# ChunLI-666/PointCloudProcessor

Hardware: AMD Instinct MI355X
Metric: Mpoints×frames/sec colorized (higher is better)
Workload: dtype f32/f64

## Files before the change

### include/pcp_hip.h

```cpp
#ifndef PCP_HIP_H
#define PCP_HIP_H

#include <stdint.h>

#ifdef __cplusplus
extern "C" {
#endif

#define PCP_ABI_VERSION 6

#define PCP_OK 0
#define PCP_ERR_INVALID (-1)
#define PCP_ERR_STATE (-2)
#define PCP_ERR_DEVICE (-3)
#define PCP_ERR_NOMEM (-4)
#define PCP_ERR_RANGE (-5)

typedef struct pcp_context pcp_context;

typedef struct pcp_pose {
  double x, y, z, qw, qx, qy, qz;
} pcp_pose;

typedef struct pcp_camera {
// ... 87 lines not shown
  int32_t h, v;
  int32_t blocks_w, blocks_h;
  int32_t down_w, down_h;
} pcp_jpeg_component;
typedef struct pcp_jpeg_header {
  uint32_t magic, version;
  int32_t width, height, ncomp, reserved;
  pcp_jpeg_component comp[3];
  int64_t n_blocks, n_values;
  int64_t quant_off, mask_off, offset_off, value_off;
} pcp_jpeg_header;
int pcp_upload_image_jpeg(pcp_context *ctx, int32_t frame, const uint8_t *blob, int64_t bytes);
int pcp_upload_image_jpeg_async(pcp_context *ctx, int32_t frame, const uint8_t *blob, int64_t bytes);
int pcp_upload_mask(pcp_context *ctx, int32_t frame, const uint8_t *gray, int64_t row_stride_bytes);

int pcp_project_frame(pcp_context *ctx, int32_t frame, int32_t *out_cell, int32_t *out_pixel, float *out_range,
                      float *out_xyz_cam);
int pcp_cull_frame(pcp_context *ctx, int32_t frame, uint8_t *out_keep, int64_t *out_kept, float *out_depth_map);
int pcp_frame_visible(pcp_context *ctx, int32_t frame, int64_t capacity, int32_t *out_index, uint8_t *out_rgb,
                      uint16_t *out_mask, float *out_xyz_cam, float *out_xyz_world, int64_t *out_count);

int pcp_hpr_stats(pcp_context *ctx, int64_t out[10]);

int pcp_depth_pass(pcp_context *ctx, int32_t frame_begin, int32_t frame_end);
int pcp_depth_maps_device(pcp_context *ctx, void **device_ptr, int64_t *n_floats);
int pcp_download_depth_map(pcp_context *ctx, int32_t frame, float *out_depth_map);
int pcp_depth_accum_reset(pcp_context *ctx);
int pcp_depth_accum_merge(pcp_context *ctx);
int pcp_depth_accum_apply(pcp_context *ctx);
int pcp_depth_accum_device(pcp_context *ctx, void **device_ptr, int64_t *n_floats);
#define PCP_DEPTH_OWN 0
#define PCP_DEPTH_BATCHED 1
int pcp_set_depth_source(pcp_context *ctx, int32_t source);
int pcp_hull_flags_import(pcp_context *ctx, int32_t frame, const uint8_t *keep);
int pcp_colour_reset(pcp_context *ctx);
int pcp_colour_pass(pcp_context *ctx, int32_t frame_begin, int32_t frame_end);
int pcp_colour_finalise(pcp_context *ctx, uint8_t *out_rgb, uint8_t *out_has, int32_t *out_count,
                        float *out_top_score, uint32_t *out_top_rgb, int32_t *out_top_frame);
int pcp_colorize(pcp_context *ctx, uint8_t *out_rgb, uint8_t *out_has);
int pcp_colorize_from_depth(pcp_context *ctx, uint8_t *out_rgb, uint8_t *out_has);
int pcp_download_result_packed(pcp_context *ctx, uint32_t *out_rgba);
int pcp_download_result_packed_async(pcp_context *ctx, uint32_t *out_rgba);
int pcp_download_wait_previous(pcp_context *ctx);
int pcp_colour_result_device(pcp_context *ctx, void **device_ptr, int64_t *n_words);
int pcp_colour_compact(pcp_context *ctx, int64_t capacity, int32_t *out_index, float *out_xyz, uint8_t *out_rgb, uint8_t *out_label,
                       int64_t *out_count);

int pcp_set_label_fusion(pcp_context *ctx, int32_t enable);
int pcp_colour_labels(pcp_context *ctx, uint8_t *out_label, uint8_t *out_hits, uint8_t *out_views);
int pcp_colour_labels_device(pcp_context *ctx, void **device_ptr, int64_t *n_words);

int pcp_view_pair_stats(pcp_context *ctx, uint64_t *out_n, uint64_t *out_sum);
int pcp_view_pair_stats_counters(pcp_context *ctx, int64_t out[5]);
int pcp_exposure_gains(int32_t n_frames, const uint64_t *n, const uint64_t *sum, double sigma_n, double sigma_g, double *out_gains);
int pcp_set_frame_gains(pcp_context *ctx, const double *gains, int32_t n);

int pcp_colour_smooth_local(pcp_context *ctx, float radius, int64_t *out_has_count);
int pcp_colour_smooth_local_packed(pcp_context *ctx, float radius, const uint32_t *in_rgba, uint32_t *out_rgba,
                                   int64_t *out_has_count);

int pcp_mls_process(pcp_context *ctx, const pcp_mls_params *p, int64_t *out_count);
int pcp_set_mls_local_plane(pcp_context *ctx, double upsampling_radius, double upsampling_step);
int pcp_mls_local_plane_samples(double radius, double step, int64_t capacity, float *out_u, float *out_v, int64_t *out_count);
int pcp_mls_process_shard(pcp_context *ctx, const pcp_mls_params *p, int64_t index_begin, int64_t index_end,
                          int64_t *out_count);
int pcp_mls_process_slab(pcp_context *ctx, const pcp_mls_params *p, int32_t slab, int32_t n_slabs, int64_t *out_count);
int pcp_mls_stream_begin(pcp_context *ctx, const pcp_mls_params *p, int64_t chunk_capacity, int64_t *out_total,
                         int32_t *out_chunks);
int pcp_mls_stream_next(pcp_context *ctx, int64_t *out_count);
int pcp_mls_stream_seek(pcp_context *ctx, int32_t chunk);
int pcp_mls_fetch(pcp_context *ctx, int64_t capacity, float *out_xyz, float *out_normal, float *out_curvature,
                  int32_t *out_index);
int pcp_cloud_smooth(pcp_context *ctx, const pcp_mls_params *p, int64_t *out_count);

int pcp_cloud_smooth_stream_begin(pcp_context *ctx, const pcp_mls_params *p, int64_t chunk_capacity, int64_t *out_total_rows,
                                  int64_t *out_kept_rows, int32_t *out_chunks);
int pcp_cloud_smooth_stream_next(pcp_context *ctx, int64_t *out_count);
int pcp_cloud_smooth_stream_end(pcp_context *ctx);
int pcp_cloud_smooth_stream_seek(pcp_context *ctx, int32_t chunk);
int pcp_cloud_smooth_stream_stats(pcp_context *ctx, double out[13]);
int pcp_sor(pcp_context *ctx, int32_t mean_k, double std_mul, uint8_t *out_keep, int64_t *out_kept);
int64_t pcp_sor_chunk_points(void);
int pcp_sor_partial(pcp_context *ctx, int32_t mean_k, int32_t slab, int32_t n_slabs, int64_t capacity, double *out_chunk_sums,
                    int64_t *out_first_chunk, int64_t *out_chunks);
int pcp_sor_finish(pcp_context *ctx, double std_mul, const double *all_chunk_sums, int64_t n_chunks, int32_t slab, int32_t n_slabs,
                   uint8_t *out_keep, int64_t *out_kept);

int pcp_upload_intensity(pcp_context *ctx, const float *intensity, int64_t n);
int pcp_nid_prepare(pcp_context *ctx, int64_t *out_points);
int pcp_nid_evaluate(pcp_context *ctx, const double T[16], const double *T_init, int32_t bins, double *cost,
                     double grad6[6], int32_t *valid);
int pcp_nid_optimize(pcp_context *ctx, const double T_init[16], int32_t bins, int32_t max_outer_iterations,
                     double T_out[16], double *final_cost, int32_t *evaluations);

int pcp_nid_accumulate(pcp_context *ctx, const double T[16], int32_t bins);
int pcp_nid_histograms_device(pcp_context *ctx, void **device_ptr, int64_t *count);
int pcp_nid_finish(pcp_context *ctx, int32_t bins, double *cost, double grad6[6], int32_t *valid);
typedef int (*pcp_nid_eval_fn)(void *user, const double T[16], int32_t bins, double *cost, double grad6[6], int32_t *valid);
int pcp_nid_optimize_with(pcp_context *ctx, pcp_nid_eval_fn eval, void *user, const double T_init[16], int32_t bins,
                          int32_t max_outer_iterations, double T_out[16], double *final_cost, int32_t *evaluations);

#define PCP_ROWS_XYZI 0
#define PCP_ROWS_XYZRGB 1
#define PCP_ROWS_XYZRGBMASK 2
#define PCP_ROWS_POINTNORMAL 3
int64_t pcp_ascii_row_bound(int32_t kind);
int pcp_ascii_rows_host(int32_t kind, int64_t n, const float *f, const uint8_t *rgb, const uint16_t *mask, int64_t capacity,
                        char *out_text, int64_t *out_bytes);
int pcp_ascii_rows(pcp_context *ctx, int32_t kind, int64_t n, const float *f, const uint8_t *rgb, const uint16_t *mask,
                   int64_t capacity, char *out_text, int64_t *out_bytes);
int pcp_colour_compact_ascii(pcp_context *ctx, int32_t with_label, int64_t first_row, int64_t max_rows, int64_t capacity,
                             char *out_text, int64_t *out_rows, int64_t *out_bytes);
int pcp_mls_fetch_ascii(pcp_context *ctx, int64_t first_row, int64_t max_rows, int64_t capacity, char *out_text,
                        int64_t *out_rows, int64_t *out_bytes);

#define PCP_ASCII_PARSE_MAX_ROW 65536
#define PCP_PARSE_LIMIT_ROW 0
#define PCP_PARSE_LIMIT_TILE 1
#define PCP_PARSE_LIMIT_PIECE 2
#define PCP_PARSE_LIMIT_TILE_ROWS 3
#define PCP_PARSE_LIMIT_WINDOW 4
int64_t pcp_ascii_parse_limit(int32_t which);
int pcp_ascii_parse_host(const char *text, int64_t bytes, int32_t columns, const int32_t col[4], int32_t final_window,
                         int64_t max_rows, float *out_x, float *out_y, float *out_z, float *out_intensity,
                         int64_t *out_rows, int64_t *out_consumed, int64_t *out_bad_row);
int pcp_ascii_parse(pcp_context *ctx, const char *text, int64_t bytes, int32_t columns, const int32_t col[4], int32_t final_window,
                    int64_t max_rows, float *out_x, float *out_y, float *out_z, float *out_intensity,
                    int64_t *out_rows, int64_t *out_consumed, int64_t *out_bad_row);

int pcp_voxel_reduce_begin(pcp_context *ctx, float leaf, int64_t initial_slots);
int pcp_voxel_reduce_add(pcp_context *ctx, int64_t *out_rows_added);
int pcp_voxel_reduce_finish(pcp_context *ctx, int64_t *out_voxels);
int pcp_voxel_reduce_fetch(pcp_context *ctx, int64_t first, int64_t max_rows, float *out_xyz, uint8_t *out_rgb, uint8_t *out_label,
                           uint32_t *out_count, int64_t *out_rows);
int pcp_voxel_reduce_stats(pcp_context *ctx, int64_t out[6]);
int pcp_voxel_reduce_end(pcp_context *ctx);
int pcp_voxel_reduce_host(float leaf, int64_t n, const float *xyz, const uint8_t *rgb, const uint8_t *label, int64_t capacity,
                          float *out_xyz, uint8_t *out_rgb, uint8_t *out_label, uint32_t *out_count, int64_t *out_voxels);

int pcp_estimate_normals(pcp_context *ctx, float radius, int64_t *out_valid, int64_t *out_moments);
int pcp_normals_fetch(pcp_context *ctx, float *out_normal, float *out_curvature, int32_t *out_neighbours);
int pcp_normals_moments_host(float radius, int64_t n, const float *xyz, int64_t *out_moments);
int pcp_frame_geometry(pcp_context *ctx, int32_t frame, int32_t *out_index, float *out_range, float *out_xyz_cam,
                       float *out_normal_cam, int64_t *out_pixels);

int pcp_close_pairs(pcp_context *ctx, double radius, int64_t *points_with_close_neighbour);

int pcp_timing_enable(pcp_context *ctx, int32_t on);
int pcp_timing_reset(pcp_context *ctx);
int pcp_timing_get(pcp_context *ctx, int32_t kernel_id, double *total_ms, int64_t *launches);
const char *pcp_kernel_name(int32_t kernel_id);
int pcp_tile_mask_density(pcp_context *ctx, double *kept_fraction);
int pcp_tile_masks(pcp_context *ctx, int64_t *tiles, int32_t *mask_words, uint32_t *out_words);
int pcp_sor_redo_fraction(pcp_context *ctx, double *fraction);
int pcp_sor_distances(pcp_context *ctx, int64_t capacity, float *out_distance);
int pcp_selftest_arithmetic(pcp_context *ctx, int64_t samples, uint64_t seed, int64_t *mismatches_fp64,
                            int64_t *mismatches_fp32);
int pcp_selftest_visit_forms(pcp_context *ctx, int64_t samples, uint64_t seed, int64_t *mismatches_uv, int64_t *mismatches_cell,
                             int64_t *mismatches_sqrt, int32_t *short_distortion);

#ifdef __cplusplus
}
#endif
#endif
```

### pointcloudprocessor_amd/_build.py

```python
from __future__ import annotations

import os
import subprocess

_PKG = os.path.dirname(os.path.abspath(__file__))
_ROOT = os.path.dirname(_PKG)
CSRC = os.path.join(_PKG, "csrc")
LIB_DIR = os.path.join(_PKG, "lib")
LIB_PATH = os.path.join(LIB_DIR, "libpcp_hip.so")
INCLUDE = os.path.join(_ROOT, "include")

SOURCES = ["pcp_context.hip", "pcp_colour.hip", "pcp_mls.hip", "pcp_nid.hip", "pcp_hpr.hip", "pcp_colour_smooth.hip", "pcp_match.hip", "pcp_jpeg.hip",
           "pcp_stream_colour.hip", "pcp_ascii.hip", "pcp_ascii_parse.hip", "pcp_exposure.hip", "pcp_voxel_reduce.hip", "pcp_normals.hip"]
HEADERS = ["pcp_internal.hpp", "pcp_device.hpp", "pcp_scan.hpp", "pcp_hsv.hpp", "pcp_exact.hpp", "pcp_ascii.hpp", "pcp_ascii_parse.hpp", "pcp_visit_forms.hpp", "pcp_voxel_reduce.hpp", "pcp_eigen33.hpp", "pcp_normals.hpp"]

HIPCC_FLAGS = [
    "--offload-arch=gfx950",
    "-O3",
    "-std=c++17",
    "-fPIC",
    "-ffp-contract=off",
    "-fhip-fp32-correctly-rounded-divide-sqrt",
    "-Wall",
    "-Wextra",
]


def _hipcc() -> str:
    for cand in (os.environ.get("HIPCC"), "/opt/rocm/bin/hipcc", "hipcc"):
        if cand and (os.path.isabs(cand) and os.path.exists(cand) or not os.path.isabs(cand)):
            return cand
    return "hipcc"


def source_sha256() -> str:
    import hashlib

    h = hashlib.sha256()
    h.update(" ".join(HIPCC_FLAGS).encode())
    for f in [os.path.join(CSRC, f) for f in SOURCES + HEADERS] + [os.path.join(INCLUDE, "pcp_hip.h")]:
        h.update(os.path.basename(f).encode())
        with open(f, "rb") as fh:
            h.update(fh.read())
    return h.hexdigest()


def is_stale() -> bool:
    if not os.path.exists(LIB_PATH):
        return True
    t = os.path.getmtime(LIB_PATH)
    deps = [os.path.join(CSRC, f) for f in SOURCES + HEADERS] + [os.path.join(INCLUDE, "pcp_hip.h")]
    return any(os.path.getmtime(d) > t for d in deps)


def build(force: bool = False, verbose: bool = False) -> str:
    if not force and not is_stale():
        return LIB_PATH
    os.makedirs(LIB_DIR, exist_ok=True)
    from concurrent.futures import ThreadPoolExecutor

    obj_dir = os.path.join(LIB_DIR, "obj")
    os.makedirs(obj_dir, exist_ok=True)
    inc = ["-I", os.path.relpath(INCLUDE, CSRC), "-I", "."]

    def compile_one(src):
        stem = os.path.splitext(src)[0]
        obj = os.path.join(os.path.relpath(obj_dir, CSRC), stem + ".o")
        cmd = [_hipcc()] + HIPCC_FLAGS + inc + [f"-cuid={stem}", "-c", src, "-o", obj]
        return cmd, subprocess.run(cmd, capture_output=True, text=True, cwd=CSRC)

    with ThreadPoolExecutor(max_workers=len(SOURCES)) as pool:
        results = list(pool.map(compile_one, SOURCES))
    log = ""
    for cmd, proc in results:
        if verbose or proc.returncode != 0:
            log += " ".join(cmd) + "\n" + proc.stdout + proc.stderr
    if any(proc.returncode != 0 for _, proc in results):
        print(log)
        raise RuntimeError("hipcc failed building libpcp_hip.so:\n" + log[-4000:])
    objs = [os.path.join(os.path.relpath(obj_dir, CSRC), os.path.splitext(src)[0] + ".o") for src in SOURCES]
    link = [_hipcc(), "--offload-arch=gfx950", "--hip-link", "-shared", "-fPIC", "-o", LIB_PATH] + objs
    proc = subprocess.run(link, capture_output=True, text=True, cwd=CSRC)
    if verbose or proc.returncode != 0:
        print(log + " ".join(link))
        print(proc.stdout)
        print(proc.stderr)
    if proc.returncode != 0:
        raise RuntimeError("hipcc failed linking libpcp_hip.so:\n" + proc.stderr[-4000:])
    return LIB_PATH


if __name__ == "__main__":
    print(build(force=True, verbose=True))
```

### pointcloudprocessor_amd/capi.py

```python
from __future__ import annotations

import ctypes as C
import os
import re

import numpy as np

from . import _build

PCP_OK = 0
PCP_ERR_INVALID = -1
PCP_ERR_STATE = -2
PCP_ERR_DEVICE = -3
PCP_ERR_NOMEM = -4
PCP_ERR_RANGE = -5

NID_EVAL_FN = C.CFUNCTYPE(C.c_int, C.c_void_p, C.POINTER(C.c_double), C.c_int32, C.POINTER(C.c_double), C.POINTER(C.c_double),
                          C.POINTER(C.c_int32))
K_PROJECT, K_DEPTH, K_COLOUR, K_VISIBILITY, K_MLS_GRID, K_MLS_FIT, K_MISC, K_SOR, K_MLS_VOXEL, K_TILE_MASK, K_NID, K_HPR = range(12)
K_COLOUR_SMOOTH = 12
K_COUNT = 13


class PcpError(RuntimeError):
# ... 780 lines not shown
        xyz = np.empty((count, 3), np.float32)
        nrm = np.empty((count, 3), np.float32)
        curv = np.empty(count, np.float32)
        idx = np.empty(count, np.int32)
        self._check(self.lib.pcp_mls_fetch(self.h, C.c_int64(count), _ptr(xyz), _ptr(nrm), _ptr(curv), _ptr(idx)))
        return dict(xyz=xyz, normal=nrm, curvature=curv, index=idx)

    def mls_fetch_index(self, count: int) -> np.ndarray:
        idx = np.empty(count, np.int32)
        self._check(self.lib.pcp_mls_fetch(self.h, C.c_int64(count), None, None, None, _ptr(idx)))
        return idx

    def sor(self, mean_k: int = 60, std_mul: float = 0.7):
        keep = np.empty(self.n, np.uint8)
        kept = C.c_int64()
        self._check(self.lib.pcp_sor(self.h, C.c_int32(mean_k), C.c_double(std_mul), _ptr(keep), C.byref(kept)))
        return keep, kept.value

    def sor_chunk_points(self) -> int:
        return int(self.lib.pcp_sor_chunk_points())

    def sor_partial(self, mean_k: int, slab: int, n_slabs: int):
        c = self.sor_chunk_points()
        chunks = (self.n + c - 1) // c
        out = np.zeros((max(chunks, 1), 2), np.float64)
        first, cnt = C.c_int64(), C.c_int64()
        self._check(self.lib.pcp_sor_partial(self.h, C.c_int32(mean_k), C.c_int32(slab), C.c_int32(n_slabs), C.c_int64(len(out)),
                                             _ptr(out), C.byref(first), C.byref(cnt)))
        return first.value, out[:cnt.value].copy()

    def sor_finish(self, std_mul: float, all_chunk_sums: np.ndarray, slab: int, n_slabs: int):
        sums = np.ascontiguousarray(all_chunk_sums, np.float64)
        keep = np.empty(self.n, np.uint8)
        kept = C.c_int64()
        self._check(self.lib.pcp_sor_finish(self.h, C.c_double(std_mul), _ptr(sums), C.c_int64(len(sums)), C.c_int32(slab),
                                            C.c_int32(n_slabs), _ptr(keep), C.byref(kept)))
        return keep, kept.value

    def close_pairs(self, radius: float = 2.5e-5) -> int:
        cnt = C.c_int64()
        self._check(self.lib.pcp_close_pairs(self.h, C.c_double(radius), C.byref(cnt)))
        return cnt.value

    def sor_distances(self) -> np.ndarray:
        out = np.empty(self.n, np.float32)
        self._check(self.lib.pcp_sor_distances(self.h, C.c_int64(len(out)), _ptr(out)))
        return out

    def sor_redo_fraction(self) -> float:
        v = C.c_double()
        self._check(self.lib.pcp_sor_redo_fraction(self.h, C.byref(v)))
        return v.value

    def upload_intensity(self, intensity):
        a = np.ascontiguousarray(intensity, np.float32)
        self._check(self.lib.pcp_upload_intensity(self.h, _ptr(a), C.c_int64(len(a))))

    def nid_prepare(self) -> int:
        cnt = C.c_int64()
        self._check(self.lib.pcp_nid_prepare(self.h, C.byref(cnt)))
        return cnt.value

    def nid_evaluate(self, T, T_init=None, bins: int = 16):
        T = np.ascontiguousarray(T, np.float64).reshape(16)
        Ti = None if T_init is None else np.ascontiguousarray(T_init, np.float64).reshape(16)
        cost = C.c_double()
        grad = np.zeros(6, np.float64)
        valid = C.c_int32()
        self._check(self.lib.pcp_nid_evaluate(self.h, _ptr(T), _ptr(Ti), C.c_int32(bins), C.byref(cost), _ptr(grad),
                                              C.byref(valid)))
        return cost.value, grad, bool(valid.value)

    def nid_optimize(self, T_init, bins: int = 16, max_outer_iterations: int = 10):
        Ti = np.ascontiguousarray(T_init, np.float64).reshape(16)
        out = np.zeros(16, np.float64)
        cost = C.c_double()
        evals = C.c_int32()
        self._check(self.lib.pcp_nid_optimize(self.h, _ptr(Ti), C.c_int32(bins), C.c_int32(max_outer_iterations), _ptr(out),
                                              C.byref(cost), C.byref(evals)))
        return out.reshape(4, 4), cost.value, evals.value

    def nid_accumulate(self, T, bins: int = 16):
        T = np.ascontiguousarray(T, np.float64).reshape(16)
        self._check(self.lib.pcp_nid_accumulate(self.h, _ptr(T), C.c_int32(bins)))

    def nid_histograms_device(self):
        p = C.c_void_p()
        n = C.c_int64()
        self._check(self.lib.pcp_nid_histograms_device(self.h, C.byref(p), C.byref(n)))
        return p.value, n.value

    def nid_finish(self, bins: int = 16):
        cost = C.c_double()
        grad = np.zeros(6, np.float64)
        valid = C.c_int32()
        self._check(self.lib.pcp_nid_finish(self.h, C.c_int32(bins), C.byref(cost), _ptr(grad), C.byref(valid)))
        return cost.value, grad, bool(valid.value)

    def nid_optimize_with(self, evaluate, T_init, bins: int = 16, max_outer_iterations: int = 10):
        errors = []

        @NID_EVAL_FN
        def trampoline(_user, T, b, cost, grad, valid):
            try:
                c, g, ok = evaluate(np.ctypeslib.as_array(T, (16,)).copy().reshape(4, 4), int(b))
                cost[0] = float(c)
                for k in range(6):
                    grad[k] = float(g[k])
                valid[0] = 1 if ok else 0
                return 0
            except Exception as e:
                errors.append(e)
                return -3

        Ti = np.ascontiguousarray(T_init, np.float64).reshape(16)
        out = np.zeros(16, np.float64)
        cost = C.c_double()
        evals = C.c_int32()
        rc = self.lib.pcp_nid_optimize_with(self.h, trampoline, None, _ptr(Ti), C.c_int32(bins), C.c_int32(max_outer_iterations),
                                            _ptr(out), C.byref(cost), C.byref(evals))
        if errors:
            raise errors[0]
        self._check(rc)
        return out.reshape(4, 4), cost.value, evals.value

    def timing_enable(self, on: bool = True):
        self._check(self.lib.pcp_timing_enable(self.h, C.c_int32(1 if on else 0)))

    def timing_reset(self):
        self._check(self.lib.pcp_timing_reset(self.h))

    def timing_get(self, kernel_id: int):
        ms = C.c_double()
        cnt = C.c_int64()
        self._check(self.lib.pcp_timing_get(self.h, C.c_int32(kernel_id), C.byref(ms), C.byref(cnt)))
        return ms.value, cnt.value

    def tile_mask_density(self) -> float:
        v = C.c_double()
        self._check(self.lib.pcp_tile_mask_density(self.h, C.byref(v)))
        return v.value

    def selftest_arithmetic(self, samples: int = 1 << 26, seed: int = 1):
        a, b = C.c_int64(), C.c_int64()
        self._check(self.lib.pcp_selftest_arithmetic(self.h, C.c_int64(samples), C.c_uint64(seed), C.byref(a), C.byref(b)))
        return a.value, b.value

    def selftest_visit_forms(self, samples: int = 1 << 24, seed: int = 1):
        a, b, c, f = C.c_int64(), C.c_int64(), C.c_int64(), C.c_int32()
        self._check(self.lib.pcp_selftest_visit_forms(self.h, C.c_int64(samples), C.c_uint64(seed), C.byref(a), C.byref(b), C.byref(c),
                                                      C.byref(f)))
        return a.value, b.value, c.value, bool(f.value)

    def tile_masks(self) -> np.ndarray:
        t, w = C.c_int64(), C.c_int32()
        self._check(self.lib.pcp_tile_masks(self.h, C.byref(t), C.byref(w), None))
        out = np.empty((t.value, w.value), np.uint32)
        self._check(self.lib.pcp_tile_masks(self.h, None, None, _ptr(out)))
        return out

    def kernel_name(self, kernel_id: int) -> str:
        return self.lib.pcp_kernel_name(C.c_int32(kernel_id)).decode()
```

### pointcloudprocessor_amd/csrc/pcp_colour.hip

```cpp
#include <algorithm>
#include <cfloat>
#include <cstdlib>

#include "pcp_device.hpp"
#include "pcp_hsv.hpp"
#include "pcp_scan.hpp"

namespace pcp {

constexpr int kBlock = 256;
constexpr uint32_t kFltMaxBits = 0x7f7fffffu;

template <bool kCommon>
__device__ __forceinline__ DevCamera common_camera(const DevCamera &in) {
  DevCamera c = in;
  if constexpr (kCommon) {
    c.cull_mode = PCP_CULL_ZBUFFER;
    c.enable_zbuf = 1;
    c.pretest = 1;
    c.ds_fast = 1;
  }
  return c;
}
inline bool is_common_camera(const pcp_context *ctx) {
  const DevCamera &c = ctx->dcam;
  return c.cull_mode == PCP_CULL_ZBUFFER && c.enable_zbuf == 1 && c.pretest == 1 && c.ds_fast == 1 && ctx->uv_tame;
}

struct ProjectOut {
  int32_t *cell;
  int32_t *pixel;
  float *range;
  float *xc, *yc, *zc;
};

__device__ __forceinline__ void project_store_one(const DevCamera &cam, const DevFrame &fr, float x, float y, float z,
                                                  int32_t &cell, int32_t &pixel, float &range, float &xc, float &yc,
                                                  float &zc) {
  const Projected p = project_point<true, false>(cam, fr.w2c, x, y, z);
  cell = p.cell;
  pixel = p.pixel;
  range = p.cell != -1 ? static_cast<float>(range64(p.xc, p.yc, p.zc)) : FLT_MAX;
  xc = p.xc;
  yc = p.yc;
  zc = p.zc;
}

template <bool kCommon>
__global__ __launch_bounds__(kBlock) void k_project_frame(const float *__restrict__ x, const float *__restrict__ y,
                                                          const float *__restrict__ z, int64_t n, DevCamera cam_in,
                                                          DevFrame fr, ProjectOut out) {
  const DevCamera cam = common_camera<kCommon>(cam_in);
  const int64_t q = static_cast<int64_t>(blockIdx.x) * kBlock + threadIdx.x;
  const int64_t i0 = q * 4;
  if (i0 >= n) return;
  if (i0 + 3 < n) {
    typedef float nt_f4 __attribute__((ext_vector_type(4)));
    typedef int nt_i4 __attribute__((ext_vector_type(4)));
    const nt_f4 ax = __builtin_nontemporal_load(reinterpret_cast<const nt_f4 *>(x + i0));
    const nt_f4 ay = __builtin_nontemporal_load(reinterpret_cast<const nt_f4 *>(y + i0));
    const nt_f4 az = __builtin_nontemporal_load(reinterpret_cast<const nt_f4 *>(z + i0));
    const float4 vx = make_float4(ax.x, ax.y, ax.z, ax.w), vy = make_float4(ay.x, ay.y, ay.z, ay.w),
                 vz = make_float4(az.x, az.y, az.z, az.w);
    int4 cell, pixel;
    float4 range, xc, yc, zc;
    project_store_one(cam, fr, vx.x, vy.x, vz.x, cell.x, pixel.x, range.x, xc.x, yc.x, zc.x);
    project_store_one(cam, fr, vx.y, vy.y, vz.y, cell.y, pixel.y, range.y, xc.y, yc.y, zc.y);
    project_store_one(cam, fr, vx.z, vy.z, vz.z, cell.z, pixel.z, range.z, xc.z, yc.z, zc.z);
    project_store_one(cam, fr, vx.w, vy.w, vz.w, cell.w, pixel.w, range.w, xc.w, yc.w, zc.w);
    if (out.cell) {
      const nt_i4 c4 = {cell.x, cell.y, cell.z, cell.w};
      __builtin_nontemporal_store(c4, reinterpret_cast<nt_i4 *>(out.cell + i0));
    }
    if (out.range) {
      const nt_f4 r4 = {range.x, range.y, range.z, range.w};
      __builtin_nontemporal_store(r4, reinterpret_cast<nt_f4 *>(out.range + i0));
    }
    if (out.pixel) *reinterpret_cast<int4 *>(out.pixel + i0) = pixel;
    if (out.xc) {
      *reinterpret_cast<float4 *>(out.xc + i0) = xc;
      *reinterpret_cast<float4 *>(out.yc + i0) = yc;
      *reinterpret_cast<float4 *>(out.zc + i0) = zc;
    }
  } else {
    for (int64_t i = i0; i < n; ++i) {
      int32_t cell, pixel;
      float range, xc, yc, zc;
      project_store_one(cam, fr, x[i], y[i], z[i], cell, pixel, range, xc, yc, zc);
      if (out.cell) out.cell[i] = cell;
      if (out.range) out.range[i] = range;
      if (out.pixel) out.pixel[i] = pixel;
      if (out.xc) {
        out.xc[i] = xc;
        out.yc[i] = yc;
        out.zc[i] = zc;
      }
    }
  }
}

struct Interval {
  double lo, hi;
};
__device__ __forceinline__ Interval iv_add(Interval a, Interval b) { return {a.lo + b.lo, a.hi + b.hi}; }
__device__ __forceinline__ Interval iv_scale(double k, Interval a) {
  return k >= 0.0 ? Interval{k * a.lo, k * a.hi} : Interval{k * a.hi, k * a.lo};
}
__device__ __forceinline__ Interval iv_mul(Interval a, Interval b) {
  const double p0 = a.lo * b.lo, p1 = a.lo * b.hi, p2 = a.hi * b.lo, p3 = a.hi * b.hi;
  return {fmin(fmin(p0, p1), fmin(p2, p3)), fmax(fmax(p0, p1), fmax(p2, p3))};
}
__device__ __forceinline__ Interval iv_sqr(Interval a) {
  const double l = fabs(a.lo), h = fabs(a.hi);
  const double mx = fmax(l, h), mn = (a.lo <= 0.0 && a.hi >= 0.0) ? 0.0 : fmin(l, h);
  return {mn * mn, mx * mx};
}
__device__ __forceinline__ Interval iv_mul_pos(Interval a, Interval b) { return {a.lo * b.lo, a.hi * b.hi}; }
__device__ __forceinline__ Interval iv_mul_by_pos(Interval a, Interval b) {
  return {a.lo * (a.lo >= 0.0 ? b.lo : b.hi), a.hi * (a.hi >= 0.0 ? b.hi : b.lo)};
}
__device__ __forceinline__ double iv_rcp_pos(double b) {
  double r = __builtin_amdgcn_rcp(b);
  r = fma(fma(-b, r, 1.0), r, r);
  r = fma(fma(-b, r, 1.0), r, r);
  return r;
}
__device__ __forceinline__ Interval iv_pad(Interval a) {
  const double e = 1e-12 * (fabs(a.lo) + fabs(a.hi)) + 1e-300;
  return {a.lo - e, a.hi + e};
}

__device__ __forceinline__ int tile_classify(const DevCamera &c, const DevFrame &fr, float4 sph) {
  const double cx = sph.x, cy = sph.y, cz = sph.z;
  const float *m = fr.w2c;
  const double X = (m[0] * cx + m[1] * cy) + (m[2] * cz + m[3]);
  const double Y = (m[4] * cx + m[5] * cy) + (m[6] * cz + m[7]);
  const double Z = (m[8] * cx + m[9] * cy) + (m[10] * cz + m[11]);
  const double mag = fr.norm_bound * (fabs(cx) + fabs(cy) + fabs(cz) + 3.0 * sph.w) + fabs(static_cast<double>(m[3])) +
                     fabs(static_cast<double>(m[7])) + fabs(static_cast<double>(m[11])) + 1e-3;
  const double rho = fr.norm_bound * static_cast<double>(sph.w) * (1.0 + 1e-6) + 1e-6 * mag;
  if (!(rho >= 0.0) || !isfinite(X + Y + Z + rho)) return 0;
  if (Z + rho <= 0.0) return 1;
  if (Z - rho <= 0.0) return 0;
  const Interval zi{Z - rho, Z + rho};
  if (!(zi.lo >= 1e-290)) return 0;
  const Interval iz{iv_rcp_pos(zi.hi) * (1.0 - 1e-13), iv_rcp_pos(zi.lo) * (1.0 + 1e-13)};
  const Interval xn = iv_pad(iv_mul_by_pos(Interval{X - rho, X + rho}, iz));
  const Interval yn = iv_pad(iv_mul_by_pos(Interval{Y - rho, Y + rho}, iz));
  const Interval x2 = iv_sqr(xn), y2 = iv_sqr(yn);
  const Interval r2 = iv_add(x2, y2);
  const Interval r4 = iv_mul_pos(r2, r2);
  const Interval r6 = iv_mul_pos(r2, r4);
  Interval rc = iv_add(iv_add(iv_scale(c.k1, r2), iv_scale(c.k2, r4)), iv_scale(c.k3, r6));
  rc.lo += 1.0;
  rc.hi += 1.0;
  const Interval t1 = iv_scale(2.0, iv_mul(xn, yn));
  const Interval t2 = iv_add(r2, iv_scale(2.0, x2));
  const Interval t3 = iv_add(r2, iv_scale(2.0, y2));
  const Interval xd = iv_pad(iv_add(iv_add(iv_mul(rc, xn), iv_scale(c.p1, t1)), iv_scale(c.p2, t2)));
  const Interval yd = iv_pad(iv_add(iv_add(iv_mul(rc, yn), iv_scale(c.p1, t3)), iv_scale(c.p2, t1)));
  Interval u = iv_pad(iv_scale(c.fx, xd)), v = iv_pad(iv_scale(c.fy, yd));
  u.lo += c.cx; u.hi += c.cx;
  v.lo += c.cy; v.hi += c.cy;
  if (!isfinite(u.lo + u.hi + v.lo + v.hi)) return 0;
  if (u.hi < static_cast<double>(c.u_lo) || u.lo > static_cast<double>(c.u_hi) ||
      v.hi < static_cast<double>(c.v_lo) || v.lo > static_cast<double>(c.v_hi))
    return 1;
  return (u.lo > static_cast<double>(c.u_lo) + 1.0 && u.hi < static_cast<double>(c.u_hi) - 1.0 &&
          v.lo > static_cast<double>(c.v_lo) + 1.0 && v.hi < static_cast<double>(c.v_hi) - 1.0)
             ? 2
             : 0;
}

constexpr int kTileGroup = 16;

__global__ __launch_bounds__(kBlock) void k_group_mask_flat(const float4 *__restrict__ spheres, int64_t groups, DevCamera cam,
                                                            const DevFrame *__restrict__ frames, int32_t n_frames,
                                                            int32_t w0, int32_t w1, int32_t words,
                                                            uint32_t *__restrict__ group_mask,
                                                            uint32_t *__restrict__ group_inside, int32_t cull_enabled,
                                                            int32_t *__restrict__ zeroed, int32_t n_zeroed,
                                                            unsigned long long *__restrict__ far_maps, int64_t far_cells) {
  const int64_t idx = static_cast<int64_t>(blockIdx.x) * kBlock + threadIdx.x;
  if (idx < n_zeroed) zeroed[idx] = 0;
  for (int64_t c = idx; c < far_cells; c += static_cast<int64_t>(gridDim.x) * kBlock) far_maps[c] = 0x7f7f7f7f7f7f7f7full;
  const int32_t nw = w1 - w0;
  const int64_t gw = idx >> 5;
  const int64_t group = gw / nw;
  const bool live = group < groups;
  const int32_t w = w0 + static_cast<int32_t>(gw - group * nw);
  const int32_t f = (w << 5) + static_cast<int32_t>(idx & 31);
  int cls = 1;
  if (live && f < n_frames) cls = cull_enabled ? tile_classify(cam, frames[f], spheres[group]) : 0;
  const unsigned long long m = __ballot(cls != 1), in = __ballot(cls == 2);
  if (live && (idx & 31) == 0) {
    group_mask[group * words + w] = static_cast<uint32_t>((threadIdx.x & 32) ? (m >> 32) : m);
    group_inside[group * words + w] = static_cast<uint32_t>((threadIdx.x & 32) ? (in >> 32) : in);
  }
}

__global__ __launch_bounds__(kBlock) void k_tile_mask_dense(const float4 *__restrict__ spheres, int64_t tiles,
                                                            DevCamera cam, const DevFrame *__restrict__ frames,
                                                            int32_t n_frames, int32_t w0, int32_t w1, int32_t words,
                                                            const uint32_t *__restrict__ group_mask,
                                                            const uint32_t *__restrict__ group_inside,
                                                            uint32_t *__restrict__ tile_mask,
                                                            uint32_t *__restrict__ inside_mask, int32_t cull_enabled) {
  const int lane = threadIdx.x & 63;
  const int32_t nw = w1 - w0;
  const int64_t gw = static_cast<int64_t>(blockIdx.x) * (kBlock / 64) + (threadIdx.x >> 6);
  const int64_t group = gw / nw;
  if (group >= (tiles + kTileGroup - 1) / kTileGroup) return;
  const int32_t w = w0 + static_cast<int32_t>(gw - group * nw);
  const int t = lane & 15, slot = lane >> 4;
  const int64_t tile = group * kTileGroup + t;
  const bool have = tile < tiles;
  uint32_t todo = __builtin_amdgcn_readfirstlane(group_mask[group * words + w]);
  const int32_t nb = n_frames - (w << 5);
  if (nb < 32) todo &= nb <= 0 ? 0u : ((1u << nb) - 1u);
  const uint32_t whole = __builtin_amdgcn_readfirstlane(group_inside[group * words + w]) & todo;
  todo &= ~whole;
  uint32_t word = whole, inside = whole;
  if (todo) {
    const float4 sph = spheres[have ? tile : tiles - 1];
    while (todo) {
      int32_t bit[4];
#pragma unroll
      for (int k = 0; k < 4; ++k) {
        bit[k] = todo ? __builtin_ctz(todo) : -1;
        todo &= todo - (todo ? 1u : 0u);
      }
      const int32_t b = slot == 0 ? bit[0] : slot == 1 ? bit[1] : slot == 2 ? bit[2] : bit[3];
      int cls = 1;
      if (b >= 0 && have) cls = cull_enabled ? tile_classify(cam, frames[(w << 5) + b], sph) : 0;
      const unsigned long long keep = __ballot(cls != 1), ins = __ballot(cls == 2);
#pragma unroll
      for (int k = 0; k < 4; ++k) {
        if (bit[k] >= 0) {
          word |= static_cast<uint32_t>((keep >> (k * 16 + t)) & 1ull) << bit[k];
          inside |= static_cast<uint32_t>((ins >> (k * 16 + t)) & 1ull) << bit[k];
        }
      }
    }
  }
  if (slot == 0 && have) {
    tile_mask[tile * words + w] = word;
    if (inside_mask) inside_mask[tile * words + w] = inside;
  }
}

constexpr int kWorkBins = 1024;
constexpr int kWorkPerBlock = 1024;
__global__ __launch_bounds__(kBlock) void k_tile_work_hist(const uint32_t *__restrict__ tile_mask, int64_t tiles, int32_t w0,
                                                          int32_t w1, int32_t words, int32_t *__restrict__ tile_work,
                                                          int32_t *__restrict__ hist) {
  __shared__ int32_t cnt[kWorkBins];
  for (int b = threadIdx.x; b < kWorkBins; b += kBlock) cnt[b] = 0;
  __syncthreads();
  const int64_t base = static_cast<int64_t>(blockIdx.x) * kWorkPerBlock;
  for (int q = 0; q < kWorkPerBlock / kBlock; ++q) {
    const int64_t t = base + q * kBlock + threadIdx.x;
    if (t < tiles) {
      int32_t visits = 0;
      for (int32_t w = w0; w < w1; ++w) visits += __builtin_popcount(tile_mask[t * words + w]);
      tile_work[t] = visits;
      atomicAdd(&cnt[min(visits, kWorkBins - 1)], 1);
    }
  }
  __syncthreads();
  for (int b = threadIdx.x; b < kWorkBins; b += kBlock)
    if (cnt[b]) atomicAdd(&hist[b], cnt[b]);
}
__device__ __forceinline__ int32_t block_exclusive_scan(int32_t v, int32_t *total);
__global__ __launch_bounds__(kBlock) void k_work_scatter(const int32_t *__restrict__ work, int64_t tiles,
                                                        const int32_t *__restrict__ hist, int32_t *__restrict__ cursor,
                                                        int32_t *__restrict__ order) {
  __shared__ int32_t cnt[kWorkBins];
  __shared__ int32_t first[kWorkBins];
  for (int b = threadIdx.x; b < kWorkBins; b += kBlock) cnt[b] = 0;
  {
    constexpr int kPer = kWorkBins / kBlock;
    int32_t h[kPer], mine = 0;
#pragma unroll
    for (int k = 0; k < kPer; ++k) {
      h[k] = hist[kWorkBins - 1 - (static_cast<int>(threadIdx.x) * kPer + k)];
      mine += h[k];
    }
    int32_t total = 0;
    int32_t run = block_exclusive_scan(mine, &total);
#pragma unroll
    for (int k = 0; k < kPer; ++k) {
      first[kWorkBins - 1 - (static_cast<int>(threadIdx.x) * kPer + k)] = run;
      run += h[k];
    }
  }
  __syncthreads();
  const int64_t base = static_cast<int64_t>(blockIdx.x) * kWorkPerBlock;
  int32_t bin[kWorkPerBlock / kBlock], rank[kWorkPerBlock / kBlock];
#pragma unroll
  for (int q = 0; q < kWorkPerBlock / kBlock; ++q) {
    const int64_t t = base + q * kBlock + threadIdx.x;
    bin[q] = t < tiles ? min(work[t], kWorkBins - 1) : -1;
    rank[q] = bin[q] >= 0 ? atomicAdd(&cnt[bin[q]], 1) : 0;
  }
  __syncthreads();
  for (int b = threadIdx.x; b < kWorkBins; b += kBlock)
    if (cnt[b]) cnt[b] = first[b] + atomicAdd(&cursor[b], cnt[b]);
  __syncthreads();
#pragma unroll
  for (int q = 0; q < kWorkPerBlock / kBlock; ++q)
    if (bin[q] >= 0) order[cnt[bin[q]] + rank[q]] = static_cast<int32_t>(base + q * kBlock + threadIdx.x);
}

constexpr uint32_t kXcdChunk = 16;
__device__ __forceinline__ uint32_t xcd_chunked_block() {
  constexpr uint32_t kXcd = 8, kSuper = kXcd * kXcdChunk;
  const uint32_t b = blockIdx.x;
  if (b >= (gridDim.x / kSuper) * kSuper) return b;
  const uint32_t x = b % kXcd, slot = b / kXcd;
  return ((slot / kXcdChunk) * kXcd + x) * kXcdChunk + slot % kXcdChunk;
}

constexpr unsigned long long kDepthEmpty = 0x7f7f7f7f7f7f7f7full;
__device__ __forceinline__ void depth_min(unsigned long long *__restrict__ map, int32_t cell, unsigned long long bits) {
  if (bits < map[cell]) atomicMin(map + cell, bits);
}
__device__ __forceinline__ double sumsq64(float xc, float yc, float zc) {
  const double X = xc, Y = yc, Z = zc;
  return (X * X + Y * Y) + Z * Z;
}
__global__ __launch_bounds__(kBlock) void k_depth_finish(const unsigned long long *__restrict__ sq, int64_t count,
                                                         uint32_t *__restrict__ range) {
  int64_t i = static_cast<int64_t>(blockIdx.x) * kBlock + threadIdx.x;
  const int64_t stride = static_cast<int64_t>(gridDim.x) * kBlock;
  for (; i < count; i += stride) {
    const unsigned long long b = sq[i];
    float r = FLT_MAX;
    if (b != kDepthEmpty) r = fminf(static_cast<float>(sqrt(__longlong_as_double(static_cast<long long>(b)))), FLT_MAX);
    range[i] = __float_as_uint(r);
  }
}

__device__ __forceinline__ uint32_t range_bits(int32_t w, int32_t f0, int32_t f1) {
  const int32_t fb = max(f0, w << 5), fe = min(f1, (w << 5) + 32);
  const int32_t nb = fe - fb;
  return nb <= 0 ? 0u : (((nb >= 32) ? 0xffffffffu : ((1u << nb) - 1u)) << (fb & 31));
}

template <bool kCommon>
__global__ __launch_bounds__(kBlock) void k_depth_pass(const float *__restrict__ x, const float *__restrict__ y,
                                                       const float *__restrict__ z, int64_t n, DevCamera cam_in,
                                                       const DevFrame *__restrict__ frames, int32_t f0, int32_t f1,
                                                       unsigned long long *__restrict__ depth, int64_t cells,
                                                       int32_t depth_first_frame, uint32_t *__restrict__ tile_mask,
                                                       const uint32_t *__restrict__ tile_inside, int32_t words,
                                                       const int32_t *__restrict__ tile_order) {
  DevCamera cam = common_camera<kCommon>(cam_in);
  if constexpr (kCommon) cam.pretest = 0;
  __shared__ unsigned long long combine[kBlock];
  const int lane = threadIdx.x & 63;
  unsigned long long *tbl = combine + (threadIdx.x & ~63);
  const int64_t j = tile_order ? static_cast<int64_t>(tile_order[blockIdx.x]) * 64 + threadIdx.x
                               : static_cast<int64_t>(xcd_chunked_block()) * kBlock + threadIdx.x;
  const bool live = j < n;
  if (!__ballot(live)) return;
  const float px = live ? x[j] : 0.0f, py = live ? y[j] : 0.0f, pz = live ? z[j] : 0.0f;
  const int64_t tile = __builtin_amdgcn_readfirstlane(static_cast<int32_t>(j >> 6));
  const bool finite_sure = cam.frames_bounded != 0 && __all(fabsf(px) <= 0x1p40f && fabsf(py) <= 0x1p40f && fabsf(pz) <= 0x1p40f);
  unsigned long long *held_at = nullptr;
  unsigned long long held_bits = 0ull, held_seen = 0ull;
  auto settle_held = [&]() {
    if (held_at && held_bits < held_seen) atomicMin(held_at, held_bits);
    held_at = nullptr;
  };
  for (int32_t w = f0 >> 5; w <= (f1 - 1) >> 5; ++w) {
    const uint32_t in_range = range_bits(w, f0, f1);
    uint32_t todo = in_range;
    if (tile_mask) todo &= tile_mask[tile * words + w];
    todo = __builtin_amdgcn_readfirstlane(todo);
    const uint32_t inside = tile_inside ? __builtin_amdgcn_readfirstlane(tile_inside[tile * words + w]) : 0u;
    uint32_t seen = 0u;
    while (todo) {
      const int32_t b = __builtin_ctz(todo);
      const int32_t f = (w << 5) + b;
      todo &= todo - 1u;
      const DevFrame &fr = frames[f];
      const auto p = project_visit<true, kCommon>(cam, fr.w2c, px, py, pz, ((inside >> b) & 1u) == 0u, finite_sure);
      bool in_map, cand;
      if constexpr (kCommon) {
        in_map = live && p.map_ok;
        cand = in_map && p.image_ok;
      } else {
        in_map = live && p.cell >= 0;
        cand = live && p.pixel >= 0 && (cam.enable_zbuf ? p.cell >= 0 : p.cell != -1);
      }
      if (__builtin_amdgcn_ballot_w64(cand)) seen |= 1u << b;
      settle_held();
      if (cam.enable_zbuf && __builtin_amdgcn_ballot_w64(in_map)) {
        unsigned long long *map = depth + static_cast<uint64_t>(static_cast<uint32_t>(f - depth_first_frame)) * static_cast<uint32_t>(cells);
        unsigned long long key = ~0ull, sbits = 0ull;
        if (in_map) {
          sbits = static_cast<unsigned long long>(__double_as_longlong(sumsq64(p.xc, p.yc, p.zc)));
          key = (static_cast<unsigned long long>(static_cast<uint32_t>(p.cell)) << 32) | (sbits >> 32);
        }
        tbl[lane] = ~0ull;
        __builtin_amdgcn_wave_barrier();
        if (in_map) atomicMin(&tbl[p.cell & 63], key);
        __builtin_amdgcn_wave_barrier();
        if (in_map) {
          const unsigned long long got = tbl[p.cell & 63];
          if (got == key || static_cast<uint32_t>(got >> 32) != static_cast<uint32_t>(p.cell)) {
            held_at = map + p.cell;
            held_bits = sbits;
            held_seen = *held_at;
          }
        }
        __builtin_amdgcn_wave_barrier();
      }
    }
    if (tile_mask && lane == 0 && live) {
      uint32_t *dst = tile_mask + tile * words + w;
      *dst = (*dst & ~in_range) | seen;
    }
  }
  settle_held();
}

__global__ __launch_bounds__(kBlock) void k_visibility(const float *__restrict__ x, const float *__restrict__ y,
                                                       const float *__restrict__ z, int64_t n, DevCamera cam,
                                                       DevFrame fr, const uint32_t *__restrict__ depth,
                                                       const int32_t *__restrict__ perm,
                                                       uint8_t *__restrict__ keep, int32_t require_pixel) {
  const int64_t i = static_cast<int64_t>(blockIdx.x) * kBlock + threadIdx.x;
  if (i >= n) return;
  const Projected p = project_point(cam, fr.w2c, x[i], y[i], z[i]);
  bool k = keep_rule(cam, p, depth);
  if (require_pixel) k = k && p.pixel >= 0;
  if (k) keep[perm ? perm[i] : i] = 1;
}

__device__ __forceinline__ bool keep_by_depth(float xc, float yc, float zc, double lim) {
  const double s = sumsq64(xc, yc, zc);
  const double L = lim * lim;
  bool keep = s < L * (1.0 - 0x1p-40);
  const bool sure = lim > 0.0 && (keep || s > L * (1.0 + 0x1p-40));
  if (!sure) keep = !(sqrt(s) > lim);
  return keep;
}

struct TopState {
  float *score;
  uint32_t *rgb;
  int32_t *frame;
  int32_t *count;
};

struct MatchArgs {
  const uint8_t *in_a;
  unsigned long long *moved;
  float e2;
};

struct LabelOut {
  uint32_t *word;
};

template <bool kCommon, int kMatch, bool kOneShot, bool kLabel = false>
__global__ __launch_bounds__(kBlock) void k_colour_pass(const float *__restrict__ x, const float *__restrict__ y,
                                                        const float *__restrict__ z, int64_t n, DevCamera cam_in,
                                                        const DevFrame *__restrict__ frames, int32_t f0, int32_t f1,
                                                        const uint32_t *__restrict__ depth, int64_t cells,
                                                        const uint32_t *__restrict__ tile_mask, int32_t words,
                                                        const uint32_t *__restrict__ images, int64_t image_px,
                                                        TopState st, const int32_t *__restrict__ perm,
                                                        uint32_t *__restrict__ rgba, int32_t flags_in,
                                                        const uint32_t *__restrict__ hull_bits_in, MatchArgs mb,
                                                        [[maybe_unused]] LabelOut lab) {
  constexpr bool kShort = kCommon && kOneShot && kMatch == 2;
  DevCamera cam = common_camera<kCommon>(cam_in);
  if constexpr (kMatch == 1) cam.match_mode = PCP_MATCH_IDENTITY;
  if constexpr (kMatch == 2 || kMatch == 3) cam.match_mode = PCP_MATCH_ROUNDTRIP;
  const uint32_t *__restrict__ hull_bits = kCommon ? nullptr : hull_bits_in;
  const int32_t flags = kOneShot ? 4 : flags_in;
  const int64_t j = static_cast<int64_t>(xcd_chunked_block()) * kBlock + threadIdx.x;
  const bool live = j < n;
  if (!__ballot(live)) return;
  const float px = live ? x[j] : 0.0f, py = live ? y[j] : 0.0f, pz = live ? z[j] : 0.0f;
  const int64_t tile = __builtin_amdgcn_readfirstlane(static_cast<int32_t>(j >> 6));
  const bool finite_sure = cam.frames_bounded != 0 && __all(fabsf(px) <= 0x1p40f && fabsf(py) <= 0x1p40f && fabsf(pz) <= 0x1p40f);
  Top5 t;
  t.init();
  if ((flags & 1) && live) {
    t.s0 = st.score[0 * n + j]; t.s1 = st.score[1 * n + j]; t.s2 = st.score[2 * n + j];
    t.s3 = st.score[3 * n + j]; t.s4 = st.score[4 * n + j];
    t.c0 = st.rgb[0 * n + j]; t.c1 = st.rgb[1 * n + j]; t.c2 = st.rgb[2 * n + j];
    t.c3 = st.rgb[3 * n + j]; t.c4 = st.rgb[4 * n + j];
    t.f0 = st.frame[0 * n + j]; t.f1 = st.frame[1 * n + j]; t.f2 = st.frame[2 * n + j];
    t.f3 = st.frame[3 * n + j]; t.f4 = st.frame[4 * n + j];
    t.count = st.count[j];
  }
  [[maybe_unused]] bool in_a = false;
  [[maybe_unused]] uint32_t moved = 0u;
  if constexpr (kMatch == 3) in_a = live && mb.in_a[j] != 0;
  for (int32_t w = f0 >> 5; w <= (f1 - 1) >> 5; ++w) {
    uint32_t todo = range_bits(w, f0, f1);
    if (tile_mask) todo &= tile_mask[tile * words + w];
    todo = __builtin_amdgcn_readfirstlane(todo);
    const uint32_t hull_word = (hull_bits && live) ? hull_bits[static_cast<int64_t>(w) * n + j] : 0xffffffffu;
    while (todo) {
      const int32_t f = (w << 5) + __builtin_ctz(todo);
      todo &= todo - 1u;
      const DevFrame &fr = frames[f];
      const auto p = project_visit<false, kShort>(cam, fr.w2c, px, py, pz, true, finite_sure);
      bool cand;
      if constexpr (kShort)
        cand = live && p.image_ok && p.map_ok && ((hull_word >> (f & 31)) & 1u);
      else
        cand = live && p.pixel >= 0 && (cam.enable_zbuf ? p.cell >= 0 : p.cell != -1) && ((hull_word >> (f & 31)) & 1u);
      if (cand) {
        const uint32_t dbits = cam.enable_zbuf ? depth[static_cast<uint64_t>(static_cast<uint32_t>(f)) * static_cast<uint32_t>(cells) + static_cast<uint32_t>(p.cell)] : 0u;
        bool keep = true;
        if (cam.enable_zbuf) keep = keep_by_depth(p.xc, p.yc, p.zc, static_cast<double>(__uint_as_float(dbits)) + cam.slack);
        float sx = p.xc, sy = p.yc, sz = p.zc;
        if constexpr (kMatch == 3) {
          if (keep) keep = roundtrip_sample_moved(cam, fr, px, py, pz, sx, sy, sz, mb.e2, moved) && !in_a;
        } else {
          if (cam.match_mode == PCP_MATCH_ROUNDTRIP && keep) keep = roundtrip_sample(cam, fr, px, py, pz, sx, sy, sz);
        }
        if (keep) {
          const uint32_t texel = images[static_cast<uint64_t>(static_cast<uint32_t>(f)) * static_cast<uint32_t>(image_px) + static_cast<uint32_t>(p.pixel)];
          t.insert(final_score<kShort>(sx, sy, sz, fr.px, fr.py, fr.pz), kLabel ? texel : texel & 0xffffffu, f);
        }
      }
    }
  }
  if constexpr (kMatch == 3) {
    if (moved) atomicAdd(mb.moved, static_cast<unsigned long long>(moved));
  }
  if (!live) return;
  if (flags & 2) {
    st.score[0 * n + j] = t.s0; st.score[1 * n + j] = t.s1; st.score[2 * n + j] = t.s2;
    st.score[3 * n + j] = t.s3; st.score[4 * n + j] = t.s4;
    st.rgb[0 * n + j] = t.c0; st.rgb[1 * n + j] = t.c1; st.rgb[2 * n + j] = t.c2;
    st.rgb[3 * n + j] = t.c3; st.rgb[4 * n + j] = t.c4;
    st.frame[0 * n + j] = t.f0; st.frame[1 * n + j] = t.f1; st.frame[2 * n + j] = t.f2;
    st.frame[3 * n + j] = t.f3; st.frame[4 * n + j] = t.f4;
    st.count[j] = t.count;
  }
  if (flags & 4) {
    const int64_t o = perm[j];
    rgba[o] = t.finalise();
    if constexpr (kLabel) {
      uint32_t bad = 0u;
      lab.word[o] = t.labels(bad);
      if (bad) lab.word[n] = 1u;
    }
  }
}

__device__ __forceinline__ Top5 load_top5(const TopState &st, int64_t n, int64_t j) {
  Top5 t;
  t.s0 = st.score[0 * n + j]; t.s1 = st.score[1 * n + j]; t.s2 = st.score[2 * n + j];
  t.s3 = st.score[3 * n + j]; t.s4 = st.score[4 * n + j];
  t.c0 = st.rgb[0 * n + j]; t.c1 = st.rgb[1 * n + j]; t.c2 = st.rgb[2 * n + j];
  t.c3 = st.rgb[3 * n + j]; t.c4 = st.rgb[4 * n + j];
  t.f0 = st.frame[0 * n + j]; t.f1 = st.frame[1 * n + j]; t.f2 = st.frame[2 * n + j];
  t.f3 = st.frame[3 * n + j]; t.f4 = st.frame[4 * n + j];
  t.count = st.count[j];
  return t;
}
__global__ __launch_bounds__(kBlock) void k_finalise(int64_t n, TopState st, const int32_t *__restrict__ perm,
// ... 47 lines not shown
    const DevFrame &fr = frames[f];
    const int32_t w = f >> 5;
    const uint32_t bit = 1u << (f & 31);
    for (int64_t r = r0; r < r1; ++r) {
      const int64_t i = cols[r];
      if (tile_mask && !(tile_mask[(i >> 6) * words + w] & bit)) continue;
      if (hull_bits && !(hull_bits[static_cast<int64_t>(w) * n + i] & bit)) continue;
      const float px = x[i], py = y[i], pz = z[i];
      const Projected p = project_point<false>(cam, fr.w2c, px, py, pz);
      const bool cand = p.pixel >= 0 && (cam.enable_zbuf ? p.cell >= 0 : p.cell != -1);
      if (!cand) continue;
      if (cam.enable_zbuf) {
        const uint32_t dbits = depth[static_cast<uint64_t>(static_cast<uint32_t>(f)) * static_cast<uint32_t>(cells) + static_cast<uint32_t>(p.cell)];
        if (!keep_by_depth(p.xc, p.yc, p.zc, static_cast<double>(__uint_as_float(dbits)) + cam.slack)) continue;
      }
      float sx = p.xc, sy = p.yc, sz = p.zc;
      if (!roundtrip_sample(cam, fr, qx, qy, qz, sx, sy, sz)) continue;
      const uint32_t texel = images[static_cast<uint64_t>(static_cast<uint32_t>(f)) * static_cast<uint32_t>(image_px) + static_cast<uint32_t>(p.pixel)];
      t.insert(final_score(sx, sy, sz, fr.px, fr.py, fr.pz), kLabel ? texel : texel & 0xffffffu, f);
    }
  }
  if (flags & 2) {
    st.score[0 * n + j] = t.s0; st.score[1 * n + j] = t.s1; st.score[2 * n + j] = t.s2;
    st.score[3 * n + j] = t.s3; st.score[4 * n + j] = t.s4;
    st.rgb[0 * n + j] = t.c0; st.rgb[1 * n + j] = t.c1; st.rgb[2 * n + j] = t.c2;
    st.rgb[3 * n + j] = t.c3; st.rgb[4 * n + j] = t.c4;
    st.frame[0 * n + j] = t.f0; st.frame[1 * n + j] = t.f1; st.frame[2 * n + j] = t.f2;
    st.frame[3 * n + j] = t.f3; st.frame[4 * n + j] = t.f4;
    st.count[j] = t.count;
  }
  if (flags & 4) {
    const int64_t o = perm[j];
    rgba[o] = t.finalise();
    if constexpr (kLabel) {
      uint32_t bad = 0u;
      lab.word[o] = t.labels(bad);
      if (bad) lab.word[n] = 1u;
    }
  }
}

template <bool kLabel>
inline auto colour_pass_kernel(bool common, int32_t match_mode, int32_t flags) {
  auto kernel = k_colour_pass<false, 0, false, kLabel>;
  if (common && match_mode == PCP_MATCH_IDENTITY)
    kernel = flags == 4 ? k_colour_pass<true, 1, true, kLabel> : k_colour_pass<true, 1, false, kLabel>;
  if (common && match_mode == PCP_MATCH_ROUNDTRIP)
    kernel = flags == 4 ? k_colour_pass<true, 2, true, kLabel> : k_colour_pass<true, 2, false, kLabel>;
  if (match_mode == PCP_MATCH_RADIUS)
    kernel = !common ? k_colour_pass<false, 3, false, kLabel>
                     : flags == 4 ? k_colour_pass<true, 3, true, kLabel> : k_colour_pass<true, 3, false, kLabel>;
  return kernel;
}

__device__ __forceinline__ uint64_t mix64(uint64_t v) {
  v += 0x9e3779b97f4a7c15ull;
  v = (v ^ (v >> 30)) * 0xbf58476d1ce4e5b9ull;
  v = (v ^ (v >> 27)) * 0x94d049bb133111ebull;
  return v ^ (v >> 31);
}
__device__ __forceinline__ bool same_f64(double a, double b) {
  if (a != a && b != b) return true;
  if (a == 0.0 && b == 0.0) return true;
  return __double_as_longlong(a) == __double_as_longlong(b);
}

__global__ __launch_bounds__(kBlock) void k_selftest_div64(int64_t samples, uint64_t seed,
                                                           unsigned long long *__restrict__ bad) {
  const int64_t i = static_cast<int64_t>(blockIdx.x) * kBlock + threadIdx.x;
  if (i >= samples) return;
  const uint64_t a = mix64(seed ^ static_cast<uint64_t>(i) * 3u), b = mix64(a);
  uint32_t bx = static_cast<uint32_t>(a), by = static_cast<uint32_t>(a >> 32), bz = static_cast<uint32_t>(b);
  const uint32_t mode = static_cast<uint32_t>(b >> 32) & 3u;
  if (mode != 0u) {
    const uint32_t span = mode == 1u ? 12u : 40u;
    bx = (bx & 0x807fffffu) | ((127u - span / 2u + (bx >> 23) % span) << 23);
    by = (by & 0x807fffffu) | ((127u - span / 2u + (by >> 23) % span) << 23);
    bz = (bz & 0x807fffffu) | ((127u - span / 2u + (bz >> 23) % span) << 23);
  }
  const float xc = __uint_as_float(bx), yc = __uint_as_float(by), zc = fabsf(__uint_as_float(bz));
  if (!(zc > 0.0f)) return;
  double xn, yn;
  divide_xy_by_z(xc, yc, zc, xn, yn);
  const double xr = static_cast<double>(xc) / static_cast<double>(zc);
  const double yr = static_cast<double>(yc) / static_cast<double>(zc);
  if (!same_f64(xn, xr) || !same_f64(yn, yr)) atomicAdd(bad, 1ull);
}

__global__ __launch_bounds__(kBlock) void k_selftest_div32(DevCamera cam, unsigned long long *__restrict__ bad) {
  const uint32_t lane = blockIdx.x * kBlock + threadIdx.x;
  uint32_t wrong = 0u;
  for (uint32_t k = 0; k < 256u; ++k) {
    const float x = __uint_as_float((k << 24) | lane);
    const float a = div_by_ds(cam, x), b = x / cam.ds_f;
    const float ax = fabsf(x);
    if (ax >= 0x1p-40f && ax <= 0x1p60f) {
      if (!((a != a && b != b) || __float_as_uint(a) == __float_as_uint(b))) ++wrong;
    } else {
      if (cell_of_quotient(a, cam.cull_wf) != cell_of_quotient(b, cam.cull_wf)) ++wrong;
      if (cell_of_quotient(a, cam.cull_hf) != cell_of_quotient(b, cam.cull_hf)) ++wrong;
    }
  }
  if (wrong) atomicAdd(bad, static_cast<unsigned long long>(wrong));
}

__device__ __forceinline__ bool same_bits_f64(double a, double b) {
  return (a != a && b != b) || __double_as_longlong(a) == __double_as_longlong(b);
}
__global__ __launch_bounds__(kBlock) void k_selftest_uv(DevCamera cam, int32_t tame, int64_t samples, uint64_t seed,
                                                        unsigned long long *__restrict__ bad) {
  const int64_t i = static_cast<int64_t>(blockIdx.x) * kBlock + threadIdx.x;
  if (i >= samples) return;
  const uint64_t a = mix64(seed ^ static_cast<uint64_t>(i) * 3u), b = mix64(a);
  uint32_t bx = static_cast<uint32_t>(a), by = static_cast<uint32_t>(a >> 32), bz = static_cast<uint32_t>(b);
  const uint32_t mode = static_cast<uint32_t>(b >> 32) & 3u;
  if (mode != 0u) {
    const uint32_t span = mode == 1u ? 12u : 40u;
    bx = (bx & 0x807fffffu) | ((127u - span / 2u + (bx >> 23) % span) << 23);
    by = (by & 0x807fffffu) | ((127u - span / 2u + (by >> 23) % span) << 23);
    bz = (bz & 0x807fffffu) | ((127u - span / 2u + (bz >> 23) % span) << 23);
  }
  const float xc = __uint_as_float(bx), yc = __uint_as_float(by), zc = fabsf(__uint_as_float(bz));
  if (!(zc > 0.0f)) return;
  double u0, v0, u1, v1;
  if (tame)
    project_uv<true, true>(cam, xc, yc, zc, u0, v0);
  else
    project_uv<true, false>(cam, xc, yc, zc, u0, v0);
  project_uv<true, false>(cam, xc, yc, zc, u1, v1);
  if (!same_bits_f64(u0, u1) || !same_bits_f64(v0, v1)) atomicAdd(bad, 1ull);
}

__global__ __launch_bounds__(kBlock) void k_selftest_cell_sqrt(DevCamera cam, unsigned long long *__restrict__ bad_cell,
                                                               unsigned long long *__restrict__ bad_sqrt) {
  const uint32_t lane = blockIdx.x * kBlock + threadIdx.x;
  uint32_t wrong_cell = 0u, wrong_sqrt = 0u;
  for (uint32_t k = 0; k < 256u; ++k) {
    const float q = __uint_as_float((k << 24) | lane);
    const float qx[3] = {q, 0.5f, q}, qy[3] = {0.5f, q, q};
#pragma unroll
    for (int t = 0; t < 3; ++t) {
      const int32_t old_cell = vf::map_cell_written(qx[t], qy[t], cam.cull_wf, cam.cull_hf, cam.mw, cam.mh);
      int32_t cell;
      const bool ok = vf::map_cell_short(qx[t], qy[t], vf::map_bound(cam.mw), vf::map_bound(cam.mh), cam.mw, cell);
      if ((ok ? cell : -1) != old_cell) ++wrong_cell;
    }
    const float r0 = sqrt_rn(q), r1 = sqrtf(q);
    if (!((r0 != r0 && r1 != r1) || __float_as_uint(r0) == __float_as_uint(r1))) ++wrong_sqrt;
  }
  if (wrong_cell) atomicAdd(bad_cell, static_cast<unsigned long long>(wrong_cell));
  if (wrong_sqrt) atomicAdd(bad_sqrt, static_cast<unsigned long long>(wrong_sqrt));
}

__global__ __launch_bounds__(kBlock) void k_unpack_result(const uint32_t *__restrict__ packed, int64_t n,
                                                         uint8_t *__restrict__ rgb, uint8_t *__restrict__ has) {
  const int64_t i = static_cast<int64_t>(blockIdx.x) * kBlock + threadIdx.x;
  if (i >= n) return;
  const uint32_t v = packed[i];
  rgb[3 * i + 0] = static_cast<uint8_t>(v & 0xffu);
  rgb[3 * i + 1] = static_cast<uint8_t>((v >> 8) & 0xffu);
  rgb[3 * i + 2] = static_cast<uint8_t>((v >> 16) & 0xffu);
  has[i] = static_cast<uint8_t>(v >> 24);
}

__global__ __launch_bounds__(kBlock) void k_unpack_labels(const uint32_t *__restrict__ packed, int64_t n,
                                                         uint8_t *__restrict__ label, uint8_t *__restrict__ hits,
                                                         uint8_t *__restrict__ views) {
  const int64_t i = static_cast<int64_t>(blockIdx.x) * kBlock + threadIdx.x;
  if (i >= n) return;
  const uint32_t v = packed[i];
  if (label) label[i] = static_cast<uint8_t>(v & 0xffu);
  if (hits) hits[i] = static_cast<uint8_t>((v >> 8) & 0xffu);
  if (views) views[i] = static_cast<uint8_t>((v >> 16) & 0xffu);
}

__global__ __launch_bounds__(kBlock) void k_fill_u32(uint32_t *__restrict__ p, int64_t n, uint32_t v) {
  int64_t i = static_cast<int64_t>(blockIdx.x) * kBlock + threadIdx.x;
  const int64_t stride = static_cast<int64_t>(gridDim.x) * kBlock;
  for (; i < n; i += stride) p[i] = v;
}

__global__ __launch_bounds__(kBlock) void k_scatter_u32(const uint32_t *__restrict__ in,
                                                        const int32_t *__restrict__ perm, int64_t n,
                                                        uint32_t *__restrict__ out) {
  const int64_t j = static_cast<int64_t>(blockIdx.x) * kBlock + threadIdx.x;
  if (j < n) out[perm[j]] = in[j];
}

__global__ __launch_bounds__(kBlock) void k_pack_bgr(const uint8_t *__restrict__ bgr, int64_t row_stride, int32_t w,
                                                     int32_t h, uint32_t *__restrict__ texels, int32_t clear_mask,
                                                     const int32_t *__restrict__ hsv_tables, float sat_scale,
                                                     float val_scale) {
  const int64_t i = static_cast<int64_t>(blockIdx.x) * kBlock + threadIdx.x;
  if (i >= static_cast<int64_t>(w) * h) return;
  const int32_t v = static_cast<int32_t>(i / w), u = static_cast<int32_t>(i - static_cast<int64_t>(v) * w);
  const uint8_t *p = bgr + static_cast<int64_t>(v) * row_stride + 3 * u;
  const uint32_t keep = clear_mask ? 0u : (texels[i] & 0xff000000u);
  uint32_t b = p[0], g = p[1], r = p[2];
  if (hsv_tables) hsv_round_trip(hsv_tables, hsv_tables + 256, sat_scale, val_scale, b, g, r);
  texels[i] = keep | b | (g << 8) | (r << 16);
}

__global__ __launch_bounds__(kBlock) void k_pack_bgr16(const uint8_t *__restrict__ bgr, int64_t row_stride, int32_t w,
                                                       int32_t h, uint32_t *__restrict__ texels, int32_t clear_mask,
                                                       const int32_t *__restrict__ hsv_tables, float sat_scale,
                                                       float val_scale) {
  const int32_t groups = w >> 4;
  const int64_t n_groups = static_cast<int64_t>(groups) * h;
  const int64_t g = static_cast<int64_t>(blockIdx.x) * kBlock + threadIdx.x;
  uint4 a, b, c;
  if (row_stride == 3 * static_cast<int64_t>(w)) {
    __shared__ uint4 piece[3 * kBlock];
    const int64_t base = static_cast<int64_t>(blockIdx.x) * (3 * kBlock);
    const int64_t pieces = 3 * n_groups;
    const uint4 *src = reinterpret_cast<const uint4 *>(bgr);
#pragma unroll
    for (int q = 0; q < 3; ++q) {
      const int64_t i = base + q * kBlock + threadIdx.x;
      if (i < pieces) piece[q * kBlock + threadIdx.x] = src[i];
    }
    __syncthreads();
    if (g >= n_groups) return;
    a = piece[3 * threadIdx.x];
    b = piece[3 * threadIdx.x + 1];
    c = piece[3 * threadIdx.x + 2];
  } else {
    if (g >= n_groups) return;
    const int32_t vr = static_cast<int32_t>(g / groups), gr = static_cast<int32_t>(g - static_cast<int64_t>(vr) * groups);
    const uint4 *src = reinterpret_cast<const uint4 *>(bgr + static_cast<int64_t>(vr) * row_stride + static_cast<int64_t>(gr) * 48);
    a = src[0];
    b = src[1];
    c = src[2];
  }
  const int32_t v = static_cast<int32_t>(g / groups), gu = static_cast<int32_t>(g - static_cast<int64_t>(v) * groups);
  const uint32_t in[12] = {a.x, a.y, a.z, a.w, b.x, b.y, b.z, b.w, c.x, c.y, c.z, c.w};
  uint4 *dst = reinterpret_cast<uint4 *>(texels + static_cast<int64_t>(v) * w + static_cast<int64_t>(gu) * 16);
  uint32_t out[16];
#pragma unroll
  for (int q = 0; q < 4; ++q) {
    const uint32_t d0 = in[3 * q], d1 = in[3 * q + 1], d2 = in[3 * q + 2];
    out[4 * q + 0] = d0 & 0xffffffu;
    out[4 * q + 1] = (d0 >> 24) | ((d1 & 0xffffu) << 8);
    out[4 * q + 2] = (d1 >> 16) | ((d2 & 0xffu) << 16);
    out[4 * q + 3] = d2 >> 8;
  }
  if (hsv_tables) {
#pragma unroll
    for (int k = 0; k < 16; ++k) {
      uint32_t bb = out[k] & 0xffu, gg = (out[k] >> 8) & 0xffu, rr = out[k] >> 16;
      hsv_round_trip(hsv_tables, hsv_tables + 256, sat_scale, val_scale, bb, gg, rr);
      out[k] = bb | (gg << 8) | (rr << 16);
    }
  }
  if (!clear_mask) {
#pragma unroll
    for (int q = 0; q < 4; ++q) {
      const uint4 old = dst[q];
      out[4 * q + 0] |= old.x & 0xff000000u;
      out[4 * q + 1] |= old.y & 0xff000000u;
      out[4 * q + 2] |= old.z & 0xff000000u;
      out[4 * q + 3] |= old.w & 0xff000000u;
    }
  }
#pragma unroll
  for (int q = 0; q < 4; ++q) dst[q] = make_uint4(out[4 * q], out[4 * q + 1], out[4 * q + 2], out[4 * q + 3]);
}

__global__ __launch_bounds__(kBlock) void k_pack_mask(const uint8_t *__restrict__ gray, int64_t row_stride, int32_t w,
                                                      int32_t h, uint32_t *__restrict__ texels) {
  const int64_t i = static_cast<int64_t>(blockIdx.x) * kBlock + threadIdx.x;
  if (i >= static_cast<int64_t>(w) * h) return;
  const int32_t v = static_cast<int32_t>(i / w), u = static_cast<int32_t>(i - static_cast<int64_t>(v) * w);
  texels[i] = (texels[i] & 0x00ffffffu) | (static_cast<uint32_t>(gray[static_cast<int64_t>(v) * row_stride + u]) << 24);
}

constexpr int kTile = 1024;

__device__ __forceinline__ int32_t block_exclusive_scan(int32_t v, int32_t *total) {
  __shared__ int32_t wave_sum[kBlock / 64];
  const int lane = threadIdx.x & 63, wid = threadIdx.x >> 6;
  int32_t incl = v;
#pragma unroll
  for (int o = 1; o < 64; o <<= 1) {
    const int32_t t = __shfl_up(incl, o, 64);
    if (lane >= o) incl += t;
  }
  if (lane == 63) wave_sum[wid] = incl;
  __syncthreads();
  int32_t base = 0, tot = 0;
#pragma unroll
  for (int k = 0; k < kBlock / 64; ++k) {
    if (k < wid) base += wave_sum[k];
    tot += wave_sum[k];
  }
  __syncthreads();
  *total = tot;
  return base + incl - v;
}

__global__ __launch_bounds__(kBlock) void k_tile_count(const uint8_t *__restrict__ flags, int64_t n,
                                                       int32_t *__restrict__ tile_count) {
  const int64_t base = static_cast<int64_t>(blockIdx.x) * kTile + threadIdx.x * 4;
  int32_t c = 0;
#pragma unroll
  for (int k = 0; k < 4; ++k)
    if (base + k < n) c += flags[base + k] ? 1 : 0;
// ... 597 lines not shown
                       row_stride_bytes, w, h, ctx->images.p + static_cast<int64_t>(frame) * px);
    PCP_HIP_TRY(ctx, hipGetLastError());
  }
  PCP_HIP_TRY(ctx, hipStreamSynchronize(ctx->stream));
  ctx->mask_set[static_cast<size_t>(frame)] = 1;
  return PCP_OK;
}

int pcp_project_frame(pcp_context *ctx, int32_t frame, int32_t *out_cell, int32_t *out_pixel, float *out_range,
                      float *out_xyz_cam) {
  int rc = check_ready(ctx, "pcp_project_frame", true);
  if (rc != PCP_OK) return rc;
  if ((rc = check_frame(ctx, "pcp_project_frame", frame)) != PCP_OK) return rc;
  const int64_t n = ctx->n;
  const size_t plane = plane_of(ctx);
  PCP_HIP_TRY(ctx, ctx->s_cell.ensure(plane + 4));
  PCP_HIP_TRY(ctx, ctx->s_range.ensure(plane + 4));
  if (out_pixel) PCP_HIP_TRY(ctx, ctx->s_pixel.ensure(plane + 4));
  if (out_xyz_cam) PCP_HIP_TRY(ctx, ctx->s_cam.ensure(3 * plane + 4));
  if (n == 0) return PCP_OK;
  ProjectOut o{};
  o.cell = ctx->s_cell.p;
  o.range = ctx->s_range.p;
  o.pixel = out_pixel ? ctx->s_pixel.p : nullptr;
  o.xc = out_xyz_cam ? ctx->s_cam.p : nullptr;
  o.yc = out_xyz_cam ? ctx->s_cam.p + plane : nullptr;
  o.zc = out_xyz_cam ? ctx->s_cam.p + 2 * plane : nullptr;
  {
    LaunchTimer t(ctx, PCP_K_PROJECT);
    hipLaunchKernelGGL(is_common_camera(ctx) ? k_project_frame<true> : k_project_frame<false>, dim3(blocks_for(div_up(n, 4))), dim3(kBlock), 0, ctx->stream, ctx->sxyz.p,
                       ctx->sxyz.p + plane, ctx->sxyz.p + 2 * plane, n, ctx->dcam,
                       ctx->hframes[static_cast<size_t>(frame)], o);
    PCP_HIP_TRY(ctx, hipGetLastError());
  }
  if (!(out_cell || out_range || out_pixel || out_xyz_cam)) return PCP_OK;
  const size_t sn = static_cast<size_t>(n);
  PCP_HIP_TRY(ctx, ctx->s_u32.ensure(plane + 4));
  auto fetch = [&](const void *sorted, void *host) -> int {
    {
      LaunchTimer t(ctx, PCP_K_MISC);
      hipLaunchKernelGGL(k_scatter_u32, dim3(blocks_for(n)), dim3(kBlock), 0, ctx->stream,
                         static_cast<const uint32_t *>(sorted), ctx->perm.p, n, ctx->s_u32.p);
      PCP_HIP_TRY(ctx, hipGetLastError());
    }
    PCP_HIP_TRY(ctx, hipMemcpyAsync(host, ctx->s_u32.p, sn * 4, hipMemcpyDeviceToHost, ctx->stream));
    PCP_HIP_TRY(ctx, hipStreamSynchronize(ctx->stream));
    return PCP_OK;
  };
  if (out_cell && (rc = fetch(o.cell, out_cell)) != PCP_OK) return rc;
  if (out_range && (rc = fetch(o.range, out_range)) != PCP_OK) return rc;
  if (out_pixel && (rc = fetch(o.pixel, out_pixel)) != PCP_OK) return rc;
  if (out_xyz_cam) {
    if ((rc = fetch(o.xc, out_xyz_cam)) != PCP_OK) return rc;
    if ((rc = fetch(o.yc, out_xyz_cam + sn)) != PCP_OK) return rc;
    if ((rc = fetch(o.zc, out_xyz_cam + 2 * sn)) != PCP_OK) return rc;
  }
  return PCP_OK;
}

int pcp_cull_frame(pcp_context *ctx, int32_t frame, uint8_t *out_keep, int64_t *out_kept, float *out_depth_map) {
  int rc = check_ready(ctx, "pcp_cull_frame", true);
  if (rc != PCP_OK) return rc;
  if ((rc = check_frame(ctx, "pcp_cull_frame", frame)) != PCP_OK) return rc;
  const int64_t n = ctx->n;
  if ((rc = single_frame_depth(ctx, frame)) != PCP_OK) return rc;
  if ((rc = frame_keep_flags(ctx, frame, false)) != PCP_OK) return rc;
  if (out_kept) {
    int64_t cnt = 0;
    if (n > 0 && (rc = compact_flags(ctx, ctx->s_keep.p, n, nullptr, 0, &cnt)) != PCP_OK) return rc;
    *out_kept = cnt;
  }
  if (out_keep && n > 0)
    PCP_HIP_TRY(ctx, hipMemcpyAsync(out_keep, ctx->s_keep.p, static_cast<size_t>(n), hipMemcpyDefault, ctx->stream));
  if (out_depth_map)
    PCP_HIP_TRY(ctx, hipMemcpyAsync(out_depth_map, ctx->s_u32.p, static_cast<size_t>(cells_of(ctx)) * 4,
                                    hipMemcpyDeviceToHost, ctx->stream));
  PCP_HIP_TRY(ctx, hipStreamSynchronize(ctx->stream));
  return PCP_OK;
}

int pcp_frame_visible(pcp_context *ctx, int32_t frame, int64_t capacity, int32_t *out_index, uint8_t *out_rgb,
                      uint16_t *out_mask, float *out_xyz_cam, float *out_xyz_world, int64_t *out_count) {
  int rc = check_ready(ctx, "pcp_frame_visible", true);
  if (rc != PCP_OK) return rc;
  if ((rc = check_frame(ctx, "pcp_frame_visible", frame)) != PCP_OK) return rc;
  if (capacity < 0) return set_error(ctx, PCP_ERR_INVALID, "pcp_frame_visible: negative capacity");
  const int64_t n = ctx->n;
  if (out_count) *out_count = 0;
  if (n == 0) return PCP_OK;
  if ((rc = ensure_images(ctx)) != PCP_OK) return rc;
  if ((rc = wait_images(ctx, frame, frame + 1)) != PCP_OK) return rc;
  int64_t m = 0;
  if ((rc = visible_indices(ctx, frame, &m)) != PCP_OK) return rc;
  const size_t plane = plane_of(ctx);
  if (out_count) *out_count = m;
  const int64_t take = std::min(m, capacity);
  if (take == 0) return PCP_OK;
  const size_t st = static_cast<size_t>(take);
  PCP_HIP_TRY(ctx, ctx->s_range.ensure(st + 4));
  const bool want_cam = out_xyz_cam != nullptr, want_world = out_xyz_world != nullptr;
  PCP_HIP_TRY(ctx, ctx->s_cam.ensure((want_cam ? 3 * st : 0) + (want_world ? 3 * st : 0) + 4));
  float *d_cam = want_cam ? ctx->s_cam.p : nullptr;
  float *d_world = want_world ? ctx->s_cam.p + (want_cam ? 3 * st : 0) : nullptr;
  const int64_t px = static_cast<int64_t>(ctx->dcam.img_w) * ctx->dcam.img_h;
  {
    LaunchTimer t(ctx, PCP_K_MISC);
    hipLaunchKernelGGL(k_gather_visible, dim3(blocks_for(take)), dim3(kBlock), 0, ctx->stream, ctx->xyz.p,
                       ctx->xyz.p + plane, ctx->xyz.p + 2 * plane, ctx->dcam, ctx->hframes[static_cast<size_t>(frame)],
                       ctx->s_cell.p, take, ctx->images.p + static_cast<int64_t>(frame) * px,
                       static_cast<int32_t>(ctx->image_set[static_cast<size_t>(frame)]),
                       static_cast<int32_t>(ctx->mask_set[static_cast<size_t>(frame)]),
                       reinterpret_cast<uint32_t *>(ctx->s_range.p), d_cam, d_world);
    PCP_HIP_TRY(ctx, hipGetLastError());
  }
  std::vector<uint32_t> rgbm;
  if (out_rgb || out_mask) {
    rgbm.resize(st);
    PCP_HIP_TRY(ctx, hipMemcpyAsync(rgbm.data(), ctx->s_range.p, st * 4, hipMemcpyDeviceToHost, ctx->stream));
  }
  if (out_index) PCP_HIP_TRY(ctx, hipMemcpyAsync(out_index, ctx->s_cell.p, st * 4, hipMemcpyDeviceToHost, ctx->stream));
  if (want_cam) PCP_HIP_TRY(ctx, hipMemcpyAsync(out_xyz_cam, d_cam, 3 * st * 4, hipMemcpyDeviceToHost, ctx->stream));
  if (want_world) PCP_HIP_TRY(ctx, hipMemcpyAsync(out_xyz_world, d_world, 3 * st * 4, hipMemcpyDeviceToHost, ctx->stream));
  PCP_HIP_TRY(ctx, hipStreamSynchronize(ctx->stream));
  for (size_t k = 0; k < rgbm.size(); ++k) {
    if (out_rgb) {
      out_rgb[3 * k + 0] = static_cast<uint8_t>(rgbm[k] & 0xffu);
      out_rgb[3 * k + 1] = static_cast<uint8_t>((rgbm[k] >> 8) & 0xffu);
      out_rgb[3 * k + 2] = static_cast<uint8_t>((rgbm[k] >> 16) & 0xffu);
    }
    if (out_mask) out_mask[k] = static_cast<uint16_t>(rgbm[k] >> 24);
  }
  return PCP_OK;
}

int pcp_depth_pass(pcp_context *ctx, int32_t frame_begin, int32_t frame_end) {
  int rc = check_ready(ctx, "pcp_depth_pass", true);
  if (rc != PCP_OK) return rc;
  if (frame_begin < 0 || frame_end > ctx->n_frames || frame_begin > frame_end)
    return set_error(ctx, PCP_ERR_RANGE, "pcp_depth_pass: keyframe range [%d,%d) outside 0..%d", frame_begin, frame_end,
                     ctx->n_frames);
  if (frame_begin == frame_end) return PCP_OK;
  if ((rc = ensure_depth(ctx)) != PCP_OK) return rc;
  const int64_t cells = cells_of(ctx);
  const int64_t map_cells = static_cast<int64_t>(frame_end - frame_begin) * cells;
  const bool z_maps = ctx->n > 0 && ctx->dcam.enable_zbuf;
  if (z_maps) {
    PCP_HIP_TRY(ctx, ctx->depth_sq.ensure(static_cast<size_t>(map_cells) + 4));
  } else if ((rc = fill_u32(ctx, ctx->depth.p + static_cast<int64_t>(frame_begin) * cells, map_cells, kFltMaxBits)) != PCP_OK) {
    return rc;
  }
  if (ctx->n > 0) {
    const size_t plane = plane_of(ctx);
    const int32_t w0 = frame_begin >> 5, w1 = ((frame_end - 1) >> 5) + 1;
    static const bool cull_tiles = [] {
      const char *e = std::getenv("PCP_DISABLE_TILE_CULL");
      return !(e && e[0] == '1');
    }();
    {
      LaunchTimer t(ctx, PCP_K_TILE_MASK);
      const int64_t groups = div_up(ctx->n_tiles, kTileGroup);
      const float4 *tile_sph = reinterpret_cast<const float4 *>(ctx->tile_sphere.p);
      const size_t gwords = static_cast<size_t>(groups) * ctx->mask_words;
      PCP_HIP_TRY(ctx, ctx->group_mask.ensure(2 * gwords + 8));
      uint32_t *group_inside = ctx->group_mask.p + gwords + 4;
      hipLaunchKernelGGL(k_group_mask_flat, dim3(std::max(blocks_for(groups * (w1 - w0) * 32), blocks_for(2 * kWorkBins))),
                         dim3(kBlock), 0, ctx->stream, tile_sph + ctx->n_tiles, groups, ctx->dcam, ctx->frames.p, ctx->n_frames,
                         w0, w1, ctx->mask_words, ctx->group_mask.p, group_inside, cull_tiles ? 1 : 0, ctx->work_hist.p,
                         2 * kWorkBins, z_maps ? reinterpret_cast<unsigned long long *>(ctx->depth_sq.p) : nullptr,
                         z_maps ? map_cells : int64_t(0));
      hipLaunchKernelGGL(k_tile_mask_dense, dim3(static_cast<uint32_t>(div_up(groups * (w1 - w0), kBlock / 64))), dim3(kBlock),
                         0, ctx->stream, tile_sph, ctx->n_tiles, ctx->dcam, ctx->frames.p, ctx->n_frames, w0, w1,
                         ctx->mask_words, ctx->group_mask.p, group_inside, ctx->tile_mask.p, ctx->tile_inside.p, cull_tiles ? 1 : 0);
      if ((rc = sort_tiles_by_work(ctx, w0, w1, ctx->tile_order.p)) != PCP_OK) return rc;
      ctx->tile_order_live = true;
    }
    if (ctx->cull.cull_mode == PCP_CULL_HPR) {
      int rch = ensure_hull_bits(ctx);
      if (rch != PCP_OK) return rch;
      if (!ctx->depth_from_batch) {
        int32_t clear_until = frame_begin;
        for (int32_t f = frame_begin; f < frame_end; ++f) {
          uint32_t *hull_plane = ctx->hull_bits.p + static_cast<size_t>(f >> 5) * static_cast<size_t>(ctx->n);
          if ((f & 31) == 0 && std::min(f + 32, ctx->n_frames) <= frame_end) {
            PCP_HIP_TRY(ctx, hipMemsetAsync(hull_plane, 0, static_cast<size_t>(ctx->n) * 4, ctx->stream));
            clear_until = std::min(f + 32, ctx->n_frames);
          }
          if (f >= clear_until) {
            LaunchTimer t(ctx, PCP_K_HPR);
            hipLaunchKernelGGL(k_hull_clear, dim3(blocks_for(ctx->n)), dim3(kBlock), 0, ctx->stream, hull_plane, ctx->n, 1u << (f & 31));
          }
        }
        PCP_HIP_TRY(ctx, hipGetLastError());
        const char *le = std::getenv("PCP_HPR_LANES");
        const int32_t lanes = le && le[0] >= '1' && le[0] <= '8' ? le[0] - '0' : 4;
        if ((rc = hpr_run_range(ctx, frame_begin, frame_end, lanes, ctx->tile_mask.p)) != PCP_OK) return rc;
        for (int32_t f = frame_begin; f < frame_end; ++f) ctx->hull_valid[static_cast<size_t>(f)] = 1;
      }
    }
    {
      LaunchTimer t(ctx, PCP_K_DEPTH);
      hipLaunchKernelGGL(is_common_camera(ctx) ? k_depth_pass<true> : k_depth_pass<false>,
                         dim3(static_cast<uint32_t>(ctx->n_tiles)), dim3(64), 0, ctx->stream, ctx->sxyz.p,
                         ctx->sxyz.p + plane, ctx->sxyz.p + 2 * plane, ctx->n, ctx->dcam, ctx->frames.p, frame_begin,
                         frame_end, ctx->depth_sq.p, cells, frame_begin, ctx->tile_mask.p, ctx->tile_inside.p,
                         ctx->mask_words, ctx->tile_order.p);
      if (z_maps)
        hipLaunchKernelGGL(k_depth_finish, dim3(static_cast<uint32_t>(std::min<int64_t>(div_up(map_cells, kBlock), 4096))),
                           dim3(kBlock), 0, ctx->stream, ctx->depth_sq.p, map_cells,
                           ctx->depth.p + static_cast<int64_t>(frame_begin) * cells);
      PCP_HIP_TRY(ctx, hipGetLastError());
    }
  }
  for (int32_t f = frame_begin; f < frame_end; ++f) ctx->depth_valid[static_cast<size_t>(f)] = 1;
  return PCP_OK;
}

int pcp_depth_maps_device(pcp_context *ctx, void **device_ptr, int64_t *n_floats) {
  int rc = check_ready(ctx, "pcp_depth_maps_device", true);
  if (rc != PCP_OK) return rc;
  if (ctx->cull.cull_mode == PCP_CULL_HPR)
    return set_error(ctx, PCP_ERR_STATE, "pcp_depth_maps_device: PCP_CULL_HPR has no depth maps to merge across point shards "
                     "(the hull needs the whole map on one GPU)");
  if ((rc = ensure_depth(ctx)) != PCP_OK) return rc;
  if (device_ptr) *device_ptr = ctx->depth.p;
  if (n_floats) *n_floats = cells_of(ctx) * ctx->n_frames;
  return PCP_OK;
}

int pcp_set_depth_source(pcp_context *ctx, int32_t source) {
  if (!ctx) return PCP_ERR_INVALID;
  if (source != PCP_DEPTH_OWN && source != PCP_DEPTH_BATCHED)
    return set_error(ctx, PCP_ERR_INVALID, "pcp_set_depth_source: unknown source %d", source);
  ctx->depth_from_batch = source == PCP_DEPTH_BATCHED;
  return PCP_OK;
}

int pcp_hull_flags_import(pcp_context *ctx, int32_t frame, const uint8_t *keep) {
  int rc = check_ready(ctx, "pcp_hull_flags_import", true);
  if (rc != PCP_OK) return rc;
  if ((rc = check_frame(ctx, "pcp_hull_flags_import", frame)) != PCP_OK) return rc;
  if (ctx->cull.cull_mode != PCP_CULL_HPR || !ctx->depth_from_batch)
    return set_error(ctx, PCP_ERR_STATE, "pcp_hull_flags_import: needs cull_mode PCP_CULL_HPR and pcp_set_depth_source(PCP_DEPTH_BATCHED)");
  if (!keep && ctx->n > 0) return set_error(ctx, PCP_ERR_INVALID, "pcp_hull_flags_import: NULL flags");
  if ((rc = ensure_hull_bits(ctx)) != PCP_OK) return rc;
  if (ctx->n > 0) {
    PCP_HIP_TRY(ctx, ctx->s_keep.ensure(static_cast<size_t>(ctx->n) + 16));
    PCP_HIP_TRY(ctx, hipMemcpyAsync(ctx->s_keep.p, keep, static_cast<size_t>(ctx->n), hipMemcpyDefault, ctx->stream));
    if ((rc = store_hull_bits(ctx, frame, false)) != PCP_OK) return rc;
    PCP_HIP_TRY(ctx, hipStreamSynchronize(ctx->stream));
  }
  ctx->hull_valid[static_cast<size_t>(frame)] = 1;
  return PCP_OK;
}

int pcp_download_depth_map(pcp_context *ctx, int32_t frame, float *out_depth_map) {
  int rc = check_ready(ctx, "pcp_download_depth_map", true);
  if (rc != PCP_OK) return rc;
  if ((rc = check_frame(ctx, "pcp_download_depth_map", frame)) != PCP_OK) return rc;
  if (!out_depth_map) return set_error(ctx, PCP_ERR_INVALID, "pcp_download_depth_map: NULL output");
  if (!ctx->depth.p || !ctx->depth_valid[static_cast<size_t>(frame)])
    return set_error(ctx, PCP_ERR_STATE, "pcp_download_depth_map: pcp_depth_pass has not covered keyframe %d", frame);
  const int64_t cells = cells_of(ctx);
  PCP_HIP_TRY(ctx, hipMemcpyAsync(out_depth_map, ctx->depth.p + static_cast<int64_t>(frame) * cells,
                                  static_cast<size_t>(cells) * 4, hipMemcpyDeviceToHost, ctx->stream));
  PCP_HIP_TRY(ctx, hipStreamSynchronize(ctx->stream));
  return PCP_OK;
}

int pcp_colour_reset(pcp_context *ctx) {
  if (!ctx) return PCP_ERR_INVALID;
  ctx->colour_state_live = false;
  ctx->colour_result_live = false;
  ctx->labels_live = false;
  return PCP_OK;
}

static int begin_result(pcp_context *ctx, uint32_t **dst) {
  const int32_t cur = ctx->rgba_cur ^ 1;
  PCP_HIP_TRY(ctx, ctx->rgba2[cur].ensure(static_cast<size_t>(ctx->n) + 4));
  if (ctx->copy_pending[cur]) {
    PCP_HIP_TRY(ctx, hipStreamWaitEvent(ctx->stream, ctx->copy_done[cur], 0));
    ctx->copy_pending[cur] = false;
  }
  *dst = ctx->rgba2[cur].p;
  return PCP_OK;
}

static int labels_begin(pcp_context *ctx) {
  ctx->labels_live = false;
  if (!ctx->label_fusion) return PCP_OK;
  PCP_HIP_TRY(ctx, ctx->labels.ensure(static_cast<size_t>(ctx->n) + 4));
  PCP_HIP_TRY(ctx, hipMemsetAsync(ctx->labels.p + ctx->n, 0, 4, ctx->stream));
  return PCP_OK;
}

static int labels_end(pcp_context *ctx) {
  if (!ctx->label_fusion) return PCP_OK;
  uint32_t bad = 0;
  uint32_t *dst = ctx->readback ? static_cast<uint32_t *>(ctx->readback) : &bad;
  PCP_HIP_TRY(ctx, hipMemcpyAsync(dst, ctx->labels.p + ctx->n, 4, hipMemcpyDeviceToHost, ctx->stream));
  PCP_HIP_TRY(ctx, hipStreamSynchronize(ctx->stream));
  if (*dst != 0)
    return set_error(ctx, PCP_ERR_RANGE, "label fusion: a view score outside [2^-3, 2) reached the label arithmetic "
                     "(final_score cannot produce one): no labels for this result");
  ctx->labels_live = true;
  return PCP_OK;
}

static int check_masks(pcp_context *ctx, int32_t frame_begin, int32_t frame_end) {
  if (!ctx->label_fusion) return PCP_OK;
  for (int32_t f = frame_begin; f < frame_end; ++f)
    if (static_cast<size_t>(f) >= ctx->mask_set.size() || !ctx->mask_set[static_cast<size_t>(f)])
      return set_error(ctx, PCP_ERR_STATE, "pcp_colour_pass: label fusion is on and no mask was uploaded for keyframe %d", f);
  return PCP_OK;
}

static int colour_pass_impl(pcp_context *ctx, int32_t frame_begin, int32_t frame_end, bool one_shot,
                            uint32_t *result = nullptr) {
  int rc = check_ready(ctx, "pcp_colour_pass", true);
  if (rc != PCP_OK) return rc;
  if (frame_begin < 0 || frame_end > ctx->n_frames || frame_begin > frame_end)
    return set_error(ctx, PCP_ERR_RANGE, "pcp_colour_pass: keyframe range [%d,%d) outside 0..%d", frame_begin, frame_end,
                     ctx->n_frames);
  if ((rc = check_masks(ctx, frame_begin, frame_end)) != PCP_OK) return rc;
  for (int32_t f = frame_begin; f < frame_end; ++f) {
    if (!ctx->depth.p || !ctx->depth_valid[static_cast<size_t>(f)])
      return set_error(ctx, PCP_ERR_STATE, "pcp_colour_pass: pcp_depth_pass has not covered keyframe %d", f);
    if (!ctx->images.p || !ctx->image_set[static_cast<size_t>(f)])
      return set_error(ctx, PCP_ERR_STATE, "pcp_colour_pass: no image uploaded for keyframe %d", f);
    if (ctx->cull.cull_mode == PCP_CULL_HPR && ctx->depth_from_batch &&
        (static_cast<size_t>(f) >= ctx->hull_valid.size() || !ctx->hull_valid[static_cast<size_t>(f)]))
      return set_error(ctx, PCP_ERR_STATE, "pcp_colour_pass: PCP_CULL_HPR on an index shard, pcp_hull_flags_import has not covered keyframe %d", f);
  }
  const bool radius = ctx->dcam.match_mode == PCP_MATCH_RADIUS;
  if (radius && ctx->depth_from_batch)
    return set_error(ctx, PCP_ERR_STATE, "pcp_colour_pass: PCP_MATCH_RADIUS needs the whole map on one context: an index shard "
                     "(PCP_DEPTH_BATCHED) cannot see the neighbours that other shards hold");
  if ((rc = ensure_state(ctx)) != PCP_OK) return rc;
  if ((rc = wait_images(ctx, frame_begin, frame_end)) != PCP_OK) return rc;
  if (ctx->n == 0) return PCP_OK;
  if (radius && (rc = match_table_prepare(ctx)) != PCP_OK) return rc;
  if (frame_begin == frame_end) {
    if (one_shot && result) PCP_HIP_TRY(ctx, hipMemsetAsync(result, 0, static_cast<size_t>(ctx->n) * 4, ctx->stream));
    if (one_shot && ctx->label_fusion)
      PCP_HIP_TRY(ctx, hipMemsetAsync(ctx->labels.p, 0, static_cast<size_t>(ctx->n) * 4, ctx->stream));
    return PCP_OK;
  }
  const size_t plane = plane_of(ctx);
  TopState st{ctx->top_score.p, ctx->top_rgb.p, ctx->top_frame.p, ctx->view_count.p};
  int32_t flags = 0;
  if (ctx->colour_state_live) flags |= 1;
  if (one_shot)
    flags |= 4;
  else
    flags |= 2;
  MatchArgs mb{nullptr, nullptr, 0.0f};
  if (radius) {
// ... 80 lines not shown
    if ((rc = finalise_gained(ctx, result)) != PCP_OK) return rc;
  } else if (n > 0) {
    TopState st{ctx->top_score.p, ctx->top_rgb.p, ctx->top_frame.p, ctx->view_count.p};
    LaunchTimer t(ctx, PCP_K_COLOUR);
    const bool label = ctx->label_fusion;
    const LabelOut lab{label ? ctx->labels.p : nullptr};
    if (label)
      hipLaunchKernelGGL(k_finalise_labels, dim3(blocks_for(n)), dim3(kBlock), 0, ctx->stream, n, st, ctx->perm.p, result, lab);
    else
      hipLaunchKernelGGL(k_finalise, dim3(blocks_for(n)), dim3(kBlock), 0, ctx->stream, n, st, ctx->perm.p, result);
    PCP_HIP_TRY(ctx, hipGetLastError());
  }
  if ((rc = labels_end(ctx)) != PCP_OK) return rc;
  if ((rc = end_result(ctx, out_rgb, out_has)) != PCP_OK) return rc;
  if ((out_count || out_top_score || out_top_rgb || out_top_frame) && n > 0) {
    std::vector<int32_t> perm(sn), cnt;
    std::vector<uint32_t> tmp(kTopM * sn);
    PCP_HIP_TRY(ctx, hipMemcpyAsync(perm.data(), ctx->perm.p, sn * 4, hipMemcpyDeviceToHost, ctx->stream));
    auto fetch5 = [&](const void *src, void *dst_v) -> int {
      PCP_HIP_TRY(ctx, hipMemcpyAsync(tmp.data(), src, kTopM * sn * 4, hipMemcpyDeviceToHost, ctx->stream));
      PCP_HIP_TRY(ctx, hipStreamSynchronize(ctx->stream));
      uint32_t *dst = static_cast<uint32_t *>(dst_v);
      for (size_t j = 0; j < sn; ++j)
        for (int k = 0; k < kTopM; ++k) dst[static_cast<size_t>(perm[j]) * kTopM + k] = tmp[static_cast<size_t>(k) * sn + j];
      return PCP_OK;
    };
    if (out_top_score && (rc = fetch5(ctx->top_score.p, out_top_score)) != PCP_OK) return rc;
    if (out_top_rgb && (rc = fetch5(ctx->top_rgb.p, out_top_rgb)) != PCP_OK) return rc;
    if (out_top_rgb && ctx->label_fusion)
      for (size_t k = 0; k < kTopM * sn; ++k) out_top_rgb[k] &= 0xffffffu;
    if (out_top_frame && (rc = fetch5(ctx->top_frame.p, out_top_frame)) != PCP_OK) return rc;
    if (out_count) {
      cnt.resize(sn);
      PCP_HIP_TRY(ctx, hipMemcpyAsync(cnt.data(), ctx->view_count.p, sn * 4, hipMemcpyDeviceToHost, ctx->stream));
      PCP_HIP_TRY(ctx, hipStreamSynchronize(ctx->stream));
      for (size_t j = 0; j < sn; ++j) out_count[perm[j]] = cnt[j];
    }
  }
  return PCP_OK;
}

static int refuse_gains(pcp_context *ctx, const char *who) {
  if (!ctx->gains_set) return PCP_OK;
  return set_error(ctx, PCP_ERR_STATE, "%s: exposure gains are set (pcp_set_frame_gains): they apply to pcp_colour_reset / "
                   "pcp_colour_pass / pcp_colour_finalise; clear them with pcp_set_frame_gains(NULL) for the one-shot call", who);
}

int pcp_colorize(pcp_context *ctx, uint8_t *out_rgb, uint8_t *out_has) {
  int rc = check_ready(ctx, "pcp_colorize", true);
  if (rc != PCP_OK) return rc;
  if ((rc = refuse_gains(ctx, "pcp_colorize")) != PCP_OK) return rc;
  if ((rc = check_masks(ctx, 0, ctx->n_frames)) != PCP_OK) return rc;
  pcp_colour_reset(ctx);
  if ((rc = pcp_depth_pass(ctx, 0, ctx->n_frames)) != PCP_OK) return rc;
  uint32_t *result = nullptr;
  if ((rc = begin_result(ctx, &result)) != PCP_OK) return rc;
  if ((rc = labels_begin(ctx)) != PCP_OK) return rc;
  if ((rc = colour_pass_impl(ctx, 0, ctx->n_frames, true, result)) != PCP_OK) return rc;
  if ((rc = labels_end(ctx)) != PCP_OK) return rc;
  return end_result(ctx, out_rgb, out_has);
}

int pcp_colorize_from_depth(pcp_context *ctx, uint8_t *out_rgb, uint8_t *out_has) {
  int rc = check_ready(ctx, "pcp_colorize_from_depth", true);
  if (rc != PCP_OK) return rc;
  if ((rc = refuse_gains(ctx, "pcp_colorize_from_depth")) != PCP_OK) return rc;
  pcp_colour_reset(ctx);
  uint32_t *result = nullptr;
  if ((rc = begin_result(ctx, &result)) != PCP_OK) return rc;
  if ((rc = labels_begin(ctx)) != PCP_OK) return rc;
  if ((rc = colour_pass_impl(ctx, 0, ctx->n_frames, true, result)) != PCP_OK) return rc;
  if ((rc = labels_end(ctx)) != PCP_OK) return rc;
  return end_result(ctx, out_rgb, out_has);
}

int pcp_colour_smooth_local(pcp_context *ctx, float radius, int64_t *out_has_count) {
  if (!ctx) return PCP_ERR_INVALID;
  if (!smooth_radius_ok(radius))
    return set_error(ctx, PCP_ERR_INVALID, "pcp_colour_smooth_local: radius %g outside (0, 1]", static_cast<double>(radius));
  if (!ctx->colour_result_live)
    return set_error(ctx, PCP_ERR_STATE, "pcp_colour_smooth_local: no result (call pcp_colorize / pcp_colour_finalise)");
  if (out_has_count) *out_has_count = 0;
  if (ctx->n == 0) return PCP_OK;
  PCP_HIP_TRY(ctx, hipSetDevice(ctx->device));
  const uint32_t *src = ctx->rgba2[ctx->rgba_cur].p;
  uint32_t *dst = nullptr;
  int rc = begin_result(ctx, &dst);
  if (rc != PCP_OK) return rc;
  if ((rc = colour_smooth_words(ctx, radius, src, dst, out_has_count)) != PCP_OK) return rc;
  return end_result(ctx, nullptr, nullptr);
}

int pcp_download_result_packed(pcp_context *ctx, uint32_t *out_rgba) {
  if (!ctx) return PCP_ERR_INVALID;
  if (!ctx->colour_result_live)
    return set_error(ctx, PCP_ERR_STATE, "pcp_download_result_packed: no result (call pcp_colorize / pcp_colour_finalise)");
  if (!out_rgba && ctx->n > 0) return set_error(ctx, PCP_ERR_INVALID, "pcp_download_result_packed: NULL output");
  if (ctx->n > 0)
    PCP_HIP_TRY(ctx, hipMemcpyAsync(out_rgba, ctx->rgba2[ctx->rgba_cur].p, static_cast<size_t>(ctx->n) * 4,
                                    hipMemcpyDeviceToHost, ctx->stream));
  PCP_HIP_TRY(ctx, hipStreamSynchronize(ctx->stream));
  return PCP_OK;
}

int pcp_download_result_packed_async(pcp_context *ctx, uint32_t *out_rgba) {
  if (!ctx) return PCP_ERR_INVALID;
  if (!ctx->colour_result_live)
    return set_error(ctx, PCP_ERR_STATE, "pcp_download_result_packed_async: no result (call pcp_colorize / pcp_colour_finalise)");
  if (!out_rgba && ctx->n > 0) return set_error(ctx, PCP_ERR_INVALID, "pcp_download_result_packed_async: NULL output");
  const int32_t cur = ctx->rgba_cur;
  PCP_HIP_TRY(ctx, hipStreamWaitEvent(ctx->copy_stream, ctx->result_ready[cur], 0));
  if (ctx->n > 0)
    PCP_HIP_TRY(ctx, hipMemcpyAsync(out_rgba, ctx->rgba2[cur].p, static_cast<size_t>(ctx->n) * 4, hipMemcpyDeviceToHost,
                                    ctx->copy_stream));
  PCP_HIP_TRY(ctx, hipEventRecord(ctx->copy_done[cur], ctx->copy_stream));
  ctx->copy_pending[cur] = true;
  return PCP_OK;
}

int pcp_download_wait_previous(pcp_context *ctx) {
  if (!ctx) return PCP_ERR_INVALID;
  const int32_t prev = ctx->rgba_cur ^ 1;
  if (ctx->copy_pending[prev]) PCP_HIP_TRY(ctx, hipEventSynchronize(ctx->copy_done[prev]));
  return PCP_OK;
}

int pcp_tile_mask_density(pcp_context *ctx, double *kept_fraction) {
  if (!ctx || !kept_fraction) return PCP_ERR_INVALID;
  if (!ctx->tile_mask.p || ctx->n_tiles == 0 || ctx->n_frames == 0)
    return set_error(ctx, PCP_ERR_STATE, "pcp_tile_mask_density: no masks (call pcp_depth_pass)");
  std::vector<uint32_t> h(static_cast<size_t>(ctx->n_tiles) * ctx->mask_words);
  PCP_HIP_TRY(ctx, hipMemcpyAsync(h.data(), ctx->tile_mask.p, h.size() * 4, hipMemcpyDeviceToHost, ctx->stream));
  PCP_HIP_TRY(ctx, hipStreamSynchronize(ctx->stream));
  uint64_t bits = 0;
  for (uint32_t w : h) bits += static_cast<uint64_t>(__builtin_popcount(w));
  *kept_fraction = static_cast<double>(bits) / (static_cast<double>(ctx->n_tiles) * ctx->n_frames);
  return PCP_OK;
}

int pcp_tile_masks(pcp_context *ctx, int64_t *tiles, int32_t *mask_words, uint32_t *out_words) {
  if (!ctx) return PCP_ERR_INVALID;
  if (!ctx->tile_mask.p || ctx->n_tiles == 0 || ctx->n_frames == 0)
    return set_error(ctx, PCP_ERR_STATE, "pcp_tile_masks: no masks (call pcp_depth_pass)");
  if (tiles) *tiles = ctx->n_tiles;
  if (mask_words) *mask_words = ctx->mask_words;
  if (out_words) {
    PCP_HIP_TRY(ctx, hipMemcpyAsync(out_words, ctx->tile_mask.p, static_cast<size_t>(ctx->n_tiles) * ctx->mask_words * 4,
                                    hipMemcpyDeviceToHost, ctx->stream));
    PCP_HIP_TRY(ctx, hipStreamSynchronize(ctx->stream));
  }
  return PCP_OK;
}

int pcp_colour_result_device(pcp_context *ctx, void **device_ptr, int64_t *n_words) {
  if (!ctx) return PCP_ERR_INVALID;
  if (!ctx->colour_result_live)
    return set_error(ctx, PCP_ERR_STATE, "pcp_colour_result_device: no result (call pcp_colorize / pcp_colour_finalise)");
  if (device_ptr) *device_ptr = ctx->rgba2[ctx->rgba_cur].p;
  if (n_words) *n_words = ctx->n;
  return PCP_OK;
}

int pcp_set_label_fusion(pcp_context *ctx, int32_t enable) {
  if (!ctx) return PCP_ERR_INVALID;
  const bool on = enable != 0;
  if (on != ctx->label_fusion && ctx->colour_state_live)
    return set_error(ctx, PCP_ERR_STATE, "pcp_set_label_fusion: a top-5 accumulation is live (its lists %s the masks): "
                     "call pcp_colour_reset first", ctx->label_fusion ? "hold" : "do not hold");
  ctx->label_fusion = on;
  return PCP_OK;
}

int pcp_colour_labels(pcp_context *ctx, uint8_t *out_label, uint8_t *out_hits, uint8_t *out_views) {
  if (!ctx) return PCP_ERR_INVALID;
  if (!ctx->labels_live)
    return set_error(ctx, PCP_ERR_STATE, "pcp_colour_labels: no labels (pcp_set_label_fusion(1), then pcp_colorize / "
                     "pcp_colorize_from_depth / pcp_colour_finalise)");
  const int64_t n = ctx->n;
  if (n == 0 || !(out_label || out_hits || out_views)) return PCP_OK;
  PCP_HIP_TRY(ctx, hipSetDevice(ctx->device));
  const size_t sn = static_cast<size_t>(n);
  PCP_HIP_TRY(ctx, ctx->s_keep.ensure(4 * sn + 16));
  uint8_t *d_label = ctx->s_keep.p, *d_hits = d_label + sn, *d_views = d_hits + sn;
  hipLaunchKernelGGL(k_unpack_labels, dim3(blocks_for(n)), dim3(kBlock), 0, ctx->stream, ctx->labels.p, n,
                     out_label ? d_label : nullptr, out_hits ? d_hits : nullptr, out_views ? d_views : nullptr);
  PCP_HIP_TRY(ctx, hipGetLastError());
  if (out_label) PCP_HIP_TRY(ctx, hipMemcpyAsync(out_label, d_label, sn, hipMemcpyDeviceToHost, ctx->stream));
  if (out_hits) PCP_HIP_TRY(ctx, hipMemcpyAsync(out_hits, d_hits, sn, hipMemcpyDeviceToHost, ctx->stream));
  if (out_views) PCP_HIP_TRY(ctx, hipMemcpyAsync(out_views, d_views, sn, hipMemcpyDeviceToHost, ctx->stream));
  PCP_HIP_TRY(ctx, hipStreamSynchronize(ctx->stream));
  return PCP_OK;
}

int pcp_colour_labels_device(pcp_context *ctx, void **device_ptr, int64_t *n_words) {
  if (!ctx) return PCP_ERR_INVALID;
  if (!ctx->labels_live)
    return set_error(ctx, PCP_ERR_STATE, "pcp_colour_labels_device: no labels (pcp_set_label_fusion(1), then pcp_colorize / "
                     "pcp_colorize_from_depth / pcp_colour_finalise)");
  if (device_ptr) *device_ptr = ctx->labels.p;
  if (n_words) *n_words = ctx->n;
  return PCP_OK;
}

int pcp_selftest_arithmetic(pcp_context *ctx, int64_t samples, uint64_t seed, int64_t *mismatches_fp64,
                            int64_t *mismatches_fp32) {
  if (!ctx) return PCP_ERR_INVALID;
  if (!ctx->have_camera) return set_error(ctx, PCP_ERR_STATE, "pcp_selftest_arithmetic: pcp_set_camera has not been called");
  PCP_HIP_TRY(ctx, hipSetDevice(ctx->device));
  if (samples < 0) return set_error(ctx, PCP_ERR_INVALID, "pcp_selftest_arithmetic: negative sample count");
  PCP_HIP_TRY(ctx, ctx->s_counter.ensure(4));
  unsigned long long *bad = ctx->s_counter.p;
  PCP_HIP_TRY(ctx, hipMemsetAsync(bad, 0, 16, ctx->stream));
  if (samples > 0)
    hipLaunchKernelGGL(k_selftest_div64, dim3(blocks_for(samples)), dim3(kBlock), 0, ctx->stream, samples, seed, bad);
  hipLaunchKernelGGL(k_selftest_div32, dim3((1u << 24) / kBlock), dim3(kBlock), 0, ctx->stream, ctx->dcam, bad + 1);
  PCP_HIP_TRY(ctx, hipGetLastError());
  unsigned long long h[2] = {0, 0};
  PCP_HIP_TRY(ctx, hipMemcpyAsync(h, bad, 16, hipMemcpyDeviceToHost, ctx->stream));
  PCP_HIP_TRY(ctx, hipStreamSynchronize(ctx->stream));
  if (mismatches_fp64) *mismatches_fp64 = static_cast<int64_t>(h[0]);
  if (mismatches_fp32) *mismatches_fp32 = static_cast<int64_t>(h[1]);
  return PCP_OK;
}

int pcp_selftest_visit_forms(pcp_context *ctx, int64_t samples, uint64_t seed, int64_t *mismatches_uv, int64_t *mismatches_cell,
                             int64_t *mismatches_sqrt, int32_t *short_distortion) {
  if (!ctx) return PCP_ERR_INVALID;
  if (!ctx->have_camera) return set_error(ctx, PCP_ERR_STATE, "pcp_selftest_visit_forms: pcp_set_camera has not been called");
  PCP_HIP_TRY(ctx, hipSetDevice(ctx->device));
  if (samples < 0) return set_error(ctx, PCP_ERR_INVALID, "pcp_selftest_visit_forms: negative sample count");
  PCP_HIP_TRY(ctx, ctx->s_counter.ensure(4));
  unsigned long long *bad = ctx->s_counter.p;
  PCP_HIP_TRY(ctx, hipMemsetAsync(bad, 0, 32, ctx->stream));
  if (samples > 0)
    hipLaunchKernelGGL(k_selftest_uv, dim3(blocks_for(samples)), dim3(kBlock), 0, ctx->stream, ctx->dcam, ctx->uv_tame ? 1 : 0, samples, seed, bad);
  hipLaunchKernelGGL(k_selftest_cell_sqrt, dim3((1u << 24) / kBlock), dim3(kBlock), 0, ctx->stream, ctx->dcam, bad + 1, bad + 2);
  PCP_HIP_TRY(ctx, hipGetLastError());
  unsigned long long h[3] = {0, 0, 0};
  PCP_HIP_TRY(ctx, hipMemcpyAsync(h, bad, 24, hipMemcpyDeviceToHost, ctx->stream));
  PCP_HIP_TRY(ctx, hipStreamSynchronize(ctx->stream));
  if (mismatches_uv) *mismatches_uv = static_cast<int64_t>(h[0]);
  if (mismatches_cell) *mismatches_cell = static_cast<int64_t>(h[1]);
  if (mismatches_sqrt) *mismatches_sqrt = static_cast<int64_t>(h[2]);
  if (short_distortion) *short_distortion = ctx->uv_tame ? 1 : 0;
  return PCP_OK;
}

}
```

### pointcloudprocessor_amd/csrc/pcp_context.hip

```cpp
#include <algorithm>
#include <cfloat>
#include <cmath>
#include <cstdlib>
#include <new>
#include <vector>

#include "pcp_internal.hpp"
#include "pcp_visit_forms.hpp"
#include "pcp_scan.hpp"

namespace pcp {

static thread_local std::string g_error;

int set_error(const pcp_context *ctx, int code, const char *fmt, ...) {
  char buf[1024];
  va_list ap;
  va_start(ap, fmt);
  vsnprintf(buf, sizeof(buf), fmt, ap);
  va_end(ap);
  if (ctx)
    ctx->error = buf;
  else
    g_error = buf;
// ... 686 lines not shown
  ctx->v_plane.release();
  ctx->v_vox.release();
  ctx->v_offsets.release();
  ctx->mls_xyz.release();
  ctx->mls_normal.release();
  ctx->mls_curv.release();
  ctx->mls_index.release();
  ctx->mls_alt_xyz.release();
  ctx->mls_alt_normal.release();
  ctx->mls_alt_curv.release();
  ctx->mls_alt_index.release();
  if (ctx->readback) (void)hipHostFree(ctx->readback);
  if (ctx->own_stream) (void)hipStreamDestroy(ctx->own_stream);
  delete ctx;
}

const char *pcp_last_error(const pcp_context *ctx) { return ctx ? ctx->error.c_str() : g_error.c_str(); }

int pcp_set_stream(pcp_context *ctx, void *hip_stream) {
  if (!ctx) return PCP_ERR_INVALID;
  PCP_HIP_TRY(ctx, hipStreamSynchronize(ctx->stream));
  ctx->stream = hip_stream ? static_cast<hipStream_t>(hip_stream) : ctx->own_stream;
  return PCP_OK;
}

int pcp_synchronize(pcp_context *ctx) {
  if (!ctx) return PCP_ERR_INVALID;
  for (hipStream_t us : ctx->upload_stream)
    if (us) PCP_HIP_TRY(ctx, hipStreamSynchronize(us));
  std::fill(ctx->image_pending.begin(), ctx->image_pending.end(), uint8_t(0));
  PCP_HIP_TRY(ctx, hipStreamSynchronize(ctx->stream));
  PCP_HIP_TRY(ctx, hipStreamSynchronize(ctx->copy_stream));
  ctx->copy_pending[0] = ctx->copy_pending[1] = false;
  return PCP_OK;
}

void pcp_default_camera(pcp_camera *cam) {
  cam->fx = 4818.200388954926;
  cam->fy = 4819.10345841615;
  cam->cx = 2032.4178620390019;
  cam->cy = 1535.1895959282901;
  cam->k1 = 0.003043514741045163;
  cam->k2 = 0.06634739187544138;
  cam->p1 = -0.000217681797407554;
  cam->p2 = -0.0006654964142658197;
  cam->k3 = 0.0;
  cam->image_width = 4096;
  cam->image_height = 3000;
  cam->cull_width = 4096;
  cam->cull_height = 3000;
}

void pcp_default_cull_params(pcp_cull_params *p) {
  p->enable_depth_buffer_culling = 1;
  p->downsample_factor = 14;
  p->depth_slack = 0.05;
  p->cull_mode = PCP_CULL_ZBUFFER;
  p->match_mode = PCP_MATCH_ROUNDTRIP;
  p->hpr_flip_radius = 90000.0;
}

void pcp_default_mls_params(pcp_mls_params *p) {
  p->search_radius = 0.03;
  p->sqr_gauss_param = 0.0009;
  p->polynomial_order = 2;
  p->compute_normals = 1;
  p->upsampling = 3;
  p->vgd_iterations = 4;
  p->vgd_voxel_size = 0.001f;
  p->sor_mean_k = 60;
  p->sor_std_mul = 0.7;
}

int pcp_set_camera(pcp_context *ctx, const pcp_camera *cam, const pcp_cull_params *cull) {
  if (!ctx || !cam) return set_error(ctx, PCP_ERR_INVALID, "pcp_set_camera: NULL argument");
  pcp_cull_params cp;
  if (cull)
    cp = *cull;
  else
    pcp_default_cull_params(&cp);
  if (cam->image_width <= 0 || cam->image_height <= 0 || cam->cull_width <= 0 || cam->cull_height <= 0)
    return set_error(ctx, PCP_ERR_INVALID, "pcp_set_camera: image / cull size must be positive");
  if (cp.downsample_factor <= 0) return set_error(ctx, PCP_ERR_INVALID, "pcp_set_camera: downsample_factor must be > 0");
  if (cp.cull_mode != PCP_CULL_ZBUFFER && cp.cull_mode != PCP_CULL_HPR_CANDIDATES && cp.cull_mode != PCP_CULL_HPR)
    return set_error(ctx, PCP_ERR_INVALID, "pcp_set_camera: unknown cull_mode %d", cp.cull_mode);
  if (cp.cull_mode == PCP_CULL_HPR && !(cp.hpr_flip_radius > 0.0 && cp.hpr_flip_radius < 1e300))
    return set_error(ctx, PCP_ERR_INVALID, "pcp_set_camera: hpr_flip_radius must be positive and finite");
  if (cp.match_mode != PCP_MATCH_IDENTITY && cp.match_mode != PCP_MATCH_ROUNDTRIP && cp.match_mode != PCP_MATCH_RADIUS)
    return set_error(ctx, PCP_ERR_INVALID, "pcp_set_camera: unknown match_mode %d", cp.match_mode);
  if (cam->cull_width > (1 << 24) || cam->cull_height > (1 << 24))
    return set_error(ctx, PCP_ERR_INVALID, "pcp_set_camera: cull size above 2^24 is not supported");
  if (static_cast<int64_t>(cam->image_width) * cam->image_height >= (int64_t(1) << 31))
    return set_error(ctx, PCP_ERR_INVALID, "pcp_set_camera: image too large for int32 pixel indices");
  ctx->camera = *cam;
  ctx->cull = cp;
  DevCamera &d = ctx->dcam;
  d.fx = cam->fx;
  d.fy = cam->fy;
  d.cx = cam->cx;
  d.cy = cam->cy;
  d.k1 = cam->k1;
  d.k2 = cam->k2;
  d.p1 = cam->p1;
  d.p2 = cam->p2;
  d.k3 = cam->k3;
  d.slack = cp.depth_slack;
  d.ds = cp.downsample_factor;
  d.ds_f = static_cast<float>(cp.downsample_factor);
  d.ds_rcp = 1.0f / d.ds_f;
  d.ds_fast = (d.ds_f >= 0x1p-20f && d.ds_f <= 0x1p20f) ? 1 : 0;
  if (const char *e = std::getenv("PCP_DISABLE_FAST_EXACT")) d.ds_fast = (e[0] == '1') ? 0 : d.ds_fast;
  d.img_w = cam->image_width;
  d.img_h = cam->image_height;
  d.cull_w = cam->cull_width;
  d.cull_h = cam->cull_height;
  d.img_wd = static_cast<double>(cam->image_width);
  d.img_hd = static_cast<double>(cam->image_height);
  d.cull_wf = static_cast<float>(cam->cull_width);
  d.cull_hf = static_cast<float>(cam->cull_height);
  d.mw = cam->cull_width / cp.downsample_factor;
  d.mh = cam->cull_height / cp.downsample_factor;
  ctx->uv_tame = vf::distortion_is_tame(cam->p1, cam->p2);
  if (const char *e = std::getenv("PCP_DISABLE_FAST_EXACT")) ctx->uv_tame = (e[0] == '1') ? false : ctx->uv_tame;
  d.cull_mode = cp.cull_mode == PCP_CULL_HPR ? PCP_CULL_HPR_CANDIDATES : cp.cull_mode;
  d.match_mode = cp.match_mode;
  d.cull_wd = static_cast<double>(cam->cull_width);
  d.cull_hd = static_cast<double>(cam->cull_height);
  {
    const double eps = static_cast<double>(1e-5f);
    d.match_r2 = static_cast<float>(eps * eps);
  }
  d.enable_zbuf = (cp.enable_depth_buffer_culling && cp.cull_mode == PCP_CULL_ZBUFFER) ? 1 : 0;
  d.pretest = 1;
  d.qfx = static_cast<float>(cam->fx);
  d.qfy = static_cast<float>(cam->fy);
  d.qcx = static_cast<float>(cam->cx);
  d.qcy = static_cast<float>(cam->cy);
  d.qk1 = static_cast<float>(cam->k1);
  d.qk2 = static_cast<float>(cam->k2);
  d.qk3 = static_cast<float>(cam->k3);
  d.qp1 = static_cast<float>(cam->p1);
  d.qp2 = static_cast<float>(cam->p2);
  {
    const float ds = static_cast<float>(cp.downsample_factor);
    const bool hpr = cp.cull_mode != PCP_CULL_ZBUFFER;
    const float cw = hpr ? static_cast<float>(d.cull_w) : ds * static_cast<float>(d.enable_zbuf ? d.mw : d.cull_w);
    const float ch = hpr ? static_cast<float>(d.cull_h) : ds * static_cast<float>(d.enable_zbuf ? d.mh : d.cull_h);
    d.u_lo = -(ds + 0.5f);
    d.v_lo = -(ds + 0.5f);
    d.u_hi = std::max(cw, static_cast<float>(d.img_w)) + 0.5f;
    d.v_hi = std::max(ch, static_cast<float>(d.img_h)) + 0.5f;
  }
  if (const char *e = std::getenv("PCP_DISABLE_PRETEST")) d.pretest = (e[0] == '1') ? 0 : 1;

  ctx->have_camera = true;
  for (hipStream_t us : ctx->upload_stream)
    if (us) (void)hipStreamSynchronize(us);
  std::fill(ctx->image_pending.begin(), ctx->image_pending.end(), uint8_t(0));
  ctx->image_set.assign(ctx->image_set.size(), 0);
  ctx->mask_set.assign(ctx->mask_set.size(), 0);
  std::fill(ctx->depth_valid.begin(), ctx->depth_valid.end(), uint8_t(0));
  ctx->hull_valid.clear();
  ctx->depth_accum.release();
  ctx->depth_accum_live = false;
  ctx->colour_state_live = false;
  ctx->colour_result_live = false;
  ctx->labels_live = false;
  return PCP_OK;
}

int pcp_upload_cloud(pcp_context *ctx, const float *x, const float *y, const float *z, int64_t n) {
  if (!ctx) return PCP_ERR_INVALID;
  if (n < 0 || n >= (int64_t(1) << 31)) return set_error(ctx, PCP_ERR_INVALID, "pcp_upload_cloud: n=%lld out of range", (long long)n);
  if (n > 0 && (!x || !y || !z)) return set_error(ctx, PCP_ERR_INVALID, "pcp_upload_cloud: NULL coordinate array");
  return store_cloud(ctx, x, y, z, n);
}

int pcp_upload_cloud_aos(pcp_context *ctx, const void *points, int64_t n, int64_t stride_bytes) {
  if (!ctx) return PCP_ERR_INVALID;
  if (n < 0 || n >= (int64_t(1) << 31)) return set_error(ctx, PCP_ERR_INVALID, "pcp_upload_cloud_aos: n out of range");
  if (stride_bytes < 12) return set_error(ctx, PCP_ERR_INVALID, "pcp_upload_cloud_aos: stride must be >= 12 bytes");
  if (n > 0 && !points) return set_error(ctx, PCP_ERR_INVALID, "pcp_upload_cloud_aos: NULL points");
  if (stride_bytes % 4 == 0 && (reinterpret_cast<uintptr_t>(points) & 3u) == 0)
    return store_cloud(ctx, nullptr, nullptr, nullptr, n, points, stride_bytes);
  std::vector<float> x(static_cast<size_t>(n)), y(static_cast<size_t>(n)), z(static_cast<size_t>(n));
  const uint8_t *base = static_cast<const uint8_t *>(points);
  for (int64_t i = 0; i < n; ++i) {
    float v[3];
    std::memcpy(v, base + i * stride_bytes, 12);
    x[static_cast<size_t>(i)] = v[0];
    y[static_cast<size_t>(i)] = v[1];
    z[static_cast<size_t>(i)] = v[2];
  }
  return store_cloud(ctx, x.data(), y.data(), z.data(), n);
}

int pcp_upload_cloud_from_result(pcp_context *dst, pcp_context *src, int64_t *out_n) {
  if (!dst || !src) return dst ? set_error(dst, PCP_ERR_INVALID, "pcp_upload_cloud_from_result: NULL source context") : PCP_ERR_INVALID;
  if (out_n) *out_n = 0;
  if (dst->device != src->device)
    return set_error(dst, PCP_ERR_INVALID, "pcp_upload_cloud_from_result: the contexts are on GPUs %d and %d (one GPU only)", dst->device,
                     src->device);
  if (!src->mls_result_live)
    return set_error(dst, PCP_ERR_STATE, "pcp_upload_cloud_from_result: the source context holds no smoothing result (pcp_mls_process*, "
                     "pcp_cloud_smooth, pcp_mls_stream_next, pcp_cloud_smooth_stream_next since its latest upload)");
  const int64_t m = src->mls_count;
  const float *rows = src->mls_xyz.p;
  if (m > 0 && !rows) return set_error(dst, PCP_ERR_STATE, "pcp_upload_cloud_from_result: the source result has no rows on the device");
  PCP_HIP_TRY(dst, hipSetDevice(dst->device));
  if (dst != src && m > 0) {
    if (!src->handoff) PCP_HIP_TRY(dst, hipEventCreateWithFlags(&src->handoff, hipEventDisableTiming));
    PCP_HIP_TRY(dst, hipEventRecord(src->handoff, src->stream));
    PCP_HIP_TRY(dst, hipStreamWaitEvent(dst->stream, src->handoff, 0));
  }
  const int rc = store_cloud(dst, nullptr, nullptr, nullptr, m, rows, 12, true, dst == src);
  if (rc == PCP_OK && out_n) *out_n = m;
  return rc;
}

int64_t pcp_cloud_size(const pcp_context *ctx) { return ctx ? ctx->n : -1; }

int pcp_pose_to_matrices(const pcp_pose *pose, const double *T_opt, float w2c[12], float c2w[12]) {
  if (!pose || !w2c || !c2w) {
    set_global_error("pcp_pose_to_matrices: NULL argument");
    return PCP_ERR_INVALID;
  }
  matrices_from_pose(*pose, T_opt, w2c, c2w);
  return PCP_OK;
}

int pcp_set_frames(pcp_context *ctx, const pcp_pose *poses, int32_t n_frames, const double *T_opt,
                   int32_t T_opt_stride) {
  if (!ctx) return PCP_ERR_INVALID;
  if (n_frames < 0 || (n_frames > 0 && !poses)) return set_error(ctx, PCP_ERR_INVALID, "pcp_set_frames: bad poses");
  if (T_opt && T_opt_stride != 0 && T_opt_stride != 16)
    return set_error(ctx, PCP_ERR_INVALID, "pcp_set_frames: T_opt_stride must be 0 (global) or 16 (per keyframe)");
  PCP_HIP_TRY(ctx, hipSetDevice(ctx->device));
  for (hipStream_t us : ctx->upload_stream)
    if (us) PCP_HIP_TRY(ctx, hipStreamSynchronize(us));
  std::fill(ctx->image_pending.begin(), ctx->image_pending.end(), uint8_t(0));
  ctx->poses.assign(poses, poses + n_frames);
  ctx->hframes.resize(static_cast<size_t>(n_frames));
  for (int32_t f = 0; f < n_frames; ++f) {
    DevFrame &d = ctx->hframes[static_cast<size_t>(f)];
    const double *T = T_opt ? T_opt + static_cast<int64_t>(T_opt_stride) * f : nullptr;
    matrices_from_pose(poses[f], T, d.w2c, d.c2w);
    invert_affine_f32(d.c2w, d.c2w_inv);
    d.pad_[0] = d.pad_[1] = d.pad_[2] = d.pad_[3] = 0.0f;
    d.px = poses[f].x;
    d.py = poses[f].y;
    d.pz = poses[f].z;
    {
      double g[3][3];
      for (int a = 0; a < 3; ++a)
        for (int b = 0; b < 3; ++b) {
          g[a][b] = 0.0;
          for (int k = 0; k < 3; ++k) g[a][b] += static_cast<double>(d.w2c[4 * k + a]) * static_cast<double>(d.w2c[4 * k + b]);
        }
      double rowmax = 0.0;
      for (int a = 0; a < 3; ++a) rowmax = std::max(rowmax, std::fabs(g[a][0]) + std::fabs(g[a][1]) + std::fabs(g[a][2]));
      d.norm_bound = std::sqrt(rowmax) * (1.0 + 1e-9);
    }
  }
  {
    bool bounded = true;
    for (int32_t f = 0; f < n_frames; ++f)
      for (int k = 0; k < 12; ++k) bounded = bounded && std::fabs(ctx->hframes[static_cast<size_t>(f)].w2c[k]) <= 0x1p40f;
    ctx->dcam.frames_bounded = bounded ? 1 : 0;
  }
  PCP_HIP_TRY(ctx, ctx->frames.ensure(static_cast<size_t>(n_frames) + 1));
  if (n_frames > 0)
    PCP_HIP_TRY(ctx, hipMemcpyAsync(ctx->frames.p, ctx->hframes.data(), sizeof(DevFrame) * n_frames,
                                    hipMemcpyHostToDevice, ctx->stream));
  PCP_HIP_TRY(ctx, hipStreamSynchronize(ctx->stream));
  ctx->n_frames = n_frames;
  ctx->image_set.assign(static_cast<size_t>(n_frames), 0);
  ctx->mask_set.assign(static_cast<size_t>(n_frames), 0);
  ctx->depth_valid.assign(static_cast<size_t>(n_frames), 0);
  ctx->hull_valid.clear();
  ctx->depth_accum.release();
  ctx->depth_accum_live = false;
  ctx->match_live = false;
  ctx->gains_set = false;
  ctx->colour_state_live = false;
  ctx->colour_result_live = false;
  ctx->labels_live = false;
  return PCP_OK;
}

int32_t pcp_frame_count(const pcp_context *ctx) { return ctx ? ctx->n_frames : -1; }

int pcp_timing_enable(pcp_context *ctx, int32_t on) {
  if (!ctx) return PCP_ERR_INVALID;
  PCP_HIP_TRY(ctx, hipStreamSynchronize(ctx->stream));
  drain_timing(ctx);
  ctx->timing = on != 0;
  return PCP_OK;
}

int pcp_timing_reset(pcp_context *ctx) {
  if (!ctx) return PCP_ERR_INVALID;
  PCP_HIP_TRY(ctx, hipStreamSynchronize(ctx->stream));
  drain_timing(ctx);
  for (auto &s : ctx->slots) s = TimingSlot{};
  return PCP_OK;
}
// ... 20 lines not shown
```

### pointcloudprocessor_amd/csrc/pcp_internal.hpp

```cpp
#pragma once

#include <hip/hip_runtime.h>

#include <cstdarg>
#include <cstdint>
#include <chrono>
#include <cstdio>
#include <cstring>
#include <string>
#include <vector>

#include "pcp_hip.h"

namespace pcp {

struct DevCamera {
  double fx, fy, cx, cy;
  double k1, k2, p1, p2, k3;
  double slack;
  float ds_f;
  double img_wd, img_hd;
  float cull_wf, cull_hf;
  float ds_rcp;
  int32_t ds_fast;
  int32_t ds;
  int32_t img_w, img_h;
  int32_t cull_w, cull_h;
  int32_t mw, mh;
  int32_t enable_zbuf;
  int32_t cull_mode;
  int32_t match_mode;
  double cull_wd, cull_hd;
  float match_r2;
  int32_t pretest;
  int32_t frames_bounded;
  float qfx, qfy, qcx, qcy;
  float qk1, qk2, qk3, qp1, qp2;
  float u_lo, u_hi, v_lo, v_hi;
};

struct DevFrame {
  float w2c[12];
  float c2w[12];
  double px, py, pz;
  double norm_bound;
  float c2w_inv[12];
  float pad_[4];
};
static_assert(sizeof(DevFrame) == 192, "DevFrame layout");

constexpr int kTopM = 5;

struct TimingSlot {
  double total_ms = 0.0;
  int64_t launches = 0;
};

struct PendingEvent {
  hipEvent_t start, stop;
  int32_t kernel;
};

struct AllocTally {
  double seconds = 0.0, bytes = 0.0;
};
inline AllocTally &alloc_tally() {
  static AllocTally t;
  return t;
}
struct AllocClock {
  std::chrono::steady_clock::time_point t0 = std::chrono::steady_clock::now();
  ~AllocClock() { alloc_tally().seconds += std::chrono::duration<double>(std::chrono::steady_clock::now() - t0).count(); }
};

template <typename T>
struct DevBuf {
  T *p = nullptr;
  size_t count = 0;
  hipError_t ensure(size_t n) {
    if (n <= count && p) return hipSuccess;
    AllocClock clk;
    if (p) (void)hipFree(p);
    p = nullptr;
    count = 0;
    if (n == 0) return hipSuccess;
    hipError_t e = hipMalloc(reinterpret_cast<void **>(&p), n * sizeof(T));
    if (e == hipSuccess) {
      count = n;
      alloc_tally().bytes += static_cast<double>(n) * sizeof(T);
    }
    return e;
  }
  void release() {
    if (!p) return;
    AllocClock clk;
    (void)hipFree(p);
    p = nullptr;
    count = 0;
  }
};

struct AsciiParseSlot {
  void *stage = nullptr, *res_h = nullptr;
  size_t stage_bytes = 0;
  DevBuf<uint8_t> text;
  DevBuf<int32_t> end, tiles;
  DevBuf<uint32_t> out;
  DevBuf<unsigned long long> res;
  hipEvent_t staged = nullptr, parsed = nullptr, drained = nullptr;
  bool staged_live = false, parsed_live = false, drained_live = false;
};

struct HprLane {
  hipStream_t own_stream = nullptr;
  hipStream_t stream = nullptr;
  unsigned long long seq = 0;
  DevBuf<int32_t> index, i32, tiles;
  DevBuf<double> f64, cells_d, cont;
  DevBuf<uint8_t> state;
  DevBuf<unsigned long long> stats;
  void *readback = nullptr;
  bool busy = false;
  int32_t frame = -1;
  uint8_t *d_flags = nullptr;
  uint32_t *hull_plane = nullptr;
  uint32_t bit = 0;
  void release() {
    index.release();
    i32.release();
    tiles.release();
    f64.release();
    cells_d.release();
    cont.release();
    state.release();
    stats.release();
    if (readback) (void)hipHostFree(readback);
    readback = nullptr;
    if (own_stream) (void)hipStreamDestroy(own_stream);
    own_stream = nullptr;
  }
};

struct VoxelReduce {
  bool live = false, finished = false;
  bool labels_fixed = false, with_label = false;
  float leaf = 0.0f;
  int64_t initial_slots = 0;
  int64_t slots = 0, used = 0;
  int64_t keyed = 0;
  int64_t rows = 0, voxels = 0, growths = 0, partials = 0, atomics = 0;
  DevBuf<unsigned long long> keys, q, scalars;
  DevBuf<uint32_t> sums;
  DevBuf<float> out_xyz;
  DevBuf<uint8_t> out_rgb, out_label;
  DevBuf<uint32_t> out_count;
};

}

struct pcp_context {
  int32_t device = 0;
  hipStream_t own_stream = nullptr;
  hipStream_t stream = nullptr;
  void *readback = nullptr;
  static constexpr size_t kReadbackBytes = 65536;
  mutable std::string error;

  bool have_camera = false;
  bool uv_tame = false;
  pcp_camera camera{};
  pcp_cull_params cull{};
  pcp::DevCamera dcam{};

  int64_t n = 0;
  int64_t nonfinite_points = 0;
  pcp::DevBuf<float> xyz;
  pcp::DevBuf<float> sxyz;
  pcp::DevBuf<int32_t> perm;
  pcp::DevBuf<int32_t> inv_perm;
  std::vector<float> host_min = {0, 0, 0}, host_max = {0, 0, 0};

  int32_t n_frames = 0;
  std::vector<pcp_pose> poses;
  std::vector<pcp::DevFrame> hframes;
  pcp::DevBuf<pcp::DevFrame> frames;
  pcp::DevBuf<uint32_t> images;
  std::vector<uint8_t> image_set, mask_set;
  static constexpr int kUploadLanes = 2;
  hipStream_t upload_stream[kUploadLanes] = {nullptr, nullptr};
  pcp::DevBuf<uint8_t> upload_stage[kUploadLanes];
  pcp::DevBuf<uint8_t> jpeg_planes[kUploadLanes];
  std::vector<hipEvent_t> image_event;
  std::vector<uint8_t> image_pending;
  std::vector<uint8_t> image_lane;
  std::vector<uint64_t> image_seq;
  bool lane_must_wait[kUploadLanes] = {false, false};
  uint64_t upload_seq = 0;
  uint64_t upload_turn = 0;
  hipEvent_t texels_idle = nullptr;
  bool texels_touched = false;
  bool adjust_images = false;
  float saturation_scale = 1.0f, brightness_scale = 1.0f;
  pcp::DevBuf<int32_t> hsv_tables;

  pcp::DevBuf<uint32_t> depth;
  pcp::DevBuf<unsigned long long> depth_sq;
  std::vector<uint8_t> depth_valid;
  bool depth_from_batch = false;
  pcp::DevBuf<uint32_t> depth_accum;
  bool depth_accum_live = false;

  int64_t n_tiles = 0;
  pcp::DevBuf<float> tile_sphere;
  pcp::DevBuf<uint32_t> tile_mask, group_mask;
  pcp::DevBuf<uint32_t> tile_inside;
  int32_t mask_words = 0;
  pcp::DevBuf<int32_t> tile_work, tile_order, work_hist;
  bool tile_order_live = false;

  pcp::DevBuf<float> top_score;
  pcp::DevBuf<uint32_t> top_rgb;
  pcp::DevBuf<int32_t> top_frame;
  pcp::DevBuf<int32_t> view_count;
  pcp::DevBuf<uint32_t> rgba2[2];
  int32_t rgba_cur = 0;
  hipStream_t copy_stream = nullptr;
  hipEvent_t result_ready[2] = {nullptr, nullptr}, copy_done[2] = {nullptr, nullptr};
  bool copy_pending[2] = {false, false};
  bool colour_state_live = false;
  bool colour_result_live = false;
  bool label_fusion = false;
  bool labels_live = false;
  pcp::DevBuf<uint32_t> labels;
  bool gains_set = false;
  pcp::DevBuf<float> gains_dev;
  pcp::DevBuf<unsigned long long> pair_stats;
  int64_t pair_counters[5] = {0, 0, 0, 0, 0};
  bool pair_counters_live = false;

  pcp::VoxelReduce voxel_reduce;

  bool gn_live = false;
  float gn_radius = 0.0f;
  pcp::DevBuf<float> gn_normal;
  pcp::DevBuf<int32_t> gn_count;
  pcp::DevBuf<unsigned long long> gm_keys;
  pcp::DevBuf<uint32_t> gm_out;

  bool match_live = false;
  double match_e = 0.0, match_rc = 0.0;
  float match_e2 = 0.0f;
  int64_t match_a = 0;
  int64_t match_entries = 0;
  pcp::DevBuf<uint8_t> match_in_a;
  pcp::DevBuf<int32_t> match_list;
  pcp::DevBuf<int64_t> match_off;
  pcp::DevBuf<int32_t> match_cols;
  pcp::DevBuf<unsigned long long> match_moved;

  pcp::DevBuf<int32_t> s_cell, s_pixel;
  pcp::DevBuf<float> s_range, s_cam;
  pcp::DevBuf<uint8_t> s_keep;
  pcp::DevBuf<uint32_t> s_u32;
  pcp::DevBuf<unsigned long long> s_counter;
  pcp::DevBuf<int32_t> s_tiles;

  static constexpr int kHprMaxLanes = 8;
  pcp::HprLane hpr_lane[kHprMaxLanes];
  int32_t hpr_last_lane = 0;
  hipEvent_t hpr_fork = nullptr, hpr_join[kHprMaxLanes] = {};
  pcp::DevBuf<uint32_t> hull_bits;
  std::vector<uint8_t> hull_valid;
  int64_t hpr_stats[10] = {0, 0, 0, 0, 0, 0, 0, 0, 0, 0};
  bool hpr_stats_pending = false;

  pcp::DevBuf<int32_t> g_cell, g_rank, g_start, g_order;
  pcp::DevBuf<unsigned long long> g_occ;
  pcp::DevBuf<int32_t> g_occ_rank;
  pcp::DevBuf<float> g_xyz;
  pcp::DevBuf<float> m_tmp;
  pcp::DevBuf<float> s_dist;
  pcp::DevBuf<double> m_state;
  double slp_radius = 0.05, slp_step = 0.01;
  pcp::DevBuf<float> slp_table;
  double slp_table_of[2] = {0.0, 0.0};
  pcp::DevBuf<int32_t> c_perm;
  pcp::DevBuf<uint8_t> m_flag;
  pcp::DevBuf<double> m_sums;
  pcp::DevBuf<int32_t> c_index;
  int32_t sor_partial_slab = -1, sor_partial_slabs = -1;
  bool sor_distances_live = false;
  pcp::DevBuf<uint8_t> c_mark;
  pcp::DevBuf<int32_t> c_where;
  pcp::DevBuf<float> c_xyz, c_xyz2;
  pcp::DevBuf<uint32_t> v_bitmap;
  pcp::DevBuf<int32_t> v_offsets;
  pcp::DevBuf<uint32_t> v_occ;
  pcp::DevBuf<int32_t> v_rank;
  pcp::DevBuf<unsigned long long> v_plane;
  pcp::DevBuf<int64_t> v_vox;
  pcp::DevBuf<float> mls_xyz, mls_normal, mls_curv;
  pcp::DevBuf<int32_t> mls_index;
  pcp::DevBuf<float> mls_alt_xyz, mls_alt_normal, mls_alt_curv;
  pcp::DevBuf<int32_t> mls_alt_index;
  int64_t mls_count = 0;
  bool mls_result_live = false;
  hipEvent_t handoff = nullptr;
  pcp::DevBuf<uint8_t> cc_out;
  pcp::DevBuf<uint8_t> ascii_in, ascii_len, ascii_text;
  pcp::DevBuf<unsigned long long> ascii_tiles;
  pcp::AsciiParseSlot parse_slot[2];
  hipStream_t parse_up = nullptr, parse_down = nullptr;
  std::vector<uint8_t> vgd_blob;
  std::vector<int64_t> vgd_chunks;
  int64_t vgd_next = -1;
  std::vector<uint8_t> css_blob;
  std::vector<int64_t> css_chunks;
  int64_t css_next = -1;
  pcp::DevBuf<float> css_dist;
  pcp::DevBuf<float> s_kth;
  pcp::DevBuf<uint32_t> css_words;
  bool css_building = false;
  double css_ball = 0.0;
  double sor_redo_fraction = 0.0;

// ... 125 lines not shown
```

### pointcloudprocessor_amd/host_build.py

```python
from __future__ import annotations

import os
import subprocess

from . import _build

HOST = os.path.join(os.path.dirname(os.path.abspath(__file__)), "host")
BIN = os.path.join(HOST, "bin")
ROCM = os.environ.get("ROCM_PATH", "/opt/rocm")

TARGETS = {
    "pcp_shim_selftest": ["shim_selftest.cpp"],
    "PointCloudProcessor": ["main.cpp"],
    "image_dump": ["image_dump.cpp"],
    "format_selftest": ["format_selftest.cpp"],
    "parse_selftest": ["parse_selftest.cpp"],
    "visit_forms_selftest": ["visit_forms_selftest.cpp"],
    "voxel_reduce_selftest": ["voxel_reduce_selftest.cpp"],
    "normals_selftest": ["normals_selftest.cpp"],
}


def build(force: bool = False) -> dict:
    os.makedirs(BIN, exist_ok=True)
    out = {}
    for name, srcs in TARGETS.items():
        exe = os.path.join(BIN, name)
        deps = [os.path.join(HOST, s) for s in srcs] + [os.path.join(HOST, "pcp_shim.hpp"), os.path.join(HOST, "pcp_multi.hpp"), os.path.join(HOST, "pcd_io.hpp"), os.path.join(HOST, "image_io.hpp"), os.path.join(HOST, "pcd_device_reader.hpp"),
                                                       os.path.join(_build.CSRC, "pcp_ascii_parse.hpp"), os.path.join(_build.CSRC, "pcp_ascii.hpp"), os.path.join(_build.CSRC, "pcp_visit_forms.hpp"), os.path.join(_build.CSRC, "pcp_voxel_reduce.hpp"), os.path.join(_build.CSRC, "pcp_normals.hpp"),
                                                       os.path.join(_build.INCLUDE, "pcp_hip.h")]
        deps = [d for d in deps if os.path.exists(d)]
        stale = force or not os.path.exists(exe) or any(os.path.getmtime(d) > os.path.getmtime(exe) for d in deps)
        if stale:
            extra = os.environ.get("PCP_HOST_CXXFLAGS", "").split()
            multi = ["-D__HIP_PLATFORM_AMD__", "-isystem", os.path.join(ROCM, "include")] if name == "PointCloudProcessor" else []
            multi_libs = ["-L", os.path.join(ROCM, "lib"), "-lrccl", "-lamdhip64", "-Wl,-rpath," + os.path.join(ROCM, "lib")] \
                if name == "PointCloudProcessor" else []
            cmd = ["g++", "-std=c++17", "-O2", "-ffp-contract=off", "-pthread", "-Wall", "-Wextra"] + extra + multi + ["-I", _build.INCLUDE, "-I", HOST] + [
                os.path.join(HOST, s) for s in srcs] + ["-L", _build.LIB_DIR, "-lpcp_hip"] + multi_libs + [
                                                        "-lz", "-Wl,-rpath,$ORIGIN/../../lib", "-o", exe]
            proc = subprocess.run(cmd, capture_output=True, text=True)
            if proc.returncode != 0:
                raise RuntimeError(f"g++ failed for {name}:\n{proc.stderr[-3000:]}")
        out[name] = exe
    return out
```

Measured before the change: 1.940 million.

## Add interior tile classification to skip per-point cull checks in depth pass

Extends tile/frame classification with a third "interior" class, proven by interval arithmetic to keep the whole tile sphere inside the depth map with a margin. For those pairs the depth visit loop takes a shortened path that projects each point and computes its cell with a cheaper form, skipping per-point in-frame and candidate checks. The change also adds an interior mask buffer, selftests and a profiling script. It adds classification work and extra mask traffic, and its correctness depends on the interval bound and the short distortion form agreeing with the reference cell.

```diff
diff --git a/include/pcp_hip.h b/include/pcp_hip.h
--- a/include/pcp_hip.h
+++ b/include/pcp_hip.h
@@ -263,12 +263,16 @@
 const char *pcp_kernel_name(int32_t kernel_id);
 int pcp_tile_mask_density(pcp_context *ctx, double *kept_fraction);
 int pcp_tile_masks(pcp_context *ctx, int64_t *tiles, int32_t *mask_words, uint32_t *out_words);
+int pcp_tile_interior_masks(pcp_context *ctx, int64_t *tiles, int32_t *mask_words, uint32_t *out_words);
+int pcp_cloud_order(pcp_context *ctx, int64_t capacity, int32_t *out_index);
 int pcp_sor_redo_fraction(pcp_context *ctx, double *fraction);
 int pcp_sor_distances(pcp_context *ctx, int64_t capacity, float *out_distance);
 int pcp_selftest_arithmetic(pcp_context *ctx, int64_t samples, uint64_t seed, int64_t *mismatches_fp64,
                             int64_t *mismatches_fp32);
 int pcp_selftest_visit_forms(pcp_context *ctx, int64_t samples, uint64_t seed, int64_t *mismatches_uv, int64_t *mismatches_cell,
                              int64_t *mismatches_sqrt, int32_t *short_distortion);
+int pcp_selftest_depth_visits(pcp_context *ctx, int64_t samples, uint64_t seed, int64_t *interior_tiles, int64_t *points_checked,
+                              int64_t *mismatches, int32_t *interior_form);
 
 #ifdef __cplusplus
 }
diff --git a/pointcloudprocessor_amd/_build.py b/pointcloudprocessor_amd/_build.py
--- a/pointcloudprocessor_amd/_build.py
+++ b/pointcloudprocessor_amd/_build.py
@@ -12,7 +12,7 @@
 
 SOURCES = ["pcp_context.hip", "pcp_colour.hip", "pcp_mls.hip", "pcp_nid.hip", "pcp_hpr.hip", "pcp_colour_smooth.hip", "pcp_match.hip", "pcp_jpeg.hip",
            "pcp_stream_colour.hip", "pcp_ascii.hip", "pcp_ascii_parse.hip", "pcp_exposure.hip", "pcp_voxel_reduce.hip", "pcp_normals.hip"]
-HEADERS = ["pcp_internal.hpp", "pcp_device.hpp", "pcp_scan.hpp", "pcp_hsv.hpp", "pcp_exact.hpp", "pcp_ascii.hpp", "pcp_ascii_parse.hpp", "pcp_visit_forms.hpp", "pcp_voxel_reduce.hpp", "pcp_eigen33.hpp", "pcp_normals.hpp"]
+HEADERS = ["pcp_internal.hpp", "pcp_device.hpp", "pcp_scan.hpp", "pcp_hsv.hpp", "pcp_exact.hpp", "pcp_ascii.hpp", "pcp_ascii_parse.hpp", "pcp_visit_forms.hpp", "pcp_depth_visit.hpp", "pcp_voxel_reduce.hpp", "pcp_eigen33.hpp", "pcp_normals.hpp"]
 
 HIPCC_FLAGS = [
     "--offload-arch=gfx950",
diff --git a/pointcloudprocessor_amd/capi.py b/pointcloudprocessor_amd/capi.py
--- a/pointcloudprocessor_amd/capi.py
+++ b/pointcloudprocessor_amd/capi.py
@@ -956,6 +956,12 @@
                                                       C.byref(f)))
         return a.value, b.value, c.value, bool(f.value)
 
+    def selftest_depth_visits(self, samples: int = 1 << 24, seed: int = 1):
+        a, b, c, f = C.c_int64(), C.c_int64(), C.c_int64(), C.c_int32()
+        self._check(self.lib.pcp_selftest_depth_visits(self.h, C.c_int64(samples), C.c_uint64(seed), C.byref(a), C.byref(b), C.byref(c),
+                                                       C.byref(f)))
+        return a.value, b.value, c.value, bool(f.value)
+
     def tile_masks(self) -> np.ndarray:
         t, w = C.c_int64(), C.c_int32()
         self._check(self.lib.pcp_tile_masks(self.h, C.byref(t), C.byref(w), None))
@@ -963,5 +969,17 @@
         self._check(self.lib.pcp_tile_masks(self.h, None, None, _ptr(out)))
         return out
 
+    def tile_interior_masks(self) -> np.ndarray:
+        t, w = C.c_int64(), C.c_int32()
+        self._check(self.lib.pcp_tile_interior_masks(self.h, C.byref(t), C.byref(w), None))
+        out = np.empty((t.value, w.value), np.uint32)
+        self._check(self.lib.pcp_tile_interior_masks(self.h, None, None, _ptr(out)))
+        return out
+
+    def cloud_order(self) -> np.ndarray:
+        out = np.empty(self.n, np.int32)
+        self._check(self.lib.pcp_cloud_order(self.h, C.c_int64(self.n), _ptr(out)))
+        return out
+
     def kernel_name(self, kernel_id: int) -> str:
         return self.lib.pcp_kernel_name(C.c_int32(kernel_id)).decode()
diff --git a/pointcloudprocessor_amd/csrc/pcp_colour.hip b/pointcloudprocessor_amd/csrc/pcp_colour.hip
--- a/pointcloudprocessor_amd/csrc/pcp_colour.hip
+++ b/pointcloudprocessor_amd/csrc/pcp_colour.hip
@@ -2,6 +2,7 @@
 #include <cfloat>
 #include <cstdlib>
 
+#include "pcp_depth_visit.hpp"
 #include "pcp_device.hpp"
 #include "pcp_hsv.hpp"
 #include "pcp_scan.hpp"
@@ -99,38 +100,9 @@
   }
 }
 
-struct Interval {
-  double lo, hi;
-};
-__device__ __forceinline__ Interval iv_add(Interval a, Interval b) { return {a.lo + b.lo, a.hi + b.hi}; }
-__device__ __forceinline__ Interval iv_scale(double k, Interval a) {
-  return k >= 0.0 ? Interval{k * a.lo, k * a.hi} : Interval{k * a.hi, k * a.lo};
-}
-__device__ __forceinline__ Interval iv_mul(Interval a, Interval b) {
-  const double p0 = a.lo * b.lo, p1 = a.lo * b.hi, p2 = a.hi * b.lo, p3 = a.hi * b.hi;
-  return {fmin(fmin(p0, p1), fmin(p2, p3)), fmax(fmax(p0, p1), fmax(p2, p3))};
-}
-__device__ __forceinline__ Interval iv_sqr(Interval a) {
-  const double l = fabs(a.lo), h = fabs(a.hi);
-  const double mx = fmax(l, h), mn = (a.lo <= 0.0 && a.hi >= 0.0) ? 0.0 : fmin(l, h);
-  return {mn * mn, mx * mx};
-}
-__device__ __forceinline__ Interval iv_mul_pos(Interval a, Interval b) { return {a.lo * b.lo, a.hi * b.hi}; }
-__device__ __forceinline__ Interval iv_mul_by_pos(Interval a, Interval b) {
-  return {a.lo * (a.lo >= 0.0 ? b.lo : b.hi), a.hi * (a.hi >= 0.0 ? b.hi : b.lo)};
-}
-__device__ __forceinline__ double iv_rcp_pos(double b) {
-  double r = __builtin_amdgcn_rcp(b);
-  r = fma(fma(-b, r, 1.0), r, r);
-  r = fma(fma(-b, r, 1.0), r, r);
-  return r;
-}
-__device__ __forceinline__ Interval iv_pad(Interval a) {
-  const double e = 1e-12 * (fabs(a.lo) + fabs(a.hi)) + 1e-300;
-  return {a.lo - e, a.hi + e};
-}
-
-__device__ __forceinline__ int tile_classify(const DevCamera &c, const DevFrame &fr, float4 sph) {
+using dv::Interval;
+
+__device__ __forceinline__ int tile_classify(const DevCamera &c, const dv::InteriorBox &ib, const DevFrame &fr, float4 sph) {
   const double cx = sph.x, cy = sph.y, cz = sph.z;
   const float *m = fr.w2c;
   const double X = (m[0] * cx + m[1] * cy) + (m[2] * cz + m[3]);
@@ -142,34 +114,18 @@
   if (!(rho >= 0.0) || !isfinite(X + Y + Z + rho)) return 0;
   if (Z + rho <= 0.0) return 1;
   if (Z - rho <= 0.0) return 0;
-  const Interval zi{Z - rho, Z + rho};
-  if (!(zi.lo >= 1e-290)) return 0;
-  const Interval iz{iv_rcp_pos(zi.hi) * (1.0 - 1e-13), iv_rcp_pos(zi.lo) * (1.0 + 1e-13)};
-  const Interval xn = iv_pad(iv_mul_by_pos(Interval{X - rho, X + rho}, iz));
-  const Interval yn = iv_pad(iv_mul_by_pos(Interval{Y - rho, Y + rho}, iz));
-  const Interval x2 = iv_sqr(xn), y2 = iv_sqr(yn);
-  const Interval r2 = iv_add(x2, y2);
-  const Interval r4 = iv_mul_pos(r2, r2);
-  const Interval r6 = iv_mul_pos(r2, r4);
-  Interval rc = iv_add(iv_add(iv_scale(c.k1, r2), iv_scale(c.k2, r4)), iv_scale(c.k3, r6));
-  rc.lo += 1.0;
-  rc.hi += 1.0;
-  const Interval t1 = iv_scale(2.0, iv_mul(xn, yn));
-  const Interval t2 = iv_add(r2, iv_scale(2.0, x2));
-  const Interval t3 = iv_add(r2, iv_scale(2.0, y2));
-  const Interval xd = iv_pad(iv_add(iv_add(iv_mul(rc, xn), iv_scale(c.p1, t1)), iv_scale(c.p2, t2)));
-  const Interval yd = iv_pad(iv_add(iv_add(iv_mul(rc, yn), iv_scale(c.p1, t3)), iv_scale(c.p2, t1)));
-  Interval u = iv_pad(iv_scale(c.fx, xd)), v = iv_pad(iv_scale(c.fy, yd));
-  u.lo += c.cx; u.hi += c.cx;
-  v.lo += c.cy; v.hi += c.cy;
+  if (!(Z - rho >= 1e-290)) return 0;
+  Interval xn, yn, u, v;
+  dv::interval_normalised(X, Y, Z, rho, xn, yn);
+  dv::interval_image(c, xn, yn, u, v);
   if (!isfinite(u.lo + u.hi + v.lo + v.hi)) return 0;
   if (u.hi < static_cast<double>(c.u_lo) || u.lo > static_cast<double>(c.u_hi) ||
       v.hi < static_cast<double>(c.v_lo) || v.lo > static_cast<double>(c.v_hi))
     return 1;
-  return (u.lo > static_cast<double>(c.u_lo) + 1.0 && u.hi < static_cast<double>(c.u_hi) - 1.0 &&
-          v.lo > static_cast<double>(c.v_lo) + 1.0 && v.hi < static_cast<double>(c.v_hi) - 1.0)
-             ? 2
-             : 0;
+  if (!(u.lo > static_cast<double>(c.u_lo) + 1.0 && u.hi < static_cast<double>(c.u_hi) - 1.0 &&
+        v.lo > static_cast<double>(c.v_lo) + 1.0 && v.hi < static_cast<double>(c.v_hi) - 1.0))
+    return 0;
+  return dv::interior_pair(ib, xn, yn, u, v) ? 3 : 2;
 }
 
 constexpr int kTileGroup = 16;
@@ -178,9 +134,11 @@
                                                             const DevFrame *__restrict__ frames, int32_t n_frames,
                                                             int32_t w0, int32_t w1, int32_t words,
                                                             uint32_t *__restrict__ group_mask,
-                                                            uint32_t *__restrict__ group_inside, int32_t cull_enabled,
+                                                            uint32_t *__restrict__ group_inside,
+                                                            uint32_t *__restrict__ group_interior, int32_t cull_enabled,
                                                             int32_t *__restrict__ zeroed, int32_t n_zeroed,
-                                                            unsigned long long *__restrict__ far_maps, int64_t far_cells) {
+                                                            unsigned long long *__restrict__ far_maps, int64_t far_cells,
+                                                            dv::InteriorBox ib) {
   const int64_t idx = static_cast<int64_t>(blockIdx.x) * kBlock + threadIdx.x;
   if (idx < n_zeroed) zeroed[idx] = 0;
   for (int64_t c = idx; c < far_cells; c += static_cast<int64_t>(gridDim.x) * kBlock) far_maps[c] = 0x7f7f7f7f7f7f7f7full;
@@ -191,11 +149,12 @@
   const int32_t w = w0 + static_cast<int32_t>(gw - group * nw);
   const int32_t f = (w << 5) + static_cast<int32_t>(idx & 31);
   int cls = 1;
-  if (live && f < n_frames) cls = cull_enabled ? tile_classify(cam, frames[f], spheres[group]) : 0;
-  const unsigned long long m = __ballot(cls != 1), in = __ballot(cls == 2);
+  if (live && f < n_frames) cls = cull_enabled ? tile_classify(cam, ib, frames[f], spheres[group]) : 0;
+  const unsigned long long m = __ballot(cls != 1), in = __ballot(cls >= 2), deep = __ballot(cls == 3);
   if (live && (idx & 31) == 0) {
     group_mask[group * words + w] = static_cast<uint32_t>((threadIdx.x & 32) ? (m >> 32) : m);
     group_inside[group * words + w] = static_cast<uint32_t>((threadIdx.x & 32) ? (in >> 32) : in);
+    group_interior[group * words + w] = static_cast<uint32_t>((threadIdx.x & 32) ? (deep >> 32) : deep);
   }
 }
 
@@ -204,8 +163,10 @@
                                                             int32_t n_frames, int32_t w0, int32_t w1, int32_t words,
                                                             const uint32_t *__restrict__ group_mask,
                                                             const uint32_t *__restrict__ group_inside,
+                                                            const uint32_t *__restrict__ group_interior,
                                                             uint32_t *__restrict__ tile_mask,
-                                                            uint32_t *__restrict__ inside_mask, int32_t cull_enabled) {
+                                                            uint32_t *__restrict__ inside_mask, int32_t interior_bits,
+                                                            int32_t cull_enabled, dv::InteriorBox ib) {
   const int lane = threadIdx.x & 63;
   const int32_t nw = w1 - w0;
   const int64_t gw = static_cast<int64_t>(blockIdx.x) * (kBlock / 64) + (threadIdx.x >> 6);
@@ -219,8 +180,9 @@
   const int32_t nb = n_frames - (w << 5);
   if (nb < 32) todo &= nb <= 0 ? 0u : ((1u << nb) - 1u);
   const uint32_t whole = __builtin_amdgcn_readfirstlane(group_inside[group * words + w]) & todo;
-  todo &= ~whole;
-  uint32_t word = whole, inside = whole;
+  const uint32_t settled = interior_bits ? __builtin_amdgcn_readfirstlane(group_interior[group * words + w]) & whole : whole;
+  todo &= ~settled;
+  uint32_t word = whole, inside = settled;
   if (todo) {
     const float4 sph = spheres[have ? tile : tiles - 1];
     while (todo) {
@@ -232,8 +194,8 @@
       }
       const int32_t b = slot == 0 ? bit[0] : slot == 1 ? bit[1] : slot == 2 ? bit[2] : bit[3];
       int cls = 1;
-      if (b >= 0 && have) cls = cull_enabled ? tile_classify(cam, frames[(w << 5) + b], sph) : 0;
-      const unsigned long long keep = __ballot(cls != 1), ins = __ballot(cls == 2);
+      if (b >= 0 && have) cls = cull_enabled ? tile_classify(cam, ib, frames[(w << 5) + b], sph) : 0;
+      const unsigned long long keep = __ballot(cls != 1), ins = __ballot(cls >= (interior_bits ? 3 : 2));
 #pragma unroll
       for (int k = 0; k < 4; ++k) {
         if (bit[k] >= 0) {
@@ -380,6 +342,46 @@
     todo = __builtin_amdgcn_readfirstlane(todo);
     const uint32_t inside = tile_inside ? __builtin_amdgcn_readfirstlane(tile_inside[tile * words + w]) : 0u;
     uint32_t seen = 0u;
+    auto to_map = [&](int32_t f, bool in_map, int32_t cell, float xc, float yc, float zc) {
+      unsigned long long *map = depth + static_cast<uint64_t>(static_cast<uint32_t>(f - depth_first_frame)) * static_cast<uint32_t>(cells);
+      unsigned long long key = ~0ull, sbits = 0ull;
+      if (in_map) {
+        sbits = static_cast<unsigned long long>(__double_as_longlong(sumsq64(xc, yc, zc)));
+        key = (static_cast<unsigned long long>(static_cast<uint32_t>(cell)) << 32) | (sbits >> 32);
+      }
+      tbl[lane] = ~0ull;
+      __builtin_amdgcn_wave_barrier();
+      if (in_map) atomicMin(&tbl[cell & 63], key);
+      __builtin_amdgcn_wave_barrier();
+      if (in_map) {
+        const unsigned long long got = tbl[cell & 63];
+        if (got == key || static_cast<uint32_t>(got >> 32) != static_cast<uint32_t>(cell)) {
+          held_at = map + cell;
+          held_bits = sbits;
+          held_seen = *held_at;
+        }
+      }
+      __builtin_amdgcn_wave_barrier();
+    };
+    if constexpr (kCommon) {
+      uint32_t deep = todo & inside;
+      todo &= ~inside;
+      while (deep) {
+        const int32_t b = __builtin_ctz(deep);
+        const int32_t f = (w << 5) + b;
+        deep &= deep - 1u;
+        const DevFrame &fr = frames[f];
+        float xc, yc, zc;
+        xform(fr.w2c, px, py, pz, xc, yc, zc);
+        double u, v;
+        project_uv<true, true>(cam, xc, yc, zc, u, v, true);
+        const int32_t cell = dv::interior_cell(div_by_ds(cam, static_cast<float>(u)), div_by_ds(cam, static_cast<float>(v)), cam.mw);
+        seen |= 1u << b;
+        asm volatile("" : "+v"(held_seen) : "v"(cell));
+        settle_held();
+        to_map(f, live, cell, xc, yc, zc);
+      }
+    }
     while (todo) {
       const int32_t b = __builtin_ctz(todo);
       const int32_t f = (w << 5) + b;
@@ -396,27 +398,7 @@
       }
       if (__builtin_amdgcn_ballot_w64(cand)) seen |= 1u << b;
       settle_held();
-      if (cam.enable_zbuf && __builtin_amdgcn_ballot_w64(in_map)) {
-        unsigned long long *map = depth + static_cast<uint64_t>(static_cast<uint32_t>(f - depth_first_frame)) * static_cast<uint32_t>(cells);
-        unsigned long long key = ~0ull, sbits = 0ull;
-        if (in_map) {
-          sbits = static_cast<unsigned long long>(__double_as_longlong(sumsq64(p.xc, p.yc, p.zc)));
-          key = (static_cast<unsigned long long>(static_cast<uint32_t>(p.cell)) << 32) | (sbits >> 32);
-        }
-        tbl[lane] = ~0ull;
-        __builtin_amdgcn_wave_barrier();
-        if (in_map) atomicMin(&tbl[p.cell & 63], key);
-        __builtin_amdgcn_wave_barrier();
-        if (in_map) {
-          const unsigned long long got = tbl[p.cell & 63];
-          if (got == key || static_cast<uint32_t>(got >> 32) != static_cast<uint32_t>(p.cell)) {
-            held_at = map + p.cell;
-            held_bits = sbits;
-            held_seen = *held_at;
-          }
-        }
-        __builtin_amdgcn_wave_barrier();
-      }
+      if (cam.enable_zbuf && __builtin_amdgcn_ballot_w64(in_map)) to_map(f, in_map, p.cell, p.xc, p.yc, p.zc);
     }
     if (tile_mask && lane == 0 && live) {
       uint32_t *dst = tile_mask + tile * words + w;
@@ -770,6 +752,51 @@
   if (wrong_sqrt) atomicAdd(bad_sqrt, static_cast<unsigned long long>(wrong_sqrt));
 }
 
+constexpr int kSelftestPoints = 8;
+__global__ __launch_bounds__(kBlock) void k_selftest_interior(DevCamera cam_in, dv::InteriorBox ib, int64_t samples, uint64_t seed,
+                                                              unsigned long long *__restrict__ out) {
+  const DevCamera cam = common_camera<true>(cam_in);
+  const int64_t i = static_cast<int64_t>(blockIdx.x) * kBlock + threadIdx.x;
+  if (i >= samples) return;
+  uint64_t h = mix64(seed ^ static_cast<uint64_t>(i) * 5u);
+  auto unit = [&]() {
+    h = mix64(h);
+    return static_cast<float>(static_cast<uint32_t>(h >> 40)) * 0x1p-24f;
+  };
+  DevFrame fr = {};
+  const uint32_t perm = static_cast<uint32_t>(h % 3u), signs = static_cast<uint32_t>(h >> 8) & 7u;
+  for (int r = 0; r < 3; ++r) {
+    fr.w2c[4 * r + (r + perm) % 3] = ((signs >> r) & 1u) ? -1.0f : 1.0f;
+    fr.w2c[4 * r + 3] = (unit() - 0.5f) * 16.0f;
+  }
+  fr.norm_bound = 1.0;
+  const float d = exp2f(unit() * 9.0f - 3.0f), rad = d * exp2f(-2.0f - unit() * 10.0f);
+  const float u0 = (unit() * 1.4f - 0.2f) * static_cast<float>(cam.img_w), v0 = (unit() * 1.4f - 0.2f) * static_cast<float>(cam.img_h);
+  const float cc[3] = {(u0 - static_cast<float>(cam.cx)) / static_cast<float>(cam.fx) * d,
+                       (v0 - static_cast<float>(cam.cy)) / static_cast<float>(cam.fy) * d, d};
+  float wc[3];
+  for (int k = 0; k < 3; ++k) {
+    const int r = (k + 3 - static_cast<int>(perm)) % 3;
+    wc[k] = fr.w2c[4 * r + k] * (cc[r] - fr.w2c[4 * r + 3]);
+  }
+  if (tile_classify(cam, ib, fr, make_float4(wc[0], wc[1], wc[2], rad)) != 3) return;
+  uint32_t wrong = 0u;
+  for (int k = 0; k < kSelftestPoints; ++k) {
+    const float s = 0.9f * rad * 0.57735f;
+    const float x = wc[0] + s * (2.0f * unit() - 1.0f), y = wc[1] + s * (2.0f * unit() - 1.0f), z = wc[2] + s * (2.0f * unit() - 1.0f);
+    const Projected p = project_point<false, true>(cam, fr.w2c, x, y, z);
+    float xc, yc, zc;
+    xform(fr.w2c, x, y, z, xc, yc, zc);
+    double u, v;
+    project_uv<true, true>(cam, xc, yc, zc, u, v, true);
+    const int32_t cell = dv::interior_cell(div_by_ds(cam, static_cast<float>(u)), div_by_ds(cam, static_cast<float>(v)), cam.mw);
+    if (!(p.zc > 0.0f) || p.cell < 0 || p.pixel < 0 || cell != p.cell) ++wrong;
+  }
+  atomicAdd(out, 1ull);
+  atomicAdd(out + 1, static_cast<unsigned long long>(kSelftestPoints));
+  if (wrong) atomicAdd(out + 2, static_cast<unsigned long long>(wrong));
+}
+
 __global__ __launch_bounds__(kBlock) void k_unpack_result(const uint32_t *__restrict__ packed, int64_t n,
                                                          uint8_t *__restrict__ rgb, uint8_t *__restrict__ has) {
   const int64_t i = static_cast<int64_t>(blockIdx.x) * kBlock + threadIdx.x;
@@ -1673,6 +1700,7 @@
   if (ctx->n > 0) {
     const size_t plane = plane_of(ctx);
     const int32_t w0 = frame_begin >> 5, w1 = ((frame_end - 1) >> 5) + 1;
+    const bool common = is_common_camera(ctx);
     static const bool cull_tiles = [] {
       const char *e = std::getenv("PCP_DISABLE_TILE_CULL");
       return !(e && e[0] == '1');
@@ -1682,16 +1710,17 @@
       const int64_t groups = div_up(ctx->n_tiles, kTileGroup);
       const float4 *tile_sph = reinterpret_cast<const float4 *>(ctx->tile_sphere.p);
       const size_t gwords = static_cast<size_t>(groups) * ctx->mask_words;
-      PCP_HIP_TRY(ctx, ctx->group_mask.ensure(2 * gwords + 8));
-      uint32_t *group_inside = ctx->group_mask.p + gwords + 4;
+      PCP_HIP_TRY(ctx, ctx->group_mask.ensure(3 * gwords + 12));
+      uint32_t *group_inside = ctx->group_mask.p + gwords + 4, *group_interior = group_inside + gwords + 4;
       hipLaunchKernelGGL(k_group_mask_flat, dim3(std::max(blocks_for(groups * (w1 - w0) * 32), blocks_for(2 * kWorkBins))),
                          dim3(kBlock), 0, ctx->stream, tile_sph + ctx->n_tiles, groups, ctx->dcam, ctx->frames.p, ctx->n_frames,
-                         w0, w1, ctx->mask_words, ctx->group_mask.p, group_inside, cull_tiles ? 1 : 0, ctx->work_hist.p,
+                         w0, w1, ctx->mask_words, ctx->group_mask.p, group_inside, group_interior, cull_tiles ? 1 : 0, ctx->work_hist.p,
                          2 * kWorkBins, z_maps ? reinterpret_cast<unsigned long long *>(ctx->depth_sq.p) : nullptr,
-                         z_maps ? map_cells : int64_t(0));
+                         z_maps ? map_cells : int64_t(0), ctx->interior_box);
       hipLaunchKernelGGL(k_tile_mask_dense, dim3(static_cast<uint32_t>(div_up(groups * (w1 - w0), kBlock / 64))), dim3(kBlock),
                          0, ctx->stream, tile_sph, ctx->n_tiles, ctx->dcam, ctx->frames.p, ctx->n_frames, w0, w1,
-                         ctx->mask_words, ctx->group_mask.p, group_inside, ctx->tile_mask.p, ctx->tile_inside.p, cull_tiles ? 1 : 0);
+                         ctx->mask_words, ctx->group_mask.p, group_inside, group_interior, ctx->tile_mask.p, ctx->tile_inside.p,
+                         common ? 1 : 0, cull_tiles ? 1 : 0, ctx->interior_box);
       if ((rc = sort_tiles_by_work(ctx, w0, w1, ctx->tile_order.p)) != PCP_OK) return rc;
       ctx->tile_order_live = true;
     }
@@ -1720,10 +1749,15 @@
     }
     {
       LaunchTimer t(ctx, PCP_K_DEPTH);
-      hipLaunchKernelGGL(is_common_camera(ctx) ? k_depth_pass<true> : k_depth_pass<false>,
+      static const bool plain_visits = [] {
+        const char *e = std::getenv("PCP_DEPTH_PLAIN_VISITS");
+        return e && e[0] == '1';
+      }();
+      const uint32_t *tile_class = common && plain_visits ? nullptr : ctx->tile_inside.p;
+      hipLaunchKernelGGL(common ? k_depth_pass<true> : k_depth_pass<false>,
                          dim3(static_cast<uint32_t>(ctx->n_tiles)), dim3(64), 0, ctx->stream, ctx->sxyz.p,
                          ctx->sxyz.p + plane, ctx->sxyz.p + 2 * plane, ctx->n, ctx->dcam, ctx->frames.p, frame_begin,
-                         frame_end, ctx->depth_sq.p, cells, frame_begin, ctx->tile_mask.p, ctx->tile_inside.p,
+                         frame_end, ctx->depth_sq.p, cells, frame_begin, ctx->tile_mask.p, tile_class,
                          ctx->mask_words, ctx->tile_order.p);
       if (z_maps)
         hipLaunchKernelGGL(k_depth_finish, dim3(static_cast<uint32_t>(std::min<int64_t>(div_up(map_cells, kBlock), 4096))),
@@ -2110,6 +2144,34 @@
   return PCP_OK;
 }
 
+int pcp_tile_interior_masks(pcp_context *ctx, int64_t *tiles, int32_t *mask_words, uint32_t *out_words) {
+  if (!ctx) return PCP_ERR_INVALID;
+  if (!ctx->tile_inside.p || ctx->n_tiles == 0 || ctx->n_frames == 0 || !ctx->tile_order_live)
+    return set_error(ctx, PCP_ERR_STATE, "pcp_tile_interior_masks: no masks (call pcp_depth_pass)");
+  if (!is_common_camera(ctx))
+    return set_error(ctx, PCP_ERR_STATE, "pcp_tile_interior_masks: the configured camera has no interior class (z-buffer cull with its "
+                     "depth buffer on and tame p1 / p2 only)");
+  if (tiles) *tiles = ctx->n_tiles;
+  if (mask_words) *mask_words = ctx->mask_words;
+  if (out_words) {
+    PCP_HIP_TRY(ctx, hipSetDevice(ctx->device));
+    PCP_HIP_TRY(ctx, hipMemcpyAsync(out_words, ctx->tile_inside.p, static_cast<size_t>(ctx->n_tiles) * ctx->mask_words * 4,
+                                    hipMemcpyDeviceToHost, ctx->stream));
+    PCP_HIP_TRY(ctx, hipStreamSynchronize(ctx->stream));
+  }
+  return PCP_OK;
+}
+
+int pcp_cloud_order(pcp_context *ctx, int64_t capacity, int32_t *out_index) {
+  if (!ctx) return PCP_ERR_INVALID;
+  if (!ctx->perm.p || ctx->n == 0) return set_error(ctx, PCP_ERR_STATE, "pcp_cloud_order: no cloud (call pcp_upload_cloud)");
+  if (!out_index || capacity < ctx->n) return set_error(ctx, PCP_ERR_INVALID, "pcp_cloud_order: out_index must hold the cloud");
+  PCP_HIP_TRY(ctx, hipSetDevice(ctx->device));
+  PCP_HIP_TRY(ctx, hipMemcpyAsync(out_index, ctx->perm.p, static_cast<size_t>(ctx->n) * 4, hipMemcpyDeviceToHost, ctx->stream));
+  PCP_HIP_TRY(ctx, hipStreamSynchronize(ctx->stream));
+  return PCP_OK;
+}
+
 int pcp_colour_result_device(pcp_context *ctx, void **device_ptr, int64_t *n_words) {
   if (!ctx) return PCP_ERR_INVALID;
   if (!ctx->colour_result_live)
@@ -2204,4 +2266,28 @@
   return PCP_OK;
 }
 
-}
+int pcp_selftest_depth_visits(pcp_context *ctx, int64_t samples, uint64_t seed, int64_t *interior_tiles, int64_t *points_checked,
+                              int64_t *mismatches, int32_t *interior_form) {
+  if (!ctx) return PCP_ERR_INVALID;
+  if (!ctx->have_camera) return set_error(ctx, PCP_ERR_STATE, "pcp_selftest_depth_visits: pcp_set_camera has not been called");
+  PCP_HIP_TRY(ctx, hipSetDevice(ctx->device));
+  if (samples < 0) return set_error(ctx, PCP_ERR_INVALID, "pcp_selftest_depth_visits: negative sample count");
+  const bool active = is_common_camera(ctx);
+  unsigned long long h[3] = {0, 0, 0};
+  if (active && samples > 0) {
+    PCP_HIP_TRY(ctx, ctx->s_counter.ensure(4));
+    unsigned long long *out = ctx->s_counter.p;
+    PCP_HIP_TRY(ctx, hipMemsetAsync(out, 0, 32, ctx->stream));
+    hipLaunchKernelGGL(k_selftest_interior, dim3(blocks_for(samples)), dim3(kBlock), 0, ctx->stream, ctx->dcam, ctx->interior_box, samples, seed, out);
+    PCP_HIP_TRY(ctx, hipGetLastError());
+    PCP_HIP_TRY(ctx, hipMemcpyAsync(h, out, 24, hipMemcpyDeviceToHost, ctx->stream));
+    PCP_HIP_TRY(ctx, hipStreamSynchronize(ctx->stream));
+  }
+  if (interior_tiles) *interior_tiles = static_cast<int64_t>(h[0]);
+  if (points_checked) *points_checked = static_cast<int64_t>(h[1]);
+  if (mismatches) *mismatches = static_cast<int64_t>(h[2]);
+  if (interior_form) *interior_form = active ? 1 : 0;
+  return PCP_OK;
+}
+
+}
diff --git a/pointcloudprocessor_amd/csrc/pcp_context.hip b/pointcloudprocessor_amd/csrc/pcp_context.hip
--- a/pointcloudprocessor_amd/csrc/pcp_context.hip
+++ b/pointcloudprocessor_amd/csrc/pcp_context.hip
@@ -862,6 +862,7 @@
     d.v_hi = std::max(ch, static_cast<float>(d.img_h)) + 0.5f;
   }
   if (const char *e = std::getenv("PCP_DISABLE_PRETEST")) d.pretest = (e[0] == '1') ? 0 : 1;
+  ctx->interior_box = dv::interior_box(d);
 
   ctx->have_camera = true;
   for (hipStream_t us : ctx->upload_stream)
diff --git a/pointcloudprocessor_amd/csrc/pcp_depth_visit.hpp b/pointcloudprocessor_amd/csrc/pcp_depth_visit.hpp
--- /dev/null
+++ b/pointcloudprocessor_amd/csrc/pcp_depth_visit.hpp
@@ -0,0 +1,111 @@
+#pragma once
+
+#include <stdint.h>
+
+#if defined(__HIPCC__)
+#include <hip/hip_runtime.h>
+#define PCP_DV_HD __host__ __device__ __forceinline__
+#else
+#define PCP_DV_HD inline
+#endif
+
+namespace pcp {
+namespace dv {
+
+struct Interval {
+  double lo, hi;
+};
+PCP_DV_HD Interval iv_add(Interval a, Interval b) { return {a.lo + b.lo, a.hi + b.hi}; }
+PCP_DV_HD Interval iv_scale(double k, Interval a) { return k >= 0.0 ? Interval{k * a.lo, k * a.hi} : Interval{k * a.hi, k * a.lo}; }
+PCP_DV_HD Interval iv_mul(Interval a, Interval b) {
+  const double p0 = a.lo * b.lo, p1 = a.lo * b.hi, p2 = a.hi * b.lo, p3 = a.hi * b.hi;
+  return {__builtin_fmin(__builtin_fmin(p0, p1), __builtin_fmin(p2, p3)), __builtin_fmax(__builtin_fmax(p0, p1), __builtin_fmax(p2, p3))};
+}
+PCP_DV_HD Interval iv_sqr(Interval a) {
+  const double l = __builtin_fabs(a.lo), h = __builtin_fabs(a.hi);
+  const double mx = __builtin_fmax(l, h), mn = (a.lo <= 0.0 && a.hi >= 0.0) ? 0.0 : __builtin_fmin(l, h);
+  return {mn * mn, mx * mx};
+}
+PCP_DV_HD Interval iv_mul_pos(Interval a, Interval b) { return {a.lo * b.lo, a.hi * b.hi}; }
+PCP_DV_HD Interval iv_mul_by_pos(Interval a, Interval b) {
+  return {a.lo * (a.lo >= 0.0 ? b.lo : b.hi), a.hi * (a.hi >= 0.0 ? b.hi : b.lo)};
+}
+PCP_DV_HD double iv_rcp_pos(double b) {
+#if defined(__HIP_DEVICE_COMPILE__)
+  double r = __builtin_amdgcn_rcp(b);
+  r = __builtin_fma(__builtin_fma(-b, r, 1.0), r, r);
+  r = __builtin_fma(__builtin_fma(-b, r, 1.0), r, r);
+  return r;
+#else
+  return 1.0 / b;
+#endif
+}
+PCP_DV_HD Interval iv_pad(Interval a) {
+  const double e = 1e-12 * (__builtin_fabs(a.lo) + __builtin_fabs(a.hi)) + 1e-300;
+  return {a.lo - e, a.hi + e};
+}
+
+PCP_DV_HD void interval_normalised(double X, double Y, double Z, double rho, Interval &xn, Interval &yn) {
+  const Interval zi{Z - rho, Z + rho};
+  const Interval iz{iv_rcp_pos(zi.hi) * (1.0 - 1e-13), iv_rcp_pos(zi.lo) * (1.0 + 1e-13)};
+  xn = iv_pad(iv_mul_by_pos(Interval{X - rho, X + rho}, iz));
+  yn = iv_pad(iv_mul_by_pos(Interval{Y - rho, Y + rho}, iz));
+}
+
+template <class Cam>
+PCP_DV_HD void interval_image(const Cam &c, Interval xn, Interval yn, Interval &u, Interval &v) {
+  const Interval x2 = iv_sqr(xn), y2 = iv_sqr(yn);
+  const Interval r2 = iv_add(x2, y2);
+  const Interval r4 = iv_mul_pos(r2, r2);
+  const Interval r6 = iv_mul_pos(r2, r4);
+  Interval rc = iv_add(iv_add(iv_scale(c.k1, r2), iv_scale(c.k2, r4)), iv_scale(c.k3, r6));
+  rc.lo += 1.0;
+  rc.hi += 1.0;
+  const Interval t1 = iv_scale(2.0, iv_mul(xn, yn));
+  const Interval t2 = iv_add(r2, iv_scale(2.0, x2));
+  const Interval t3 = iv_add(r2, iv_scale(2.0, y2));
+  const Interval xd = iv_pad(iv_add(iv_add(iv_mul(rc, xn), iv_scale(c.p1, t1)), iv_scale(c.p2, t2)));
+  const Interval yd = iv_pad(iv_add(iv_add(iv_mul(rc, yn), iv_scale(c.p1, t3)), iv_scale(c.p2, t1)));
+  u = iv_pad(iv_scale(c.fx, xd));
+  v = iv_pad(iv_scale(c.fy, yd));
+  u.lo += c.cx; u.hi += c.cx;
+  v.lo += c.cy; v.hi += c.cy;
+}
+
+constexpr double kInteriorMargin = 2.0;
+constexpr double kInteriorMagnitude = 0x1p38;
+
+struct InteriorBox {
+  double lo, u_hi, v_hi;
+  double r2_max;
+};
+
+template <class Cam>
+inline InteriorBox interior_box(const Cam &c) {
+  InteriorBox b{kInteriorMargin, 0.0, 0.0, 0.0};
+  b.u_hi = __builtin_fmin(static_cast<double>(c.mw) * static_cast<double>(c.ds), static_cast<double>(c.img_w)) - kInteriorMargin;
+  b.v_hi = __builtin_fmin(static_cast<double>(c.mh) * static_cast<double>(c.ds), static_cast<double>(c.img_h)) - kInteriorMargin;
+  for (double r2 = 0x1p40; r2 >= 0x1p-40; r2 *= 0.5) {
+    const double r = __builtin_sqrt(r2) * (1.0 + 0x1p-40);
+    const double A = 1.0 + r2 * (__builtin_fabs(c.k1) + r2 * (__builtin_fabs(c.k2) + r2 * __builtin_fabs(c.k3)));
+    const double T = 3.0 * (__builtin_fabs(c.p1) + __builtin_fabs(c.p2)) * r2;
+    const double Su = __builtin_fabs(c.fx) * (A * r + T) + __builtin_fabs(c.cx);
+    const double Sv = __builtin_fabs(c.fy) * (A * r + T) + __builtin_fabs(c.cy);
+    if (2.0 * Su <= kInteriorMagnitude && 2.0 * Sv <= kInteriorMagnitude) {
+      b.r2_max = r2;
+      break;
+    }
+  }
+  if (!(b.u_hi > b.lo && b.v_hi > b.lo)) b.r2_max = 0.0;
+  return b;
+}
+
+PCP_DV_HD bool interior_pair(const InteriorBox &b, Interval xn, Interval yn, Interval u, Interval v) {
+  const double xa = __builtin_fmax(__builtin_fabs(xn.lo), __builtin_fabs(xn.hi)), ya = __builtin_fmax(__builtin_fabs(yn.lo), __builtin_fabs(yn.hi));
+  return (u.lo > b.lo) & (u.hi < b.u_hi) & (v.lo > b.lo) & (v.hi < b.v_hi) & (xa * xa + ya * ya <= b.r2_max);
+}
+
+PCP_DV_HD int32_t interior_cell(float qx, float qy, int32_t mw) { return static_cast<int32_t>(qy) * mw + static_cast<int32_t>(qx); }
+
+}
+}
diff --git a/pointcloudprocessor_amd/csrc/pcp_internal.hpp b/pointcloudprocessor_amd/csrc/pcp_internal.hpp
--- a/pointcloudprocessor_amd/csrc/pcp_internal.hpp
+++ b/pointcloudprocessor_amd/csrc/pcp_internal.hpp
@@ -10,6 +10,7 @@
 #include <string>
 #include <vector>
 
+#include "pcp_depth_visit.hpp"
 #include "pcp_hip.h"
 
 namespace pcp {
@@ -171,6 +172,7 @@
   pcp_camera camera{};
   pcp_cull_params cull{};
   pcp::DevCamera dcam{};
+  pcp::dv::InteriorBox interior_box{};
 
   int64_t n = 0;
   int64_t nonfinite_points = 0;
diff --git a/pointcloudprocessor_amd/host/depth_visits_selftest.cpp b/pointcloudprocessor_amd/host/depth_visits_selftest.cpp
--- /dev/null
+++ b/pointcloudprocessor_amd/host/depth_visits_selftest.cpp
@@ -0,0 +1,194 @@
+#include <cmath>
+#include <cstdint>
+#include <cstdio>
+#include <cstdlib>
+
+#include "../csrc/pcp_depth_visit.hpp"
+#include "../csrc/pcp_visit_forms.hpp"
+
+namespace dv = pcp::dv;
+namespace vf = pcp::vf;
+
+static uint64_t mix(uint64_t v) {
+  v += 0x9e3779b97f4a7c15ull;
+  v = (v ^ (v >> 30)) * 0xbf58476d1ce4e5b9ull;
+  v = (v ^ (v >> 27)) * 0x94d049bb133111ebull;
+  return v ^ (v >> 31);
+}
+
+struct Camera {
+  const char *name;
+  double fx, fy, cx, cy, k1, k2, p1, p2, k3;
+  int32_t img_w, img_h, cull_w, cull_h, ds;
+  int32_t mw, mh;
+  float ds_f, ds_rcp, cull_wf, cull_hf;
+  float u_lo, u_hi, v_lo, v_hi;
+};
+static Camera make_camera(const char *name, double fx, double fy, double cx, double cy, double k1, double k2, double p1, double p2,
+                          double k3, int32_t w, int32_t h, int32_t ds) {
+  Camera c{name, fx, fy, cx, cy, k1, k2, p1, p2, k3, w, h, w, h, ds, w / ds, h / ds, 0, 0, 0, 0, 0, 0, 0, 0};
+  c.ds_f = static_cast<float>(ds);
+  c.ds_rcp = 1.0f / c.ds_f;
+  c.cull_wf = static_cast<float>(w);
+  c.cull_hf = static_cast<float>(h);
+  c.u_lo = c.v_lo = -(c.ds_f + 0.5f);
+  c.u_hi = std::fmax(c.ds_f * static_cast<float>(c.mw), static_cast<float>(w)) + 0.5f;
+  c.v_hi = std::fmax(c.ds_f * static_cast<float>(c.mh), static_cast<float>(h)) + 0.5f;
+  return c;
+}
+
+static int classify(const Camera &c, const float *m, double norm_bound, const float *sph) {
+  const double cx = sph[0], cy = sph[1], cz = sph[2];
+  const double X = (m[0] * cx + m[1] * cy) + (m[2] * cz + m[3]);
+  const double Y = (m[4] * cx + m[5] * cy) + (m[6] * cz + m[7]);
+  const double Z = (m[8] * cx + m[9] * cy) + (m[10] * cz + m[11]);
+  const double mag = norm_bound * (std::fabs(cx) + std::fabs(cy) + std::fabs(cz) + 3.0 * sph[3]) + std::fabs(static_cast<double>(m[3])) +
+                     std::fabs(static_cast<double>(m[7])) + std::fabs(static_cast<double>(m[11])) + 1e-3;
+  const double rho = norm_bound * static_cast<double>(sph[3]) * (1.0 + 1e-6) + 1e-6 * mag;
+  if (!(rho >= 0.0) || !std::isfinite(X + Y + Z + rho)) return 0;
+  if (Z + rho <= 0.0) return 1;
+  if (Z - rho <= 0.0) return 0;
+  if (!(Z - rho >= 1e-290)) return 0;
+  dv::Interval xn, yn, u, v;
+  dv::interval_normalised(X, Y, Z, rho, xn, yn);
+  dv::interval_image(c, xn, yn, u, v);
+  if (!std::isfinite(u.lo + u.hi + v.lo + v.hi)) return 0;
+  if (u.hi < static_cast<double>(c.u_lo) || u.lo > static_cast<double>(c.u_hi) || v.hi < static_cast<double>(c.v_lo) ||
+      v.lo > static_cast<double>(c.v_hi))
+    return 1;
+  if (!(u.lo > static_cast<double>(c.u_lo) + 1.0 && u.hi < static_cast<double>(c.u_hi) - 1.0 &&
+        v.lo > static_cast<double>(c.v_lo) + 1.0 && v.hi < static_cast<double>(c.v_hi) - 1.0))
+    return 0;
+  return dv::interior_pair(dv::interior_box(c), xn, yn, u, v) ? 3 : 2;
+}
+
+static void xform(const float *m, float x, float y, float z, float &xc, float &yc, float &zc) {
+  xc = x * m[0] + (y * m[1] + (z * m[2] + m[3]));
+  yc = x * m[4] + (y * m[5] + (z * m[6] + m[7]));
+  zc = x * m[8] + (y * m[9] + (z * m[10] + m[11]));
+}
+static float div_by_ds(const Camera &c, float x) {
+  float q = x * c.ds_rcp;
+  float e = std::fma(-c.ds_f, q, x);
+  q = std::fma(e, c.ds_rcp, q);
+  e = std::fma(-c.ds_f, q, x);
+  return std::fma(e, c.ds_rcp, q);
+}
+
+struct Tally {
+  long tiles = 0, interior = 0, inside = 0, points = 0, bad = 0;
+};
+
+static void check_point(const Camera &c, const float *m, float x, float y, float z, Tally &t) {
+  float xc, yc, zc;
+  xform(m, x, y, z, xc, yc, zc);
+  const vf::Distortion d{c.k1, c.k2, c.k3, c.p1, c.p2};
+  const double xn = static_cast<double>(xc) / static_cast<double>(zc), yn = static_cast<double>(yc) / static_cast<double>(zc);
+  double xd, yd;
+  vf::distort_written(d, xn, yn, xd, yd);
+  const double u = c.fx * xd + c.cx, v = c.fy * yd + c.cy;
+  const int32_t cell = vf::map_cell_written(static_cast<float>(u) / c.ds_f, static_cast<float>(v) / c.ds_f, c.cull_wf, c.cull_hf, c.mw, c.mh);
+  const bool pixel = u > -1.0 && u < static_cast<double>(c.img_w) && v > -1.0 && v < static_cast<double>(c.img_h);
+  double xs, ys;
+  vf::distort_short(d, xn, yn, xs, ys);
+  const double us = c.fx * xs + c.cx, vs = c.fy * ys + c.cy;
+  const int32_t got = dv::interior_cell(div_by_ds(c, static_cast<float>(us)), div_by_ds(c, static_cast<float>(vs)), c.mw);
+  ++t.points;
+  if (!(zc > 0.0f) || cell < 0 || !pixel || got != cell) {
+    if (t.bad < 10)
+      std::printf("%s: point (%a, %a, %a): zc %a cell %d pixel %d, interior form %d (u %.17g v %.17g)\n", c.name, x, y, z, zc, cell,
+                  pixel ? 1 : 0, got, u, v);
+    ++t.bad;
+  }
+}
+
+static Tally check_camera(const Camera &c, long tiles) {
+  Tally t;
+  uint64_t h = mix(0x5eedull + static_cast<uint64_t>(c.img_w) * 977u + static_cast<uint64_t>(c.ds));
+  auto unit = [&]() {
+    h = mix(h);
+    return static_cast<double>(h >> 11) * 0x1p-53;
+  };
+  for (long i = 0; i < tiles; ++i) {
+    double q[4], qn = 0.0;
+    for (double &e : q) {
+      e = 2.0 * unit() - 1.0;
+      qn += e * e;
+    }
+    if (qn < 1e-3) continue;
+    qn = std::sqrt(qn);
+    const double a = q[0] / qn, b = q[1] / qn, cc = q[2] / qn, d = q[3] / qn;
+    const double R[9] = {a * a + b * b - cc * cc - d * d, 2 * (b * cc - a * d), 2 * (b * d + a * cc),
+                         2 * (b * cc + a * d), a * a - b * b + cc * cc - d * d, 2 * (cc * d - a * b),
+                         2 * (b * d - a * cc), 2 * (cc * d + a * b), a * a - b * b - cc * cc + d * d};
+    float m[12];
+    double frob = 0.0;
+    for (int r = 0; r < 3; ++r) {
+      for (int k = 0; k < 3; ++k) {
+        m[4 * r + k] = static_cast<float>(R[3 * r + k]);
+        frob += static_cast<double>(m[4 * r + k]) * m[4 * r + k];
+      }
+      m[4 * r + 3] = static_cast<float>((unit() - 0.5) * 16.0);
+    }
+    const double norm_bound = std::sqrt(frob) * (1.0 + 1e-6);
+    const double depth = std::exp2(unit() * 9.0 - 3.0), rad = depth * std::exp2(-2.0 - unit() * 10.0);
+    double u0 = (unit() * 1.4 - 0.2) * c.img_w, v0 = (unit() * 1.4 - 0.2) * c.img_h;
+    if ((i & 3) == 0) {
+      const double W = std::fmin(static_cast<double>(c.mw) * c.ds, c.img_w), H = std::fmin(static_cast<double>(c.mh) * c.ds, c.img_h);
+      const double edge = dv::kInteriorMargin + rad / depth * std::fabs(c.fx) + (unit() * 8.0 - 4.0);
+      switch ((i >> 2) & 3) {
+        case 0: u0 = edge; break;
+        case 1: u0 = W - edge; break;
+        case 2: v0 = edge; break;
+        default: v0 = H - edge; break;
+      }
+    }
+    const double pc[3] = {(u0 - c.cx) / c.fx * depth, (v0 - c.cy) / c.fy * depth, depth};
+    float sph[4];
+    for (int k = 0; k < 3; ++k) {
+      double w = 0.0;
+      for (int r = 0; r < 3; ++r) w += static_cast<double>(m[4 * r + k]) * (pc[r] - static_cast<double>(m[4 * r + 3]));
+      sph[k] = static_cast<float>(w);
+    }
+    sph[3] = static_cast<float>(rad);
+    ++t.tiles;
+    const int cls = classify(c, m, norm_bound, sph);
+    if (cls >= 2) ++t.inside;
+    if (cls != 3) continue;
+    ++t.interior;
+    for (int k = 0; k < 16; ++k) {
+      double o[3], on = 0.0;
+      for (double &e : o) {
+        e = 2.0 * unit() - 1.0;
+        on += e * e;
+      }
+      const double s = 0.9 * rad * ((k & 1) ? 1.0 / std::sqrt(on + 1e-30) : 0.57735);
+      check_point(c, m, static_cast<float>(sph[0] + s * o[0]), static_cast<float>(sph[1] + s * o[1]), static_cast<float>(sph[2] + s * o[2]), t);
+    }
+  }
+  std::printf("%s: %ld tiles, %ld inside, %ld interior, %ld points, %ld mismatches\n", c.name, t.tiles, t.inside, t.interior, t.points, t.bad);
+  return t;
+}
+
+int main(int argc, char **argv) {
+  const long tiles = argc > 1 ? std::atol(argv[1]) : 400000;
+  const double k1 = 0.003043514741045163, k2 = 0.06634739187544138, p1 = -0.000217681797407554, p2 = -0.0006654964142658197;
+  const Camera sets[] = {
+      make_camera("cfg", 2258.5, 2258.5, 960.0, 540.0, k1, k2, p1, p2, 0.0, 1920, 1080, 14),
+      make_camera("ref", 4818.200388954926, 4819.10345841615, 2032.4178620390019, 1535.1895959282901, k1, k2, p1, p2, 0.0, 4096, 3000, 14),
+      make_camera("tiny", 564.625, 564.625, 240.0, 135.0, k1, k2, p1, p2, 0.0, 480, 270, 14),
+      make_camera("pinhole", 600.0, 600.0, 351.5, 202.5, 0.0, 0.0, 0.0, 0.0, 0.0, 703, 405, 14),
+      make_camera("tame_edge", 600.0, 600.0, 351.5, 202.5, 0.1, 0.2, 0x1p-400, -0x1p400, 0.3, 703, 405, 7),
+      make_camera("fold_back", 564.625, 564.625, 240.0, 135.0, -0.3, 0.0, 0.0, 0.0, 0.0, 480, 270, 14),
+      make_camera("tangential_only", 564.625, 564.625, 240.0, 135.0, 0.0, 0.0, 0.01, -0.02, 0.0, 480, 270, 1),
+      make_camera("ds_one_wide", 3000.0, 3000.0, 8000.0, 50.0, k1, k2, p1, p2, 0.0, 1 << 14, 100, 1),
+  };
+  long bad = 0, interior = 0;
+  for (const Camera &c : sets) {
+    const Tally t = check_camera(c, tiles);
+    bad += t.bad;
+    interior += t.interior;
+  }
+  std::printf("depth_visits_selftest: %ld interior tiles, %ld mismatches\n", interior, bad);
+  return bad == 0 ? 0 : 1;
+}
diff --git a/pointcloudprocessor_amd/host_build.py b/pointcloudprocessor_amd/host_build.py
--- a/pointcloudprocessor_amd/host_build.py
+++ b/pointcloudprocessor_amd/host_build.py
@@ -16,6 +16,7 @@
     "format_selftest": ["format_selftest.cpp"],
     "parse_selftest": ["parse_selftest.cpp"],
     "visit_forms_selftest": ["visit_forms_selftest.cpp"],
+    "depth_visits_selftest": ["depth_visits_selftest.cpp"],
     "voxel_reduce_selftest": ["voxel_reduce_selftest.cpp"],
     "normals_selftest": ["normals_selftest.cpp"],
 }
@@ -27,7 +28,7 @@
     for name, srcs in TARGETS.items():
         exe = os.path.join(BIN, name)
         deps = [os.path.join(HOST, s) for s in srcs] + [os.path.join(HOST, "pcp_shim.hpp"), os.path.join(HOST, "pcp_multi.hpp"), os.path.join(HOST, "pcd_io.hpp"), os.path.join(HOST, "image_io.hpp"), os.path.join(HOST, "pcd_device_reader.hpp"),
-                                                       os.path.join(_build.CSRC, "pcp_ascii_parse.hpp"), os.path.join(_build.CSRC, "pcp_ascii.hpp"), os.path.join(_build.CSRC, "pcp_visit_forms.hpp"), os.path.join(_build.CSRC, "pcp_voxel_reduce.hpp"), os.path.join(_build.CSRC, "pcp_normals.hpp"),
+                                                       os.path.join(_build.CSRC, "pcp_ascii_parse.hpp"), os.path.join(_build.CSRC, "pcp_ascii.hpp"), os.path.join(_build.CSRC, "pcp_visit_forms.hpp"), os.path.join(_build.CSRC, "pcp_depth_visit.hpp"), os.path.join(_build.CSRC, "pcp_voxel_reduce.hpp"), os.path.join(_build.CSRC, "pcp_normals.hpp"),
                                                        os.path.join(_build.INCLUDE, "pcp_hip.h")]
         deps = [d for d in deps if os.path.exists(d)]
         stale = force or not os.path.exists(exe) or any(os.path.getmtime(d) > os.path.getmtime(exe) for d in deps)
diff --git a/profiles/depth_visit_counts.py b/profiles/depth_visit_counts.py
--- /dev/null
+++ b/profiles/depth_visit_counts.py
@@ -0,0 +1,28 @@
+#!/usr/bin/env python3
+import json
+import os
+import sys
+
+import numpy as np
+
+sys.path.insert(0, os.path.dirname(os.path.dirname(os.path.abspath(__file__))))
+import torch
+
+from pointcloudprocessor_amd import capi, synth
+
+kind = sys.argv[1] if len(sys.argv) > 1 else "cfg"
+cam = synth.camera_dict(kind)
+N = int(sys.argv[2]) if len(sys.argv) > 2 else 10_000_000
+F = int(sys.argv[3]) if len(sys.argv) > 3 else 256
+x, y, z, _ = synth.make_cloud(N)
+poses, _ = synth.make_trajectory(F)
+ctx = capi.Context(0)
+ctx.set_camera(capi.camera_from_dict(cam))
+ctx.upload_cloud(x, y, z)
+ctx.set_frames(poses)
+ctx.depth_pass()
+ctx.synchronize()
+masks, interior = ctx.tile_masks(), ctx.tile_interior_masks()
+bits = lambda a: int(np.unpackbits(a.view(np.uint8)).sum())
+print(json.dumps({"camera": kind, "tiles": int(masks.shape[0]), "keyframes": F, "pairs_after_refinement": bits(masks),
+                  "interior_pairs": bits(interior), "interior_not_kept": bits(interior & ~masks)}))
```

Measured after the change: 1.927 million. About the same (-0.7%).
